# FunAudioLLM/CosyVoice

Measured on NVIDIA H100. Metric: audio-sec/s, CosyVoice2-0.5B zero-shot batch-32, NFE=10, higher is better.
Workload: dtype bf16

## Files before the change

cosyvoice_b200/csrc/cvk_internal.h:

```cpp
#pragma once
#include <cuda_runtime.h>
#include <cuda_bf16.h>
#include <cuda_fp16.h>
#include <cuda.h>
#include <stdint.h>
#include <stdio.h>
#include <string>
#include <vector>
#include <map>
#include <unordered_map>
#include <stdexcept>
#include <atomic>

#include "../../include/cvk.h"

typedef __nv_bfloat16 bf16;

struct CvkError : std::runtime_error {
  int code;
  CvkError(int c, const std::string& m) : std::runtime_error(m), code(c) {}
};

#define CVK_CHECK_CUDA(expr)                                                                       \
  do {                                                                                             \
    cudaError_t _e = (expr);                                                                       \
    if (_e != cudaSuccess)                                                                         \
      throw CvkError(CVK_ERR_CUDA, std::string(#expr) + ": " + cudaGetErrorString(_e) + " @" +     \
                                       __FILE__ + ":" + std::to_string(__LINE__));                 \
  } while (0)

#define CVK_REQUIRE(cond, msg)                                                                     \
  do {                                                                                             \
    if (!(cond))                                                                                   \
      throw CvkError(CVK_ERR_INVALID, std::string(msg) + " (" #cond ") @" + __FILE__ + ":" +       \
                                          std::to_string(__LINE__));                               \
  } while (0)

#define CVK_LAUNCH_CHECK() CVK_CHECK_CUDA(cudaGetLastError())

enum DType { DT_F32 = 0, DT_BF16 = 1, DT_F16 = 2 };

struct Mat {
  void* p = nullptr;
  int dtype = DT_F32;
  int rows = 0;
  int cols = 0;
  int ld = 0;
  Mat() {}
  Mat(void* p_, int dt, int r, int c, int ld_) : p(p_), dtype(dt), rows(r), cols(c), ld(ld_) {}
  size_t esize() const { return dtype == DT_F32 ? 4 : 2; }
  Mat slice(int c0, int n) const { return Mat((char*)p + (size_t)c0 * esize(), dtype, rows, n, ld); }
  float* f32() const { return (float*)p; }
  bf16* b16() const { return (bf16*)p; }
};

struct Seqs {
  int B = 0;
  int R = 0;
  std::vector<int> start, len;
  int* d_start = nullptr;
  int* d_len = nullptr;
  int* d_row2seq = nullptr;
  int max_len = 0;
  int64_t sum_len = 0;
};

struct ConvW {
  int N = 0, K = 0, taps = 1, dil = 1, shift0 = 0;
  float* w32 = nullptr;
  bf16* w16 = nullptr;
  __half* wf16 = nullptr;
  float* bias = nullptr;
};

enum Act {
  ACT_NONE = 0, ACT_GELU = 1, ACT_SILU = 2, ACT_MISH = 3, ACT_ELU = 4, ACT_LRELU = 5, ACT_SNAKE = 6, ACT_TANH = 7, ACT_ABS = 8,
  ACT_GELU_TANH = 9
};

struct Epilogue {
  const float* bias = nullptr;
  const float* rowvec = nullptr;
  int rowvec_ld = 0;
  int act1 = ACT_NONE;
  float act1_param = 0.f;
  const float* alpha1 = nullptr;
  float scale = 1.f;
  Mat resid;
  const int* row2seq = nullptr;
  int accumulate = 0;
  Mat out;
  int act2 = ACT_NONE;
  float act2_param = 0.f;
  const float* alpha2 = nullptr;
  Mat out2;
};

extern thread_local int cvk_in_capture;

struct Arena {
  char* base = nullptr;
  size_t cap = 0, off = 0, high = 0;
  void* alloc(size_t bytes) {
    size_t a = (off + 255) & ~(size_t)255;
    if (a + bytes > cap) throw CvkError(CVK_ERR_OOM, "workspace arena exhausted: need " + std::to_string(a + bytes) +
                                                          " of " + std::to_string(cap));
    off = a + bytes;
    if (off > high) high = off;
    return base + a;
  }
  void reset() { off = 0; }
};

struct RawTensor {
  float* p = nullptr;
  std::vector<int64_t> shape;
  int64_t numel() const { int64_t n = 1; for (auto s : shape) n *= s; return n; }
};

enum ProfFamily { FAM_GEMM_TC = 0, FAM_GEMM_SIMT = 1, FAM_ATTN = 2, FAM_COUNT = 3 };
struct ProfRec {
  cudaEvent_t a, b;
  int family;
  double work;
  double bytes;
};

struct HiftModel;
struct FlowModel;
struct DitModel;
struct LlmModel;

struct cvk_ctx {
  int device = 0;
  int precision = CVK_PREC_FP32;
  int act_dtype = DT_F32;
  int num_sms = 132;
  std::string last_error;
  std::map<std::string, RawTensor> raw;
  std::vector<void*> owned;
  Arena arena;
  HiftModel* hift = nullptr;
  HiftModel* hift3 = nullptr;
  void* hift3_extra = nullptr;
  FlowModel* flow = nullptr;
  DitModel* dit = nullptr;
  LlmModel* llm = nullptr;
  void* mel_model = nullptr;
  void* prompt_feat_model = nullptr;
  void* encode_tiled = nullptr;
  std::atomic<int64_t> launches{0};
  int op_out_bf16 = 0;
  int op_iters = 0;
  double op_ms = 0.0;
  int tc_epi = 2;
  int tc_persist = 2;
  void* tl = nullptr;
  int tl_seq = 0;
  long long* tl_next() {
    if (!tl) return nullptr;
    long long* p = (long long*)tl + 4 * (tl_seq % 1024);
    ++tl_seq;
    return p;
  }
  int prof_on = 0;
  std::vector<ProfRec> prof;
  std::unordered_map<const void*, void*> tiled;
  std::vector<cudaEvent_t> event_pool;
  int pdl = 1;
  int lm_fused = 1;
  int hift_f16 = 1;
  int build_f16 = 0;
  int enc_tc_attn = 1;
  int lm_mega = 0;
  int mega_coop = 1;
  int use_skinny = 1;
  int use_tc_attn = 1;
  int use_graph = 1;
  int use_tc = 1;
  int flow_fused_ff = 1;
  int flow_qkv_panel = 1;

  void* dmalloc(size_t bytes) {
    void* p = nullptr;
    CVK_CHECK_CUDA(cudaMalloc(&p, bytes ? bytes : 16));
    owned.push_back(p);
    return p;
  }
  const RawTensor& get_raw(const std::string& name) const {
    auto it = raw.find(name);
    if (it == raw.end()) throw CvkError(CVK_ERR_MISSING_WEIGHT, "missing weight tensor: " + name);
    return it->second;
  }
  bool has_raw(const std::string& name) const { return raw.find(name) != raw.end(); }
};

template <typename... KArgs, typename... Args>
inline void launch_ex(void (*kern)(KArgs...), dim3 grid, dim3 block, size_t smem, cudaStream_t st, bool pdl, Args&&... args) {
  cudaLaunchConfig_t cfg = {};
  cfg.gridDim = grid;
  cfg.blockDim = block;
  cfg.dynamicSmemBytes = smem;
  cfg.stream = st;
  cudaLaunchAttribute at[1];
  if (pdl) {
    at[0].id = cudaLaunchAttributeProgrammaticStreamSerialization;
    at[0].val.programmaticStreamSerializationAllowed = 1;
    cfg.attrs = at;
    cfg.numAttrs = 1;
  }
  CVK_CHECK_CUDA(cudaLaunchKernelEx(&cfg, kern, KArgs(std::forward<Args>(args))...));
}

void encode_tma_map(cvk_ctx* ctx, CUtensorMap* map, const void* base, int rank, const cuuint64_t* dims, const cuuint64_t* strides,
                    const cuuint32_t* box, int dtype, CUtensorMapL2promotion l2, const char* what);
void gemm_tc_setup();
void attention_tc_setup();
void skinny_setup();

Seqs make_seqs(cvk_ctx* ctx, const int* lens, int B, int gap, int scale, int extra_front, cudaStream_t st, bool with_row2seq = true);
Seqs scale_seqs(cvk_ctx* ctx, const Seqs& s, int scale, int extra_front, cudaStream_t st, bool with_row2seq = true);

ConvW make_linear(cvk_ctx* ctx, const std::string& wname, const std::string& bname);
ConvW make_conv(cvk_ctx* ctx, const float* w_oik , const float* bias, int N, int K, int taps,
                int dil, int shift0);
ConvW make_conv_named(cvk_ctx* ctx, const std::string& wname, const std::string& bname, int dil, int shift0);
float* fold_weight_norm(cvk_ctx* ctx, const std::string& prefix, int64_t* numel_out);
void finish_convw(cvk_ctx* ctx, ConvW& w);
float* dev_copy_f32(cvk_ctx* ctx, const float* src_dev, size_t n);

void conv_gemm(cvk_ctx* ctx, cudaStream_t st, const Mat& A, const ConvW& W, const Epilogue& ep);
void conv_gemm_simt(cvk_ctx* ctx, cudaStream_t st, const Mat& A, const ConvW& W, const Epilogue& ep);
void conv_gemm_tc(cvk_ctx* ctx, cudaStream_t st, const Mat& A, const ConvW& W, const Epilogue& ep);
void ffn_fused(cvk_ctx* ctx, cudaStream_t st, const Mat& x, const int* row2seq, const float* ln3_g, const float* ln3_b, const ConvW& w1,
               const ConvW& w2, const float* ln_g, const float* ln_b, const Mat& out);
void flow_ff(cvk_ctx* ctx, cudaStream_t st, const Mat& x, const int* row2seq, const float* ln3_g, const float* ln3_b, const ConvW& ff1,
             const ConvW& ff2, const float* ln_g, const float* ln_b, const Mat& out, const Mat& xn, const Mat& hid);
size_t skinny_scratch_floats(int rows, int maxN);
const bf16* skinny_tiled_weights(cvk_ctx* ctx, const ConvW& W);
int conv_gemm_skinny_ex(cvk_ctx* ctx, cudaStream_t st, const Mat& A, const ConvW& W, const Epilogue& ep, float* scratch, size_t scratch_floats,
                        int mode);
void conv_gemm_skinny(cvk_ctx* ctx, cudaStream_t st, const Mat& A, const ConvW& W, const Epilogue& ep, float* scratch, size_t scratch_floats);

void zero_mat(cvk_ctx* ctx, cudaStream_t st, const Mat& m);
void layernorm(cvk_ctx* ctx, cudaStream_t st, const Mat& x, const float* gamma, const float* beta, float eps, int act,
               float post_scale, const int* row2seq, const Mat& out, const float* rowvec = nullptr, int rowvec_ld = 0);
void unpack_rows_skip(cvk_ctx* ctx, cudaStream_t st, const Mat& in, const Seqs& s, const int* skip_host, float* dense, int C);
Seqs shrink_seqs(cvk_ctx* ctx, const Seqs& s, int drop_tail, cudaStream_t st);
Seqs subseqs(cvk_ctx* ctx, const Seqs& s, const int* skip_host, cudaStream_t st);
void rmsnorm(cvk_ctx* ctx, cudaStream_t st, const Mat& x, const float* gamma, float eps, const Mat& out);
void act_copy(cvk_ctx* ctx, cudaStream_t st, const Mat& x, int act, float param, const float* alpha, const int* row2seq,
              const Mat& out);
void act_copy_scaled(cvk_ctx* ctx, cudaStream_t st, const Mat& x, float pre_scale, int act, float param, const float* alpha,
                     const int* row2seq, const Mat& out);
void pack_rows(cvk_ctx* ctx, cudaStream_t st, const float* dense, int C, const Seqs& s, const Mat& out);
void unpack_rows(cvk_ctx* ctx, cudaStream_t st, const Mat& in, const Seqs& s, int skip, float* dense, int C);
void bcast_rows(cvk_ctx* ctx, cudaStream_t st, const float* vec, int C, int vec_ld, const Seqs& s, const Mat& out);
void convert_mat(cvk_ctx* ctx, cudaStream_t st, const Mat& in, const Mat& out);

struct KvGeom {
  const int* d_kstart = nullptr;
  const int* d_klen = nullptr;
  const int* d_qoff = nullptr;
};
void whisper_log_mel(cvk_ctx* ctx, const float* wav, const int* lens, int B, float* out, cudaStream_t st);
void kaldi_fbank80(cvk_ctx* ctx, const float* wav, const int* lens, int B, int subtract_mean, float* out, cudaStream_t st);
struct cvk_flow_stream;
cvk_flow_stream* flow_stream_create(cvk_ctx* ctx, int kind, int slots, int max_frames, int n_timesteps);
void flow_stream_destroy(cvk_flow_stream* fs);
size_t flow_stream_bytes(const cvk_flow_stream* fs);
void flow_stream_begin(cvk_ctx* ctx, cvk_flow_stream* fs, int slot, const float* prompt_feat, int prompt_frames, const float* embedding,
                       cudaStream_t st);
void flow_stream_chunk(cvk_ctx* ctx, cvk_flow_stream* fs, int B, const int* slots, const int32_t* tokens, const int* token_lens,
                       float* mel_out, int mel_cap_frames, int* n_out, cudaStream_t st);
void attention_fwd(cvk_ctx* ctx, cudaStream_t st, const Mat& q, const Mat& k, const Mat& v, const Seqs& s, int H, int chunk,
                   float scale, const Mat& out, int kv_div = 1, const KvGeom* kg = nullptr);
void relpos_attention_fwd(cvk_ctx* ctx, cudaStream_t st, const Mat& q, const Mat& k, const Mat& v, const Mat& pos ,
                          int pos_center, const float* bias_u, const float* bias_v, const Seqs& s, int H, int chunk, float scale,
                          const Mat& out);

struct ProfScope {
  cvk_ctx* ctx;
  cudaStream_t st;
  ProfRec rec;
  bool on;
  ProfScope(cvk_ctx* c, cudaStream_t s, int family, double work, double bytes) : ctx(c), st(s), on(c->prof_on && !cvk_in_capture) {
    if (!on) return;
    auto get = [&]() {
      cudaEvent_t e;
      if (!ctx->event_pool.empty()) { e = ctx->event_pool.back(); ctx->event_pool.pop_back(); }
      else cudaEventCreate(&e);
      return e;
    };
    rec.a = get(); rec.b = get(); rec.family = family; rec.work = work; rec.bytes = bytes;
    cudaEventRecord(rec.a, st);
  }
  ~ProfScope() {
    if (!on) return;
    cudaEventRecord(rec.b, st);
    ctx->prof.push_back(rec);
  }
};

static inline int ceil_div(int a, int b) { return (a + b - 1) / b; }
static inline int round_up(int a, int b) { return ceil_div(a, b) * b; }

inline Mat arena_mat(cvk_ctx* ctx, int dtype, int rows, int cols, int ld = 0) {
  if (ld == 0) ld = round_up(cols, 8);
  size_t es = dtype == DT_F32 ? 4 : 2;
  void* p = ctx->arena.alloc((size_t)rows * ld * es);
  return Mat(p, dtype, rows, cols, ld);
}
```

cosyvoice_b200/csrc/gemm_skinny.cu:

```cuda
#include "common.cuh"
#include "wgmma.cuh"
#include "tma.cuh"

namespace {

constexpr int SK_BM = 128;
constexpr int SK_BK = 64;
constexpr int SK_STAGES = 8;
constexpr int SK_THREADS = 384;

__global__ void tile_weights_kernel(const bf16* __restrict__ w, bf16* __restrict__ out, int N, int K, int tiles, int kchunks) {
  size_t total = (size_t)tiles * kchunks * SK_BM * 8;
  for (size_t i = blockIdx.x * (size_t)blockDim.x + threadIdx.x; i < total; i += (size_t)gridDim.x * blockDim.x) {
    int c = i & 7;
    int r = (i >> 3) & (SK_BM - 1);
    size_t blk = i >> 10;
    int kc = blk % kchunks, nt = blk / kchunks;
    int n = nt * SK_BM + r, k = kc * SK_BK + c * 8;
    uint4 v = make_uint4(0, 0, 0, 0);
    if (n < N && k + 8 <= K) v = *reinterpret_cast<const uint4*>(w + (size_t)n * K + k);
    else if (n < N && k < K) {
      __align__(16) bf16 t[8];
      for (int e = 0; e < 8; ++e) t[e] = k + e < K ? w[(size_t)n * K + k + e] : __float2bfloat16_rn(0.f);
      v = *reinterpret_cast<uint4*>(t);
    }
    *reinterpret_cast<uint4*>(reinterpret_cast<char*>(out) + blk * (SK_BM * SK_BK * 2) + r * 128 + ((c ^ (r & 7)) << 4)) = v;
  }
}

template <int BPAD>
__global__ void __launch_bounds__(SK_THREADS, 1)
skinny_gemm_kernel(const bf16* __restrict__ w_tiled, const __grid_constant__ CUtensorMap tmap_x, int N, int K, int rows,
                   int chunks_per_split, float* __restrict__ partial , EpiDev ep, int swiglu,
                   long long* __restrict__ tl) {
  extern __shared__ uint8_t smem_raw[];
  pdl_trigger();
  tl_stamp(tl, 0);
  __shared__ __align__(8) uint64_t bar_full[SK_STAGES];
  __shared__ __align__(8) uint64_t bar_empty[SK_STAGES];
  constexpr uint32_t A_BYTES = SK_BM * SK_BK * 2;
  constexpr uint32_t B_BYTES = BPAD * SK_BK * 2;
  constexpr uint32_t STAGE = A_BYTES + B_BYTES;

  const uint32_t base = (smem_u32(smem_raw) + 1023u) & ~1023u;
  const int warp = threadIdx.x >> 5, lane = threadIdx.x & 31;
  const int n0 = blockIdx.x * SK_BM;
  const int kchunks = (K + SK_BK - 1) / SK_BK;
  const int kc0 = blockIdx.y * chunks_per_split;
  const int kc1 = min(kchunks, kc0 + chunks_per_split);
  const int iters = kc1 - kc0;

  if (threadIdx.x == 0) {
    for (int s = 0; s < SK_STAGES; ++s) {
      mbar_init(smem_u32(&bar_full[s]), 1);
      mbar_init(smem_u32(&bar_empty[s]), 8);
    }
    asm volatile("fence.mbarrier_init.release.cluster;" ::: "memory");
  }
  __syncthreads();

  if (warp < 4) {
    if (warp == 0 && lane == 0) {
      const int pre = min(iters, SK_STAGES);
      for (int it = 0; it < pre; ++it) {
        const uint32_t fb = smem_u32(&bar_full[it]);
        mbar_expect_tx(fb, STAGE);
        bulk_load(base + it * STAGE, w_tiled + ((size_t)blockIdx.x * kchunks + (kc0 + it)) * (SK_BM * SK_BK), A_BYTES, fb);
      }
      pdl_wait();
      tl_stamp(tl, 1);
      for (int it = 0; it < pre; ++it) tma_load_2d(base + it * STAGE + A_BYTES, &tmap_x, smem_u32(&bar_full[it]), (kc0 + it) * SK_BK, 0);
      for (int it = pre; it < iters; ++it) {
        const int s = it % SK_STAGES;
        const uint32_t round = (uint32_t)(it / SK_STAGES);
        mbar_wait(smem_u32(&bar_empty[s]), (round & 1u) ^ 1u);
        const uint32_t sa = base + s * STAGE, sb = sa + A_BYTES;
        const uint32_t fb = smem_u32(&bar_full[s]);
        mbar_expect_tx(fb, STAGE);
        bulk_load(sa, w_tiled + ((size_t)blockIdx.x * kchunks + (kc0 + it)) * (SK_BM * SK_BK), A_BYTES, fb);
        tma_load_2d(sb, &tmap_x, fb, (kc0 + it) * SK_BK, 0);
      }
    } else {
      pdl_wait();
    }
  } else {
    const int wg = (threadIdx.x - 128) >> 7;
    const int q = lane & 3;
    const int fr = wg * 64 + (warp & 3) * 16 + (lane >> 2);
    float bias_n[2];
#pragma unroll
    for (int hh = 0; hh < 2; ++hh) bias_n[hh] = (!partial && !swiglu && ep.bias && n0 + fr + 8 * hh < N) ? ep.bias[n0 + fr + 8 * hh] : 0.f;
    pdl_wait();
    float acc[BPAD / 2];
#pragma unroll
    for (int e = 0; e < BPAD / 2; ++e) acc[e] = 0.f;
    for (int it = 0; it < iters; ++it) {
      const int s = it % SK_STAGES;
      mbar_wait(smem_u32(&bar_full[s]), (uint32_t)(it / SK_STAGES) & 1u);
      const uint32_t sa = base + s * STAGE + (uint32_t)wg * (A_BYTES / 2), sb = base + s * STAGE + A_BYTES;
      const uint64_t da = wg_desc_sw128(sa), db = wg_desc_sw128(sb);
      wg_fence();
#pragma unroll
      for (int k = 0; k < SK_BK / 16; ++k) wgmma_ss<BPAD, 0>(acc, da + (uint64_t)(2 * k), db + (uint64_t)(2 * k), 1);
      wg_commit();
      wg_wait<0>();
      __syncwarp();
      if (lane == 0) mbar_arrive(smem_u32(&bar_empty[s]));
    }
    wg_touch<BPAD / 2>(acc);
    const bool plain = ep.act1 == ACT_NONE && !ep.resid && !ep.rowvec && !ep.row2seq && !ep.accumulate && !ep.out2 && ep.scale == 1.f;
#pragma unroll
    for (int e = 0; e < BPAD / 2; ++e) {
      const int hh = (e >> 1) & 1;
      const int n = n0 + fr + 8 * hh, b = 8 * (e >> 2) + 2 * q + (e & 1);
      if (swiglu) {
        const float other = __shfl_xor_sync(0xffffffffu, acc[e], 4);
        if (!((lane >> 2) & 1) && n + 1 < N && b < rows) {
          const float g = acc[e];
          st_any(ep.out, ep.out_dtype, (size_t)b * ep.out_ld + (n >> 1), __fdividef(g, 1.f + fast_exp(-g)) * other);
        }
      } else if (n < N && b < rows) {
        if (partial) partial[((size_t)blockIdx.y * rows + b) * N + n] = acc[e];
        else if (plain) st_any(ep.out, ep.out_dtype, (size_t)b * ep.out_ld + n, acc[e] + bias_n[hh]);
        else epi_store(ep, b, n, acc[e]);
      }
    }
  }
  tl_stamp(tl, 2);
}

__global__ void splitk_finish_kernel(const float* __restrict__ partial, int splits, int rows, int N, EpiDev ep, long long* __restrict__ tl) {
  pdl_trigger();
  tl_stamp(tl, 0);
  pdl_wait();
  tl_stamp(tl, 1);
  size_t total = (size_t)rows * N;
  for (size_t i = blockIdx.x * (size_t)blockDim.x + threadIdx.x; i < total; i += (size_t)gridDim.x * blockDim.x) {
    float acc = 0.f;
    for (int s = 0; s < splits; ++s) acc += partial[(size_t)s * total + i];
    epi_store(ep, (int)(i / N), (int)(i % N), acc);
  }
  tl_stamp(tl, 2);
}

template <int BPAD>
constexpr size_t skinny_smem() {
  return (size_t)SK_STAGES * (SK_BM * SK_BK * 2 + BPAD * SK_BK * 2) + 1024;
}

template <int BPAD>
void launch(cudaStream_t st, dim3 grid, const bf16* tw, const CUtensorMap& tx, const ConvW& W, int rows, int cps, float* partial,
            const EpiDev& e, int swiglu, bool pdl, long long* tl) {
  launch_ex(skinny_gemm_kernel<BPAD>, grid, dim3(SK_THREADS), skinny_smem<BPAD>(), st, pdl, tw, tx, W.N, W.K, rows, cps, partial, e, swiglu, tl);
}

}

const bf16* skinny_tiled_weights(cvk_ctx* ctx, const ConvW& W) {
  auto it = ctx->tiled.find(W.w16);
  if (it != ctx->tiled.end()) return (const bf16*)it->second;
  CVK_REQUIRE(!cvk_in_capture, "skinny_tiled_weights: weight was not pre-tiled before graph capture");
  const int tiles = ceil_div(W.N, SK_BM), kchunks = ceil_div(W.K, SK_BK);
  bf16* out = (bf16*)ctx->dmalloc((size_t)tiles * kchunks * SK_BM * SK_BK * sizeof(bf16));
  tile_weights_kernel<<<ctx->num_sms * 8, 256>>>(W.w16, out, W.N, W.K, tiles, kchunks);
  CVK_LAUNCH_CHECK();
  CVK_CHECK_CUDA(cudaDeviceSynchronize());
  ctx->tiled[W.w16] = out;
  return out;
}

size_t skinny_scratch_floats(int rows, int maxN) { return (size_t)32 * rows * maxN; }

int conv_gemm_skinny_ex(cvk_ctx* ctx, cudaStream_t st, const Mat& A, const ConvW& W, const Epilogue& ep, float* scratch, size_t scratch_floats,
                        int mode) {
  CVK_REQUIRE(A.dtype == DT_BF16 && W.w16 != nullptr && W.taps == 1, "conv_gemm_skinny: bf16 1-tap operands required");
  const int rows = mode == 1 ? A.rows : ep.out.rows;
  CVK_REQUIRE(rows <= 64 && A.rows >= rows, "conv_gemm_skinny: at most 64 rows");
  CVK_REQUIRE(W.K % 8 == 0 && A.ld % 8 == 0 && ((uintptr_t)A.p & 15) == 0, "conv_gemm_skinny: 16-byte aligned operands required");
  const int BPAD = rows <= 32 ? 32 : 64;
  CUtensorMap tx;
  const bf16* tw = skinny_tiled_weights(ctx, W);
  {
    const cuuint64_t dims[2] = {(cuuint64_t)W.K, (cuuint64_t)rows};
    const cuuint64_t strides[1] = {(cuuint64_t)A.ld * 2};
    const cuuint32_t box[2] = {SK_BK, (cuuint32_t)BPAD};
    encode_tma_map(ctx, &tx, A.p, 2, dims, strides, box, DT_BF16, CU_TENSOR_MAP_L2_PROMOTION_L2_128B, "skinny x");
  }
  const int tiles = ceil_div(W.N, SK_BM);
  const int kchunks = ceil_div(W.K, SK_BK);
  int splits = ctx->num_sms / tiles;
  if (splits > kchunks / 4) splits = kchunks / 4;
  if (splits > 32) splits = 32;
  if (splits < 1) splits = 1;
  int cps = ceil_div(kchunks, splits);
  splits = ceil_div(kchunks, cps);
  if (mode == 2 || (splits > 1 && (scratch == nullptr || (size_t)splits * rows * W.N > scratch_floats))) {
    splits = 1;
    cps = kchunks;
  }
  CVK_REQUIRE(mode != 1 || (scratch != nullptr && (size_t)splits * rows * W.N <= scratch_floats), "conv_gemm_skinny: scratch too small");
  EpiDev e = to_dev(ep);
  if (!e.bias) e.bias = W.bias;
  const double flops = 2.0 * rows * (double)W.N * W.K;
  const double bytes = (double)W.N * W.K * 2 + (double)rows * W.K * 2 + (double)rows * W.N * 2;
  ProfScope ps(ctx, st, FAM_GEMM_TC, flops, bytes);
  dim3 grid(tiles, splits);
  float* partial = (splits > 1 || mode == 1) ? scratch : nullptr;
  long long* tl = ctx->tl_next();
  if (BPAD == 32) launch<32>(st, grid, tw, tx, W, rows, cps, partial, e, mode == 2, ctx->pdl != 0, tl);
  else launch<64>(st, grid, tw, tx, W, rows, cps, partial, e, mode == 2, ctx->pdl != 0, tl);
  ctx->launches++;
  CVK_LAUNCH_CHECK();
  if (splits > 1 && mode == 0) {
    size_t total = (size_t)rows * W.N;
    int g = (int)((total + 255) / 256);
    if (g > ctx->num_sms * 4) g = ctx->num_sms * 4;
    launch_ex(splitk_finish_kernel, dim3(g), dim3(256), 0, st, ctx->pdl != 0, (const float*)partial, splits, rows, W.N, e, ctx->tl_next());
    ctx->launches++;
    CVK_LAUNCH_CHECK();
  }
  return splits;
}

void conv_gemm_skinny(cvk_ctx* ctx, cudaStream_t st, const Mat& A, const ConvW& W, const Epilogue& ep, float* scratch, size_t scratch_floats) {
  conv_gemm_skinny_ex(ctx, st, A, W, ep, scratch, scratch_floats, 0);
}

void skinny_setup() {
  CVK_CHECK_CUDA(cudaFuncSetAttribute(skinny_gemm_kernel<32>, cudaFuncAttributeMaxDynamicSharedMemorySize, (int)skinny_smem<32>()));
  CVK_CHECK_CUDA(cudaFuncSetAttribute(skinny_gemm_kernel<64>, cudaFuncAttributeMaxDynamicSharedMemorySize, (int)skinny_smem<64>()));
  CVK_CHECK_CUDA(cudaFuncSetAttribute(skinny_gemm_kernel<32>, cudaFuncAttributePreferredSharedMemoryCarveout, cudaSharedmemCarveoutMaxShared));
  CVK_CHECK_CUDA(cudaFuncSetAttribute(skinny_gemm_kernel<64>, cudaFuncAttributePreferredSharedMemoryCarveout, cudaSharedmemCarveoutMaxShared));
  CVK_CHECK_CUDA(cudaFuncSetAttribute(splitk_finish_kernel, cudaFuncAttributePreferredSharedMemoryCarveout, cudaSharedmemCarveoutMaxShared));
}
```

cosyvoice_b200/csrc/llm.cu:

```cuda
#include "llm_decode_attn.cuh"
#include <math.h>
#include <algorithm>

using namespace lm;

namespace {

float* copy_param(cvk_ctx* ctx, const std::string& name) {
  const RawTensor& t = ctx->get_raw(name);
  return dev_copy_f32(ctx, t.p, (size_t)t.numel());
}

ConvW concat_linear(cvk_ctx* ctx, const std::vector<std::string>& wn, const std::vector<std::string>& bn) {
  int K = (int)ctx->get_raw(wn[0]).shape[1], N = 0;
  for (auto& n : wn) N += (int)ctx->get_raw(n).shape[0];
  ConvW w;
  w.N = N; w.K = K;
  w.w32 = (float*)ctx->dmalloc((size_t)N * K * sizeof(float));
  size_t off = 0;
  for (auto& n : wn) {
    const RawTensor& t = ctx->get_raw(n);
    CVK_CHECK_CUDA(cudaMemcpy(w.w32 + off, t.p, (size_t)t.numel() * sizeof(float), cudaMemcpyDeviceToDevice));
    off += t.numel();
  }
  if (!bn.empty()) {
    w.bias = (float*)ctx->dmalloc((size_t)N * sizeof(float));
    size_t bo = 0;
    for (auto& n : bn) {
      const RawTensor& t = ctx->get_raw(n);
      CVK_CHECK_CUDA(cudaMemcpy(w.bias + bo, t.p, (size_t)t.numel() * sizeof(float), cudaMemcpyDeviceToDevice));
      bo += t.numel();
    }
  }
  finish_convw(ctx, w);
  return w;
}

__global__ void build_input_kernel(const int32_t* __restrict__ text, const int* __restrict__ text_off, const int* __restrict__ text_len,
                                   const int32_t* __restrict__ speech, const int* __restrict__ sp_off, const int* __restrict__ sp_len,
                                   const float* __restrict__ text_emb, const float* __restrict__ llm_emb, const float* __restrict__ speech_emb,
                                   const int* __restrict__ start, float* __restrict__ out) {
  int b = blockIdx.y;
  int nt = text_len[b], ns = sp_len[b];
  int L = 1 + nt + 1 + ns;
  for (int t = blockIdx.x; t < L; t += gridDim.x) {
    const float* src;
    if (t == 0) src = llm_emb;
    else if (t <= nt) src = text_emb + (size_t)text[text_off[b] + t - 1] * D;
    else if (t == nt + 1) src = llm_emb + D;
    else src = speech_emb + (size_t)speech[sp_off[b] + t - nt - 2] * D;
    float* dst = out + (size_t)(start[b] + t) * D;
    for (int c = threadIdx.x; c < D; c += blockDim.x) dst[c] = src[c];
  }
}

template <typename T>
__global__ void rope_append_kernel(T* __restrict__ qkv, int ld, const int* __restrict__ start, const int* __restrict__ len,
                                   const int* __restrict__ pos0, const float* __restrict__ inv_freq, T* __restrict__ kc, T* __restrict__ vc,
                                   int max_ctx, int rows_are_seqs, const int2* __restrict__ rowpos) {
  int b = blockIdx.y;
  int L = rows_are_seqs ? 1 : len[b];
  int base = rows_are_seqs ? b : start[b];
  const int cb = rowpos ? rowpos[b].x : b;
  const int p0 = rowpos ? rowpos[b].y : (pos0 ? pos0[b] : 0);
  for (int t = blockIdx.x; t < L; t += gridDim.x) {
    int pos = p0 + t;
    T* row = qkv + (size_t)(base + t) * ld;
    for (int e = threadIdx.x; e < (NH + NKV) * (HD / 2); e += blockDim.x) {
      int h = e / (HD / 2), i = e % (HD / 2);
      float fr = (float)pos * inv_freq[i];
      float c = cosf(fr), s = sinf(fr);
      T* p = row + h * HD;
      float x1 = to_f32(p[i]), x2 = to_f32(p[i + HD / 2]);
      p[i] = from_f32<T>(x1 * c - x2 * s);
      p[i + HD / 2] = from_f32<T>(x2 * c + x1 * s);
    }
    __syncthreads();
    if (pos < max_ctx) {
      for (int e = threadIdx.x; e < NKV * HD; e += blockDim.x) {
        int h = e / HD, d = e % HD;
        size_t ci = (((size_t)cb * NKV + h) * max_ctx + pos) * HD + d;
        kc[ci] = row[NH * HD + e];
        vc[ci] = row[NH * HD + NKV * HD + e];
      }
    }
    __syncthreads();
  }
}

template <typename T>
__global__ void __launch_bounds__((NH / NKV) * 32)
decode_attn_kernel(const T* __restrict__ qkv, int ld, const T* __restrict__ kc, const T* __restrict__ vc,
                   const int* __restrict__ ctx_len, int max_ctx, T* __restrict__ out, int ldo, const int2* __restrict__ rowpos) {
  extern __shared__ float sc_all[];
  const int b = blockIdx.x, kvh = blockIdx.y;
  const int w = threadIdx.x >> 5, lane = threadIdx.x & 31;
  const int h = kvh * (NH / NKV) + w;
  const int cb = rowpos ? rowpos[b].x : b;
  const int L = min((rowpos ? rowpos[b].y : ctx_len[b]) + 1, max_ctx);
  float* sc = sc_all + (size_t)w * max_ctx;
  const T* q = qkv + (size_t)b * ld + h * HD;
  const T* kb = kc + ((size_t)cb * NKV + kvh) * max_ctx * HD;
  const T* vb = vc + ((size_t)cb * NKV + kvh) * max_ctx * HD;
  float qr[HD];
#pragma unroll
  for (int d = 0; d < HD; ++d) qr[d] = to_f32(q[d]) * 0.125f;
  float m = -INFINITY;
  for (int j = lane; j < L; j += 32) {
    const T* kr = kb + (size_t)j * HD;
    float s = 0.f;
    if (sizeof(T) == 2) {
      const uint4* k4 = reinterpret_cast<const uint4*>(kr);
#pragma unroll
      for (int c = 0; c < 8; ++c) {
        uint4 u = k4[c];
        const __nv_bfloat162* h2 = reinterpret_cast<const __nv_bfloat162*>(&u);
#pragma unroll
        for (int e = 0; e < 4; ++e) {
          float2 f = __bfloat1622float2(h2[e]);
          s = fmaf(qr[c * 8 + 2 * e], f.x, s);
          s = fmaf(qr[c * 8 + 2 * e + 1], f.y, s);
        }
      }
    } else {
      const float4* k4 = reinterpret_cast<const float4*>(kr);
#pragma unroll
      for (int c = 0; c < 16; ++c) {
        float4 f = k4[c];
        s = fmaf(qr[c * 4], f.x, s);
        s = fmaf(qr[c * 4 + 1], f.y, s);
        s = fmaf(qr[c * 4 + 2], f.z, s);
        s = fmaf(qr[c * 4 + 3], f.w, s);
      }
    }
    sc[j] = s;
    m = fmaxf(m, s);
  }
  m = warp_max(m);
  float l = 0.f;
  for (int j = lane; j < L; j += 32) {
    float p = expf(sc[j] - m);
    sc[j] = p;
    l += p;
  }
  l = warp_sum(l);
  __syncwarp();
  float o0 = 0.f, o1 = 0.f;
  int j = 0;
  for (; j + 4 <= L; j += 4) {
    float p0 = sc[j], p1 = sc[j + 1], p2 = sc[j + 2], p3 = sc[j + 3];
    const T* v0 = vb + (size_t)j * HD;
    float a0 = to_f32(v0[lane]), a1 = to_f32(v0[lane + 32]);
    float b0 = to_f32(v0[HD + lane]), b1 = to_f32(v0[HD + lane + 32]);
    float c0 = to_f32(v0[2 * HD + lane]), c1 = to_f32(v0[2 * HD + lane + 32]);
    float d0 = to_f32(v0[3 * HD + lane]), d1 = to_f32(v0[3 * HD + lane + 32]);
    o0 = fmaf(p0, a0, o0); o1 = fmaf(p0, a1, o1);
    o0 = fmaf(p1, b0, o0); o1 = fmaf(p1, b1, o1);
    o0 = fmaf(p2, c0, o0); o1 = fmaf(p2, c1, o1);
    o0 = fmaf(p3, d0, o0); o1 = fmaf(p3, d1, o1);
  }
  for (; j < L; ++j) {
    float p = sc[j];
    o0 = fmaf(p, to_f32(vb[(size_t)j * HD + lane]), o0);
    o1 = fmaf(p, to_f32(vb[(size_t)j * HD + lane + 32]), o1);
  }
  T* op = out + (size_t)b * ldo + h * HD;
  float inv = 1.f / l;
  op[lane] = from_f32<T>(o0 * inv);
  op[lane + 32] = from_f32<T>(o1 * inv);
}

__global__ void qkv_reduce_kernel(const float* __restrict__ partial, int splits, int rows, const float* __restrict__ bias, bf16* __restrict__ qkv) {
  const size_t total = (size_t)rows * QKV_N;
  for (size_t i = blockIdx.x * (size_t)blockDim.x + threadIdx.x; i < total; i += (size_t)gridDim.x * blockDim.x) {
    float acc = 0.f;
    for (int s = 0; s < splits; ++s) acc += partial[(size_t)s * total + i];
    qkv[i] = __float2bfloat16_rn(acc + bias[i % QKV_N]);
  }
}

__global__ void __launch_bounds__(D) finish_rms_kernel(const float* __restrict__ partial, int splits, int rows, float* __restrict__ x,
                                                       const float* __restrict__ gamma, bf16* __restrict__ xn, long long* __restrict__ tl) {
  __shared__ float red[D / 32];
  pdl_trigger();
  tl_stamp(tl, 0);
  const int b = blockIdx.x, n = threadIdx.x;
  const float gam = gamma[n];
  pdl_wait();
  tl_stamp(tl, 1);
  const float* p = partial + (size_t)b * D + n;
  const size_t stride = (size_t)rows * D;
  float a0 = 0.f, a1 = 0.f, a2 = 0.f, a3 = 0.f;
  int s = 0;
  for (; s + 4 <= splits; s += 4) {
    a0 += p[(size_t)s * stride];
    a1 += p[(size_t)(s + 1) * stride];
    a2 += p[(size_t)(s + 2) * stride];
    a3 += p[(size_t)(s + 3) * stride];
  }
  for (; s < splits; ++s) a0 += p[(size_t)s * stride];
  const float v = x[(size_t)b * D + n] + ((a0 + a1) + (a2 + a3));
  x[(size_t)b * D + n] = v;
  float ss = warp_sum(v * v);
  if ((n & 31) == 0) red[n >> 5] = ss;
  __syncthreads();
  float tot = 0.f;
#pragma unroll
  for (int i = 0; i < D / 32; ++i) tot += red[i];
  xn[(size_t)b * D + n] = __float2bfloat16_rn(gam * (v * rsqrtf(tot / D + RMS_EPS)));
  tl_stamp(tl, 2);
}

constexpr int AF_WARPS = 16;
__global__ void __launch_bounds__(32 * AF_WARPS)
attn_fused_kernel(const float* __restrict__ partial , int splits, int rows, const float* __restrict__ bias,
                  bf16* __restrict__ kc, bf16* __restrict__ vc, const int* __restrict__ ctx_len, int max_ctx,
                  const float* __restrict__ inv_freq, bf16* __restrict__ out, int ldo, long long* __restrict__ tl) {
  extern __shared__ float sm_all[];
  const int b = blockIdx.x, kvh = blockIdx.y;
  pdl_trigger();
  tl_stamp(tl, 0);
  bf16* kb = kc + ((size_t)b * NKV + kvh) * max_ctx * HD;
  bf16* vb = vc + ((size_t)b * NKV + kvh) * max_ctx * HD;
  const int p0 = min(*reinterpret_cast<const volatile int*>(ctx_len + b), max_ctx);
  const int wj0 = (threadIdx.x >> 5) * 16;
  KvFrag pre;
  const bool have_pre = wj0 + 16 <= p0;
  if (have_pre) decode_attn_load_block(kb, vb, wj0, p0, threadIdx.x & 31, pre);
  pdl_wait();
  tl_stamp(tl, 1);
  decode_attn_unit<AF_WARPS, 0>(sm_all, threadIdx.x, partial, splits, rows, b, kvh, bias, kb, vb, ctx_len[b], max_ctx, inv_freq,
                                out + (size_t)b * ldo, pre, have_pre);
  tl_stamp(tl, 2);
}

__global__ void interleave_rows_kernel(const float* __restrict__ gu , float* __restrict__ out, int F, int K) {
  size_t total = (size_t)2 * F * K;
  for (size_t i = blockIdx.x * (size_t)blockDim.x + threadIdx.x; i < total; i += (size_t)gridDim.x * blockDim.x) {
    int k = i % K;
    int r = i / K;
    int src = (r & 1) ? F + (r >> 1) : (r >> 1);
    out[i] = gu[(size_t)src * K + k];
  }
}

template <typename T>
__global__ void swiglu_kernel(const T* __restrict__ gu, int ld, int rows, T* __restrict__ out, int ldo) {
  size_t total = (size_t)rows * DFF;
  for (size_t i = blockIdx.x * (size_t)blockDim.x + threadIdx.x; i < total; i += (size_t)gridDim.x * blockDim.x) {
    int r = i / DFF, c = i % DFF;
    float g = to_f32(gu[(size_t)r * ld + c]), u = to_f32(gu[(size_t)r * ld + DFF + c]);
    out[(size_t)r * ldo + c] = from_f32<T>(g / (1.f + expf(-g)) * u);
  }
}

__global__ void gather_last_kernel(const float* __restrict__ x, const int* __restrict__ start, const int* __restrict__ len,
                                   float* __restrict__ out) {
  int b = blockIdx.x;
  const float* src = x + (size_t)(start[b] + len[b] - 1) * D;
  for (int c = threadIdx.x; c < D; c += blockDim.x) out[(size_t)b * D + c] = src[c];
}

__global__ void ragged_embed_kernel(const int* __restrict__ ids, const int* __restrict__ kinds, const float* __restrict__ text_emb,
                                    const float* __restrict__ llm_emb, const float* __restrict__ speech_emb, float* __restrict__ x) {
  const int m = blockIdx.x, kind = kinds[m], id = ids[m];
  const float* src = kind == 0 ? text_emb + (size_t)id * D : (kind == 1 ? speech_emb + (size_t)id * D : llm_emb + (size_t)id * D);
  for (int c = threadIdx.x; c < D; c += blockDim.x) x[(size_t)m * D + c] = src[c];
}

__global__ void feed_scatter_kernel(const int* __restrict__ sc, const float* __restrict__ x, float* __restrict__ hidden, int* __restrict__ ctx_len) {
  const int i = blockIdx.x, b = sc[3 * i], ml = sc[3 * i + 1];
  for (int c = threadIdx.x; c < D; c += blockDim.x) hidden[(size_t)b * D + c] = x[(size_t)ml * D + c];
  if (threadIdx.x == 0) ctx_len[b] += sc[3 * i + 2];
}

__global__ void gather_rows_kernel(const int* __restrict__ rows, const float* __restrict__ hidden, float* __restrict__ out) {
  const int i = blockIdx.x;
  for (int c = threadIdx.x; c < D; c += blockDim.x) out[(size_t)i * D + c] = hidden[(size_t)rows[i] * D + c];
}

__device__ __forceinline__ void mma_16816_full(float* c, uint32_t a0, uint32_t a1, uint32_t a2, uint32_t a3, uint32_t b0, uint32_t b1) {
  asm volatile("mma.sync.aligned.m16n8k16.row.col.f32.bf16.bf16.f32 {%0,%1,%2,%3}, {%4,%5,%6,%7}, {%8,%9}, {%0,%1,%2,%3};"
               : "+f"(c[0]), "+f"(c[1]), "+f"(c[2]), "+f"(c[3])
               : "r"(a0), "r"(a1), "r"(a2), "r"(a3), "r"(b0), "r"(b1));
}

constexpr int RA_WARPS = 4;
__global__ void __launch_bounds__(32 * RA_WARPS)
ragged_attn_tc_kernel(const bf16* __restrict__ qkv, int ld, const bf16* __restrict__ kc, const bf16* __restrict__ vc, int max_ctx,
                      const int4* __restrict__ tiles, bf16* __restrict__ out, int ldo) {
  constexpr int G = NH / NKV;
  __shared__ float ml[RA_WARPS][16][2];
  __shared__ __align__(16) float po[RA_WARPS][16][HD];
  const int4 tl = tiles[blockIdx.x];
  const int m0 = tl.x, b = tl.y, pos0 = tl.z, n = tl.w, kvh = blockIdx.y;
  const int warp = threadIdx.x >> 5, lane = threadIdx.x & 31, g = lane >> 2, t4 = lane & 3;
  const bf16* kb = kc + ((size_t)b * NKV + kvh) * max_ctx * HD;
  const bf16* vb = vc + ((size_t)b * NKV + kvh) * max_ctx * HD;
  const int L0 = pos0 + 1, L1 = pos0 + n;
  const bf16* qa_row = qkv + (size_t)m0 * ld + (kvh * G + g) * HD;
  const bf16* qb_row = qkv + (size_t)(m0 + n - 1) * ld + (kvh * G + g) * HD;
  auto qpair = [&](const bf16* p, int d) -> uint32_t {
    if (g >= G) return 0u;
    const float2 f = __bfloat1622float2(*reinterpret_cast<const __nv_bfloat162*>(p + d));
    return pack_bf16x2(f.x * 0.125f, f.y * 0.125f);
  };
  uint32_t qf[4][4];
#pragma unroll
  for (int kk = 0; kk < 4; ++kk) {
    const int d = kk * 16 + t4 * 2;
    qf[kk][0] = qpair(qa_row, d);
    qf[kk][1] = qpair(qb_row, d);
    qf[kk][2] = qpair(qa_row, d + 8);
    qf[kk][3] = qpair(qb_row, d + 8);
  }
  float o[4][2][4];
#pragma unroll
  for (int q = 0; q < 4; ++q)
#pragma unroll
    for (int t = 0; t < 2; ++t)
#pragma unroll
      for (int e = 0; e < 4; ++e) o[q][t][e] = 0.f;
  float m_a = -INFINITY, l_a = 0.f, m_b = -INFINITY, l_b = 0.f;
  KvFrag fr;
  for (int j0 = warp * 16; j0 < L1; j0 += RA_WARPS * 16) {
    decode_attn_load_block(kb, vb, j0, L1, lane, fr);
    float s0[4] = {0.f, 0.f, 0.f, 0.f}, s1[4] = {0.f, 0.f, 0.f, 0.f};
#pragma unroll
    for (int kk = 0; kk < 4; ++kk) {
      mma_16816_full(s0, qf[kk][0], qf[kk][1], qf[kk][2], qf[kk][3], fr.kf[0][kk][0], fr.kf[0][kk][1]);
      mma_16816_full(s1, qf[kk][0], qf[kk][1], qf[kk][2], qf[kk][3], fr.kf[1][kk][0], fr.kf[1][kk][1]);
    }
    const int ka = j0 + t4 * 2;
    const int key[4] = {ka, ka + 1, ka + 8, ka + 9};
    const float sa[4] = {s0[0], s0[1], s1[0], s1[1]}, sb[4] = {s0[2], s0[3], s1[2], s1[3]};
    float mxa = -INFINITY, mxb = -INFINITY;
#pragma unroll
    for (int e = 0; e < 4; ++e) {
      if (key[e] < L0) mxa = fmaxf(mxa, sa[e]);
      if (key[e] < L1) mxb = fmaxf(mxb, sb[e]);
    }
    mxa = fmaxf(mxa, __shfl_xor_sync(0xffffffffu, mxa, 1));
    mxa = fmaxf(mxa, __shfl_xor_sync(0xffffffffu, mxa, 2));
    mxb = fmaxf(mxb, __shfl_xor_sync(0xffffffffu, mxb, 1));
    mxb = fmaxf(mxb, __shfl_xor_sync(0xffffffffu, mxb, 2));
    const float na = fmaxf(m_a, mxa), nb = fmaxf(m_b, mxb);
    const float ua = na == -INFINITY ? 0.f : na, ub = nb == -INFINITY ? 0.f : nb;
    const float ca = __expf(m_a - ua), cb = __expf(m_b - ub);
    float pa[4], pb[4];
#pragma unroll
    for (int e = 0; e < 4; ++e) {
      pa[e] = key[e] < L0 ? __expf(sa[e] - ua) : 0.f;
      pb[e] = key[e] < L1 ? __expf(sb[e] - ub) : 0.f;
    }
    l_a = l_a * ca + ((pa[0] + pa[1]) + (pa[2] + pa[3]));
    l_b = l_b * cb + ((pb[0] + pb[1]) + (pb[2] + pb[3]));
    m_a = na;
    m_b = nb;
    const uint32_t p0 = pack_bf16x2(pa[0], pa[1]), p1 = pack_bf16x2(pb[0], pb[1]), p2 = pack_bf16x2(pa[2], pa[3]), p3 = pack_bf16x2(pb[2], pb[3]);
#pragma unroll
    for (int q = 0; q < 4; ++q) {
#pragma unroll
      for (int t = 0; t < 2; ++t) {
        o[q][t][0] *= ca; o[q][t][1] *= ca;
        o[q][t][2] *= cb; o[q][t][3] *= cb;
      }
      mma_16816_full(o[q][0], p0, p1, p2, p3, __byte_perm(fr.vw[q][0], fr.vw[q][1], 0x5410), __byte_perm(fr.vw[q][2], fr.vw[q][3], 0x5410));
      mma_16816_full(o[q][1], p0, p1, p2, p3, __byte_perm(fr.vw[q][0], fr.vw[q][1], 0x7632), __byte_perm(fr.vw[q][2], fr.vw[q][3], 0x7632));
    }
  }
  l_a += __shfl_xor_sync(0xffffffffu, l_a, 1);
  l_a += __shfl_xor_sync(0xffffffffu, l_a, 2);
  l_b += __shfl_xor_sync(0xffffffffu, l_b, 1);
  l_b += __shfl_xor_sync(0xffffffffu, l_b, 2);
  if (g < G) {
    if (t4 == 0) {
      ml[warp][g][0] = m_a;
      ml[warp][g][1] = l_a;
      ml[warp][g + 8][0] = m_b;
      ml[warp][g + 8][1] = l_b;
    }
#pragma unroll
    for (int q = 0; q < 4; ++q) {
      *reinterpret_cast<float4*>(&po[warp][g][q * 16 + t4 * 4]) = make_float4(o[q][0][0], o[q][1][0], o[q][0][1], o[q][1][1]);
      *reinterpret_cast<float4*>(&po[warp][g + 8][q * 16 + t4 * 4]) = make_float4(o[q][0][2], o[q][1][2], o[q][0][3], o[q][1][3]);
    }
  }
  __syncthreads();
  for (int e = threadIdx.x; e < n * G * HD; e += 32 * RA_WARPS) {
    const int r = e / (G * HD), hq = (e / HD) % G, d = e % HD, mr = r * 8 + hq;
    float M = -INFINITY;
#pragma unroll
    for (int w2 = 0; w2 < RA_WARPS; ++w2) M = fmaxf(M, ml[w2][mr][0]);
    float num = 0.f, den = 0.f;
#pragma unroll
    for (int w2 = 0; w2 < RA_WARPS; ++w2) {
      const float wgt = __expf(ml[w2][mr][0] - M);
      den = fmaf(wgt, ml[w2][mr][1], den);
      num = fmaf(wgt, po[w2][mr][d], num);
    }
    out[(size_t)(m0 + r) * ldo + (kvh * G + hq) * HD + d] = __float2bfloat16_rn(num / den);
  }
}

static inline size_t sampler_smem(int V) { return (size_t)2 * ((V + 3) & ~3) * sizeof(float); }

__device__ __forceinline__ float block_max(float v, float* red) {
  v = warp_max(v);
  __syncthreads();
  if ((threadIdx.x & 31) == 0) red[threadIdx.x >> 5] = v;
  __syncthreads();
  float r = red[0];
  for (int i = 1; i < SAMPLER_THREADS / 32; ++i) r = fmaxf(r, red[i]);
  return r;
}
__device__ __forceinline__ float block_hsum(float seg, float* part, float* total) {
  __syncthreads();
  part[threadIdx.x] = seg;
  __syncthreads();
  if (threadIdx.x == 0) {
    float t = 0.f;
    for (int i = 0; i < SAMPLER_THREADS; ++i) t += part[i];
    *total = t;
  }
  __syncthreads();
  return *total;
}

__global__ void __launch_bounds__(SAMPLER_THREADS)
ras_sampler_kernel(float* __restrict__ scores, int V, int from_logits, const float* __restrict__ uniforms , int B,
                   const int32_t* __restrict__ min_len, const int32_t* __restrict__ max_len, int32_t* __restrict__ out_ids, int out_ld,
                   int32_t* __restrict__ out_count, int32_t* __restrict__ done, int* __restrict__ ctx_len, const int* __restrict__ base_len,
                   int* __restrict__ live,
                   const float* __restrict__ speech_emb, float* __restrict__ next_x,
                   const int32_t* __restrict__ history, int hist_ld, const int32_t* __restrict__ hist_count,
                   const int32_t* __restrict__ ignore_eos_in, int32_t* __restrict__ ids_out, const float* __restrict__ ln_gamma,
                   bf16* __restrict__ xn_out, long long* __restrict__ tl, long long* __restrict__ dbg_fine) {
  extern __shared__ __align__(16) float sp_all[];
  __shared__ float red[SAMPLER_THREADS / 32];
  __shared__ float part[SAMPLER_THREADS];
  __shared__ float tot;
  __shared__ int bi[2][SAMPLER_THREADS / 32];
  __shared__ float kept_p[TOPK];
  __shared__ int kept_i[TOPK];
  __shared__ int s_n, s_top;

  const int b = blockIdx.x, tid = threadIdx.x;
  const bool standalone = ids_out != nullptr;
  pdl_trigger();
  tl_stamp(tl, 0);
  pdl_wait();
  tl_stamp(tl, 1);
  long long* sf = (dbg_fine && b == 0 && tid == 0) ? dbg_fine : nullptr;
  int sf_i = 0;
#define SF() do { if (sf) { long long t_; asm volatile("mov.u64 %0, %globaltimer;" : "=l"(t_)); sf[sf_i++] = t_; } } while (0)
  SF();
  if (!standalone && done[b]) { tl_stamp(tl, 2); return; }
  const int V4 = (V + 3) & ~3;
  float* sp = sp_all;
  float* x = sp_all + V4;
  float* xg = scores + (size_t)b * V;
  if ((V & 3) == 0) {
    for (int i = tid; i < V / 4; i += SAMPLER_THREADS) reinterpret_cast<float4*>(x)[i] = __ldcg(reinterpret_cast<const float4*>(xg) + i);
  } else {
    for (int i = tid; i < V; i += SAMPLER_THREADS) x[i] = __ldcg(xg + i);
  }
  const int per = (V + SAMPLER_THREADS - 1) / SAMPLER_THREADS;
  const int lo = tid * per, hi = min(lo + per, V);
  const int cnt = standalone ? hist_count[b] : out_count[b];
  const bool ignore_eos = standalone ? (ignore_eos_in[b] != 0) : (cnt < min_len[b]);
  const float u1 = standalone ? uniforms[b * 2] : uniforms[((size_t)cnt * B + b) * 2];
  const float u2 = standalone ? uniforms[b * 2 + 1] : uniforms[((size_t)cnt * B + b) * 2 + 1];
  __syncthreads();
  float xr[SAMPLER_PER], pr[SAMPLER_PER];
#pragma unroll
  for (int i = 0; i < SAMPLER_PER; ++i) xr[i] = (i < per && lo + i < hi) ? x[lo + i] : -INFINITY;
  SF();

  if (from_logits) {
    float mx = -INFINITY;
#pragma unroll
    for (int i = 0; i < SAMPLER_PER; ++i) mx = fmaxf(mx, xr[i]);
    mx = block_max(mx, red);
    float seg = 0.f;
#pragma unroll
    for (int i = 0; i < SAMPLER_PER; ++i)
      if (i < per && lo + i < hi) seg += expf(xr[i] - mx);
    float s = block_hsum(seg, part, &tot);
    float ls = logf(s);
#pragma unroll
    for (int i = 0; i < SAMPLER_PER; ++i)
      if (i < per && lo + i < hi) xr[i] = (xr[i] - mx) - ls;
  }
  SF();
  if (ignore_eos) {
#pragma unroll
    for (int i = 0; i < SAMPLER_PER; ++i)
      if (i < per && lo + i == EOS && lo + i < hi) xr[i] = -INFINITY;
  }
  float mx = -INFINITY;
#pragma unroll
  for (int i = 0; i < SAMPLER_PER; ++i) mx = fmaxf(mx, xr[i]);
  mx = block_max(mx, red);
  {
    float seg = 0.f;
#pragma unroll
    for (int i = 0; i < SAMPLER_PER; ++i) {
      const bool ok = i < per && lo + i < hi;
      float e = (!ok || xr[i] == -INFINITY) ? 0.f : expf(xr[i] - mx);
      pr[i] = e;
      if (ok) seg += e;
    }
    float s = block_hsum(seg, part, &tot);
#pragma unroll
    for (int i = 0; i < SAMPLER_PER; ++i) pr[i] = (i < per && lo + i < hi) ? pr[i] / s : -3.f;
  }
  SF();
  float c_v[3];
  int c_i[3], c_n;
  auto rebuild = [&]() {
    c_v[0] = c_v[1] = c_v[2] = -1.f;
    c_i[0] = c_i[1] = c_i[2] = -1;
#pragma unroll
    for (int i = 0; i < SAMPLER_PER; ++i) {
      const float v = pr[i];
      const int ix = lo + i;
      if (v > c_v[0]) { c_v[2] = c_v[1]; c_i[2] = c_i[1]; c_v[1] = c_v[0]; c_i[1] = c_i[0]; c_v[0] = v; c_i[0] = ix; }
      else if (v > c_v[1]) { c_v[2] = c_v[1]; c_i[2] = c_i[1]; c_v[1] = v; c_i[1] = ix; }
      else if (v > c_v[2]) { c_v[2] = v; c_i[2] = ix; }
    }
    c_n = (c_v[0] >= 0.f) + (c_v[1] >= 0.f) + (c_v[2] >= 0.f);
  };
  rebuild();
  __shared__ unsigned bk[2][SAMPLER_THREADS / 32];
  __shared__ int s_cnt[SAMPLER_THREADS / 32 + 1];
  __shared__ unsigned s_thr_key;
  int n_kept = 0;
  float cum = 0.f;
  constexpr int CAND_CAP = 512;
  unsigned* tk = reinterpret_cast<unsigned*>(sp);
  int* ti = reinterpret_cast<int*>(sp) + SAMPLER_THREADS;
  float* cv = sp + 2 * SAMPLER_THREADS;
  int* ci = reinterpret_cast<int*>(sp) + 2 * SAMPLER_THREADS + CAND_CAP;
  bool fast_done = false;
  {
    const unsigned mykey = c_n > 0 ? __float_as_uint(c_v[0]) + 1u : 0u;
    const int myidx = c_n > 0 ? c_i[0] : 0x7fffffff;
    tk[tid] = mykey;
    ti[tid] = myidx;
    __syncthreads();
    int rank = 0;
    for (int q = 0; q < SAMPLER_THREADS / 4; ++q) {
      const uint4 k4 = reinterpret_cast<const uint4*>(tk)[q];
      const int4 i4 = reinterpret_cast<const int4*>(ti)[q];
      rank += (k4.x > mykey || (k4.x == mykey && i4.x < myidx)) + (k4.y > mykey || (k4.y == mykey && i4.y < myidx)) +
              (k4.z > mykey || (k4.z == mykey && i4.z < myidx)) + (k4.w > mykey || (k4.w == mykey && i4.w < myidx));
    }
    if (tid == 0) s_thr_key = 0u;
    __syncthreads();
    if (rank == TOPK - 1) s_thr_key = mykey;
    __syncthreads();
    const unsigned thr = s_thr_key;
    if (thr != 0u) {
      int cnt = 0;
#pragma unroll
      for (int i = 0; i < SAMPLER_PER; ++i) cnt += (pr[i] >= 0.f && __float_as_uint(pr[i]) + 1u >= thr) ? 1 : 0;
      int incl = cnt;
#pragma unroll
      for (int o = 1; o < 32; o <<= 1) {
        const int t = __shfl_up_sync(0xffffffffu, incl, o);
        if ((tid & 31) >= o) incl += t;
      }
      if ((tid & 31) == 31) s_cnt[tid >> 5] = incl;
      __syncthreads();
      int base = 0, total = 0;
#pragma unroll
      for (int w = 0; w < SAMPLER_THREADS / 32; ++w) {
        if (w < (tid >> 5)) base += s_cnt[w];
        total += s_cnt[w];
      }
      if (total <= CAND_CAP) {
        int pos = base + incl - cnt;
#pragma unroll
        for (int i = 0; i < SAMPLER_PER; ++i)
          if (pr[i] >= 0.f && __float_as_uint(pr[i]) + 1u >= thr) { cv[pos] = pr[i]; ci[pos] = lo + i; ++pos; }
        __syncthreads();
        for (int j = tid; j < total; j += SAMPLER_THREADS) {
          const float vj = cv[j];
          const int ij = ci[j];
          int r = 0;
          for (int k = 0; k < total; ++k) r += (cv[k] > vj || (cv[k] == vj && ci[k] < ij)) ? 1 : 0;
          if (r < TOPK) { kept_p[r] = vj; kept_i[r] = ij; }
        }
        __syncthreads();
        const int avail = total < TOPK ? total : TOPK;
        while (n_kept < avail && cum < 0.8f) {
          cum = cum + kept_p[n_kept];
          ++n_kept;
        }
        fast_done = true;
      }
    }
  }
  for (int round = 0; round < TOPK && !fast_done; ++round) {
    if (!(cum < 0.8f)) break;
    const unsigned key = c_n > 0 ? __float_as_uint(c_v[0]) + 1u : 0u;
    const unsigned wmax = __reduce_max_sync(0xffffffffu, key);
    const int widx = __reduce_min_sync(0xffffffffu, (key == wmax && wmax != 0u) ? c_i[0] : 0x7fffffff);
    const int pb = round & 1;
    if ((tid & 31) == 0) { bk[pb][tid >> 5] = wmax; bi[pb][tid >> 5] = widx; }
    __syncthreads();
    unsigned gk = bk[pb][0];
    int gi = bi[pb][0];
#pragma unroll
    for (int w = 1; w < SAMPLER_THREADS / 32; ++w) {
      const unsigned k2 = bk[pb][w];
      const int i2 = bi[pb][w];
      if (k2 > gk || (k2 == gk && i2 < gi)) { gk = k2; gi = i2; }
    }
    if (gk == 0u) break;
    const float gv = __uint_as_float(gk - 1u);
    if (tid == 0) {
      kept_p[n_kept] = gv;
      kept_i[n_kept] = gi;
    }
    n_kept += 1;
    cum = cum + gv;
    if (gi >= lo && gi < hi) {
#pragma unroll
      for (int i = 0; i < SAMPLER_PER; ++i)
        if (lo + i == gi) pr[i] = -2.f;
      c_v[0] = c_v[1]; c_i[0] = c_i[1];
      c_v[1] = c_v[2]; c_i[1] = c_i[2];
      c_v[2] = -1.f; c_i[2] = -1;
      if (--c_n == 0) rebuild();
    }
  }
  SF();
  if (tid == 0) {
    int n = n_kept;
    float total = 0.f;
    for (int i = 0; i < n; ++i) total += kept_p[i];
    float thr = u1 * total, acc = 0.f;
    int pick = -1, last = -1;
    for (int i = 0; i < n; ++i) {
      if (kept_p[i] > 0.f) last = i;
      acc += kept_p[i];
      if (pick < 0 && acc > thr && kept_p[i] > 0.f) pick = i;
    }
    if (pick < 0) pick = last;
    int top = kept_i[pick];
    int rep = 0;
    const int32_t* hist = standalone ? history + (size_t)b * hist_ld : out_ids + (size_t)b * out_ld;
    for (int i = max(0, cnt - WIN); i < cnt; ++i) rep += hist[i] == top;
    s_top = top;
    s_n = rep >= 1 ? 1 : 0;
  }
  __syncthreads();
  SF();
  if (s_n) {
    int top = s_top;
#pragma unroll
    for (int i = 0; i < SAMPLER_PER; ++i)
      if (lo + i == top) xr[i] = -INFINITY;
    float m3 = -INFINITY;
#pragma unroll
    for (int i = 0; i < SAMPLER_PER; ++i) m3 = fmaxf(m3, xr[i]);
    m3 = block_max(m3, red);
    float seg = 0.f;
#pragma unroll
    for (int i = 0; i < SAMPLER_PER; ++i) {
      const bool ok = i < per && lo + i < hi;
      float e = (!ok || xr[i] == -INFINITY) ? 0.f : expf(xr[i] - m3);
      pr[i] = e;
      if (ok) seg += e;
    }
    float s = block_hsum(seg, part, &tot);
    seg = 0.f;
#pragma unroll
    for (int i = 0; i < SAMPLER_PER; ++i) {
      if (i < per && lo + i < hi) {
        pr[i] = pr[i] / s;
        seg += pr[i];
        sp[lo + i] = pr[i];
      }
    }
    __syncthreads();
    part[tid] = seg;
    __syncthreads();
    if (tid == 0) {
      float pre = 0.f;
      for (int i = 0; i < SAMPLER_THREADS; ++i) pre += part[i];
      float thr = u2 * pre;
      float acc = 0.f;
      int segi = -1, lastseg = -1;
      float segbase = 0.f, lastbase = 0.f;
      for (int i = 0; i < SAMPLER_THREADS; ++i) {
        if (part[i] > 0.f) {
          lastseg = i;
          lastbase = acc;
          if (acc + part[i] > thr) { segi = i; segbase = acc; break; }
        }
        acc += part[i];
      }
      int pick = -1, last = -1;
      if (segi < 0) { segi = lastseg; segbase = lastbase; }
      float sgbase = segbase;
      for (int sg = segi; sg >= 0 && sg < SAMPLER_THREADS && pick < 0; ++sg) {
        const float a0 = sgbase;
        sgbase += part[sg];
        if (sg > segi && !(part[sg] > 0.f)) continue;
        float a = a0;
        int l2 = sg * per, h2 = min(l2 + per, V);
        for (int i = l2; i < h2; ++i) {
          if (sp[i] > 0.f) last = i;
          a += sp[i];
          if (a > thr && sp[i] > 0.f) { pick = i; break; }
        }
      }
      if (pick < 0) pick = last;
      s_top = pick;
    }
    __syncthreads();
  }
  SF();
#pragma unroll
  for (int i = 0; i < SAMPLER_PER; ++i)
    if (i < per && lo + i < hi) x[lo + i] = xr[i];
  __syncthreads();
  const int top = s_top;
  if ((V & 3) == 0) {
    for (int i = tid; i < V / 4; i += SAMPLER_THREADS) reinterpret_cast<float4*>(xg)[i] = reinterpret_cast<const float4*>(x)[i];
  } else {
    for (int i = tid; i < V; i += SAMPLER_THREADS) xg[i] = x[i];
  }
  SF();
  if (standalone) {
    if (tid == 0) ids_out[b] = top;
    return;
  }
  const bool stop = top >= EOS;
  if (!stop) {
    float ss = 0.f;
    float ev[(D + SAMPLER_THREADS - 1) / SAMPLER_THREADS];
#pragma unroll
    for (int k = 0; k < (D + SAMPLER_THREADS - 1) / SAMPLER_THREADS; ++k) {
      const int c = tid + k * SAMPLER_THREADS;
      ev[k] = c < D ? speech_emb[(size_t)top * D + c] : 0.f;
    }
#pragma unroll
    for (int k = 0; k < (D + SAMPLER_THREADS - 1) / SAMPLER_THREADS; ++k) {
      const int c = tid + k * SAMPLER_THREADS;
      if (c < D) {
        next_x[(size_t)b * D + c] = ev[k];
        ss += ev[k] * ev[k];
      }
    }
    if (xn_out) {
      ss = warp_sum(ss);
      __syncthreads();
      if ((tid & 31) == 0) red[tid >> 5] = ss;
      __syncthreads();
      float t2 = 0.f;
      for (int i = 0; i < SAMPLER_THREADS / 32; ++i) t2 += red[i];
      const float r = rsqrtf(t2 / D + RMS_EPS);
#pragma unroll
      for (int k = 0; k < (D + SAMPLER_THREADS - 1) / SAMPLER_THREADS; ++k) {
        const int c = tid + k * SAMPLER_THREADS;
        if (c < D) xn_out[(size_t)b * D + c] = __float2bfloat16_rn(ln_gamma[c] * (ev[k] * r));
      }
    }
  }
  if (tid == 0) {
    bool fin = stop;
    if (!stop) {
      out_ids[(size_t)b * out_ld + cnt] = top;
      out_count[b] = cnt + 1;
      ctx_len[b] = base_len[b] + cnt;
      if (cnt + 1 >= max_len[b]) fin = true;
    }
    if (fin) {
      done[b] = 1;
      atomicSub(live, 1);
    }
  }
  SF();
  tl_stamp(tl, 2);
#undef SF
}

__global__ void logsoftmax_rows_kernel(float* __restrict__ x, int V) {
  __shared__ float red[SAMPLER_THREADS / 32];
  __shared__ float part[SAMPLER_THREADS];
  __shared__ float tot;
  float* row = x + (size_t)blockIdx.x * V;
  const int per = (V + SAMPLER_THREADS - 1) / SAMPLER_THREADS;
  const int lo = threadIdx.x * per, hi = min(lo + per, V);
  float mx = -INFINITY;
  for (int i = lo; i < hi; ++i) mx = fmaxf(mx, row[i]);
  mx = block_max(mx, red);
  float seg = 0.f;
  for (int i = lo; i < hi; ++i) seg += expf(row[i] - mx);
  float s = block_hsum(seg, part, &tot);
  float ls = logf(s);
  for (int i = lo; i < hi; ++i) row[i] = (row[i] - mx) - ls;
}

__global__ void init_state_kernel(const int* __restrict__ len, int B, int* ctx_len, int* base_len, int* live) {
  int b = threadIdx.x;
  if (b < B) {
    ctx_len[b] = len[b];
    base_len[b] = len[b];
  }
  if (b == 0) *live = B;
}

int* upload(cvk_ctx* ctx, const std::vector<int>& v, cudaStream_t st) {
  int* d = (int*)ctx->arena.alloc(sizeof(int) * (v.size() ? v.size() : 1));
  if (!v.empty()) CVK_CHECK_CUDA(cudaMemcpyAsync(d, v.data(), sizeof(int) * v.size(), cudaMemcpyHostToDevice, st));
  return d;
}
std::vector<int> prefix(const int* lens, int B) {
  std::vector<int> off(B);
  int a = 0;
  for (int b = 0; b < B; ++b) { off[b] = a; a += lens[b]; }
  return off;
}

void lm_gemm(cvk_ctx* ctx, cudaStream_t st, const Mat& A, const ConvW& W, const Epilogue& e, float* scratch, size_t scratch_floats) {
  if (scratch && A.dtype == DT_BF16 && ctx->use_tc && ctx->use_skinny && e.out.rows <= 64 && W.w16)
    conv_gemm_skinny(ctx, st, A, W, e, scratch, scratch_floats);
  else
    conv_gemm(ctx, st, A, W, e);
}

static Mat row_slice(const Mat& a, int r0, int n) { return Mat((char*)a.p + (size_t)r0 * a.ld * a.esize(), a.dtype, n, a.cols, a.ld); }

void lm_gemm_rows(cvk_ctx* ctx, cudaStream_t st, const Mat& A, const ConvW& W, const Epilogue& e, float* scratch, size_t scratch_floats) {
  if (!(scratch && A.dtype == DT_BF16 && ctx->use_tc && ctx->use_skinny && W.w16)) {
    conv_gemm(ctx, st, A, W, e);
    return;
  }
  for (int r0 = 0; r0 < e.out.rows; r0 += 64) {
    const int n = std::min(64, e.out.rows - r0);
    Epilogue es = e;
    es.out = row_slice(e.out, r0, n);
    if (e.resid.p) es.resid = row_slice(e.resid, r0, n);
    conv_gemm_skinny(ctx, st, row_slice(A, r0, n), W, es, scratch, scratch_floats);
  }
}

struct RaggedPass {
  const int2* rowpos = nullptr;
  const int4* tiles = nullptr;
  int ntiles = 0;
};

void layer_forward(cvk_ctx* ctx, cudaStream_t st, const LlmModel* m, int li, const Mat& x, const Mat& xn, const Mat& qkv, const Mat& att,
                   const Mat& gu, const Mat& ffa, const Seqs* s, cvk_lm_session* sess, bool decode, const RaggedPass* rg = nullptr) {
  const LayerW& w = m->layers[li];
  const int rows = x.rows;
  float* scr = rg ? sess->fscratch : (decode ? sess->scratch : nullptr);
  const size_t scr_n = rg ? sess->fscratch_floats : (decode ? sess->scratch_floats : 0);
  rmsnorm(ctx, st, x, w.ln1, RMS_EPS, xn);
  {
    Epilogue e;
    e.out = qkv;
    (rg ? lm_gemm_rows : lm_gemm)(ctx, st, xn, w.qkv, e, scr, scr_n);
  }
  size_t es = qkv.dtype == DT_F32 ? 4 : 2;
  void* kc = sess ? (char*)sess->kcache + (size_t)li * sess->max_batch * NKV * sess->max_ctx * HD * es : nullptr;
  void* vc = sess ? (char*)sess->vcache + (size_t)li * sess->max_batch * NKV * sess->max_ctx * HD * es : nullptr;
  if (rg) {
    if (qkv.dtype == DT_F32) {
      rope_append_kernel<float><<<dim3(1, rows), 128, 0, st>>>(qkv.f32(), qkv.ld, nullptr, nullptr, nullptr, m->d_inv_freq, (float*)kc,
                                                               (float*)vc, sess->max_ctx, 1, rg->rowpos);
      decode_attn_kernel<float><<<dim3(rows, NKV), (NH / NKV) * 32, (NH / NKV) * sess->max_ctx * sizeof(float), st>>>(
          qkv.f32(), qkv.ld, (const float*)kc, (const float*)vc, nullptr, sess->max_ctx, att.f32(), att.ld, rg->rowpos);
    } else {
      rope_append_kernel<bf16><<<dim3(1, rows), 128, 0, st>>>(qkv.b16(), qkv.ld, nullptr, nullptr, nullptr, m->d_inv_freq, (bf16*)kc,
                                                              (bf16*)vc, sess->max_ctx, 1, rg->rowpos);
      ragged_attn_tc_kernel<<<dim3(rg->ntiles, NKV), 32 * RA_WARPS, 0, st>>>(qkv.b16(), qkv.ld, (const bf16*)kc, (const bf16*)vc, sess->max_ctx,
                                                                              rg->tiles, att.b16(), att.ld);
    }
    ctx->launches += 2;
    CVK_LAUNCH_CHECK();
  } else if (decode) {
    if (qkv.dtype == DT_F32) {
      rope_append_kernel<float><<<dim3(1, rows), 128, 0, st>>>(qkv.f32(), qkv.ld, nullptr, nullptr, sess->ctx_len, m->d_inv_freq, (float*)kc,
                                                               (float*)vc, sess->max_ctx, 1, nullptr);
      decode_attn_kernel<float><<<dim3(rows, NKV), (NH / NKV) * 32, (NH / NKV) * sess->max_ctx * sizeof(float), st>>>(qkv.f32(), qkv.ld, (const float*)kc, (const float*)vc, sess->ctx_len, sess->max_ctx,
                                                          att.f32(), att.ld, nullptr);
    } else {
      rope_append_kernel<bf16><<<dim3(1, rows), 128, 0, st>>>(qkv.b16(), qkv.ld, nullptr, nullptr, sess->ctx_len, m->d_inv_freq, (bf16*)kc,
                                                              (bf16*)vc, sess->max_ctx, 1, nullptr);
      decode_attn_kernel<bf16><<<dim3(rows, NKV), (NH / NKV) * 32, (NH / NKV) * sess->max_ctx * sizeof(float), st>>>(qkv.b16(), qkv.ld, (const bf16*)kc, (const bf16*)vc, sess->ctx_len, sess->max_ctx,
                                                         att.b16(), att.ld, nullptr);
    }
    ctx->launches += 2;
    CVK_LAUNCH_CHECK();
  } else {
    int bx = s->max_len < 256 ? s->max_len : 256;
    int mc = sess ? sess->max_ctx : 0;
    if (qkv.dtype == DT_F32)
      rope_append_kernel<float><<<dim3(bx, s->B), 128, 0, st>>>(qkv.f32(), qkv.ld, s->d_start, s->d_len, nullptr, m->d_inv_freq, (float*)kc,
                                                                (float*)vc, mc, 0, nullptr);
    else
      rope_append_kernel<bf16><<<dim3(bx, s->B), 128, 0, st>>>(qkv.b16(), qkv.ld, s->d_start, s->d_len, nullptr, m->d_inv_freq, (bf16*)kc,
                                                               (bf16*)vc, mc, 0, nullptr);
    ctx->launches++;
    CVK_LAUNCH_CHECK();
    attention_fwd(ctx, st, qkv.slice(0, NH * HD), qkv.slice(NH * HD, NKV * HD), qkv.slice(NH * HD + NKV * HD, NKV * HD), *s, NH, 1, 0.125f,
                  att, NH / NKV);
  }
  {
    Epilogue e;
    e.resid = x;
    e.out = x;
    (rg ? lm_gemm_rows : lm_gemm)(ctx, st, att, w.o, e, scr, scr_n);
  }
  rmsnorm(ctx, st, x, w.ln2, RMS_EPS, xn);
  {
    Epilogue e;
    e.out = gu;
    (rg ? lm_gemm_rows : lm_gemm)(ctx, st, xn, w.gate_up, e, scr, scr_n);
  }
  {
    size_t total = (size_t)rows * DFF;
    int g = (int)((total + 255) / 256);
    if (g > 132 * 8) g = 132 * 8;
    if (gu.dtype == DT_F32) swiglu_kernel<float><<<g, 256, 0, st>>>(gu.f32(), gu.ld, rows, ffa.f32(), ffa.ld);
    else swiglu_kernel<bf16><<<g, 256, 0, st>>>(gu.b16(), gu.ld, rows, ffa.b16(), ffa.ld);
    ctx->launches++;
    CVK_LAUNCH_CHECK();
  }
  {
    Epilogue e;
    e.resid = x;
    e.out = x;
    (rg ? lm_gemm_rows : lm_gemm)(ctx, st, ffa, w.down, e, scr, scr_n);
  }
}

void head_logits(cvk_ctx* ctx, cudaStream_t st, const LlmModel* m, const Mat& hidden_f32, const Mat& xn_act, const Mat& logits,
                 cvk_lm_session* sess = nullptr) {
  rmsnorm(ctx, st, hidden_f32, m->final_norm, RMS_EPS, xn_act);
  Epilogue e;
  e.out = logits;
  lm_gemm(ctx, st, xn_act, m->head, e, sess ? sess->scratch : nullptr, sess ? sess->scratch_floats : 0);
}

void decode_attn_allow_ctx(int max_ctx) {
  static int decode_attn_smem = 0;
  const size_t need = (size_t)(NH / NKV) * max_ctx * sizeof(float);
  CVK_REQUIRE(need <= 200 * 1024, "session context too long for the decode attention kernel (max ~7300 positions)");
  if ((int)need > decode_attn_smem) {
    CVK_CHECK_CUDA(cudaFuncSetAttribute(decode_attn_kernel<float>, cudaFuncAttributeMaxDynamicSharedMemorySize, (int)need));
    CVK_CHECK_CUDA(cudaFuncSetAttribute(decode_attn_kernel<bf16>, cudaFuncAttributeMaxDynamicSharedMemorySize, (int)need));
    decode_attn_smem = (int)need;
  }
}

constexpr size_t ATTN_FUSED_SMEM = ((NH / NKV + 2) * HD + AF_WARPS * 8 * 2 + AF_WARPS * (NH / NKV) * HD) * sizeof(float);

}

void lm_rope_inv_freq(float* out) {
  for (int i = 0; i < HD / 2; ++i) out[i] = 1.0f / powf(ROPE_THETA, (float)(2 * i) / (float)HD);
}

void llm_decode_attention_op(cvk_ctx* ctx, const float* partial, int splits, int rows, const float* bias, float* k_cache, float* v_cache,
                             const int* ctx_len_host, int max_ctx, float* out, cudaStream_t st) {
  decode_attn_allow_ctx(max_ctx);
  ctx->arena.reset();
  float inv[HD / 2];
  lm_rope_inv_freq(inv);
  float* d_inv = (float*)ctx->arena.alloc(sizeof(inv));
  CVK_CHECK_CUDA(cudaMemcpyAsync(d_inv, inv, sizeof(inv), cudaMemcpyHostToDevice, st));
  int* d_len = upload(ctx, std::vector<int>(ctx_len_host, ctx_len_host + rows), st);
  const int cache_rows = rows * NKV * max_ctx;
  Mat k32(k_cache, DT_F32, cache_rows, HD, HD), v32(v_cache, DT_F32, cache_rows, HD, HD);
  Mat kc = arena_mat(ctx, DT_BF16, cache_rows, HD, HD), vc = arena_mat(ctx, DT_BF16, cache_rows, HD, HD);
  Mat att = arena_mat(ctx, DT_BF16, rows, D, D);
  convert_mat(ctx, st, k32, kc);
  convert_mat(ctx, st, v32, vc);
  if (ctx->lm_fused) {
    launch_ex(attn_fused_kernel, dim3(rows, NKV), dim3(32 * AF_WARPS), ATTN_FUSED_SMEM, st, false, partial, splits, rows, bias, kc.b16(),
              vc.b16(), (const int*)d_len, max_ctx, (const float*)d_inv, att.b16(), att.ld, (long long*)nullptr);
    ctx->launches++;
  } else {
    Mat qkv = arena_mat(ctx, DT_BF16, rows, QKV_N, QKV_N);
    qkv_reduce_kernel<<<ceil_div(rows * QKV_N, 256), 256, 0, st>>>(partial, splits, rows, bias, qkv.b16());
    rope_append_kernel<bf16><<<dim3(1, rows), 128, 0, st>>>(qkv.b16(), qkv.ld, nullptr, nullptr, d_len, d_inv, kc.b16(), vc.b16(), max_ctx, 1, nullptr);
    decode_attn_kernel<bf16><<<dim3(rows, NKV), (NH / NKV) * 32, (NH / NKV) * max_ctx * sizeof(float), st>>>(
        qkv.b16(), qkv.ld, kc.b16(), vc.b16(), d_len, max_ctx, att.b16(), att.ld, nullptr);
    ctx->launches += 3;
  }
  CVK_LAUNCH_CHECK();
  convert_mat(ctx, st, kc, k32);
  convert_mat(ctx, st, vc, v32);
  convert_mat(ctx, st, att, Mat(out, DT_F32, rows, D, D));
  CVK_CHECK_CUDA(cudaStreamSynchronize(st));
}

void llm_ragged_attention_op(cvk_ctx* ctx, const float* q, const float* k_cache, const float* v_cache, int cache_rows, int max_ctx,
                             const int* rowpos, int M, float* out, cudaStream_t st) {
  for (int i = 0; i < M; ++i)
    CVK_REQUIRE(rowpos[2 * i] >= 0 && rowpos[2 * i] < cache_rows && rowpos[2 * i + 1] >= 0 && rowpos[2 * i + 1] < max_ctx,
                "cvk_op_ragged_attention: row or position out of range");
  std::vector<int> tiles;
  for (int i = 0; i < M;) {
    const int n = (i + 1 < M && rowpos[2 * i + 2] == rowpos[2 * i] && rowpos[2 * i + 3] == rowpos[2 * i + 1] + 1) ? 2 : 1;
    tiles.insert(tiles.end(), {i, rowpos[2 * i], rowpos[2 * i + 1], n});
    i += n;
  }
  ctx->arena.reset();
  const int ntiles = (int)tiles.size() / 4;
  int* d_tiles = upload(ctx, tiles, st);
  const int crows = cache_rows * NKV * max_ctx;
  Mat q16 = arena_mat(ctx, DT_BF16, M, D, D), kc = arena_mat(ctx, DT_BF16, crows, HD, HD), vc = arena_mat(ctx, DT_BF16, crows, HD, HD),
      att = arena_mat(ctx, DT_BF16, M, D, D);
  convert_mat(ctx, st, Mat(const_cast<float*>(q), DT_F32, M, D, D), q16);
  convert_mat(ctx, st, Mat(const_cast<float*>(k_cache), DT_F32, crows, HD, HD), kc);
  convert_mat(ctx, st, Mat(const_cast<float*>(v_cache), DT_F32, crows, HD, HD), vc);
  ragged_attn_tc_kernel<<<dim3(ntiles, NKV), 32 * RA_WARPS, 0, st>>>(q16.b16(), q16.ld, kc.b16(), vc.b16(), max_ctx,
                                                                     reinterpret_cast<const int4*>(d_tiles), att.b16(), att.ld);
  ctx->launches++;
  CVK_LAUNCH_CHECK();
  convert_mat(ctx, st, att, Mat(out, DT_F32, M, D, D));
  CVK_CHECK_CUDA(cudaStreamSynchronize(st));
}

void llm_build(cvk_ctx* ctx, const int* cfg, int ncfg) {
  LlmModel* m = new LlmModel();
  if (ncfg >= 1) m->num_layers = cfg[0];
  const std::string P = "llm.";
  m->text_emb = copy_param(ctx, P + "llm.model.model.embed_tokens.weight");
  m->speech_emb = copy_param(ctx, P + "speech_embedding.weight");
  if (ctx->has_raw(P + "llm_embedding.weight")) {
    m->llm_emb = copy_param(ctx, P + "llm_embedding.weight");
    m->head = make_linear(ctx, P + "llm_decoder.weight", P + "llm_decoder.bias");
  } else {
    const RawTensor& se = ctx->get_raw(P + "speech_embedding.weight");
    const RawTensor& hw = ctx->get_raw(P + "llm_decoder.weight");
    CVK_REQUIRE(se.shape[0] == VOUT3 && hw.shape[0] == VOUT3 && hw.shape[1] == D, "CosyVoice3LM: speech_embedding / llm_decoder must have 6761 rows");
    m->llm_emb = (float*)ctx->dmalloc(2 * D * sizeof(float));
    CVK_CHECK_CUDA(cudaMemcpy(m->llm_emb, se.p + (size_t)EOS * D, D * sizeof(float), cudaMemcpyDeviceToDevice));
    CVK_CHECK_CUDA(cudaMemcpy(m->llm_emb + D, se.p + (size_t)(EOS + 2) * D, D * sizeof(float), cudaMemcpyDeviceToDevice));
    float* wpad = (float*)ctx->dmalloc((size_t)VOUT3_PAD * D * sizeof(float));
    CVK_CHECK_CUDA(cudaMemset(wpad, 0, (size_t)VOUT3_PAD * D * sizeof(float)));
    CVK_CHECK_CUDA(cudaMemcpy(wpad, hw.p, (size_t)VOUT3 * D * sizeof(float), cudaMemcpyDeviceToDevice));
    std::vector<float> hb(VOUT3_PAD, 0.f);
    for (int i = VOUT3; i < VOUT3_PAD; ++i) hb[i] = -1.0e30f;
    float* bpad = (float*)ctx->dmalloc(VOUT3_PAD * sizeof(float));
    CVK_CHECK_CUDA(cudaMemcpy(bpad, hb.data(), VOUT3_PAD * sizeof(float), cudaMemcpyHostToDevice));
    m->head = make_conv(ctx, wpad, bpad, VOUT3_PAD, D, 1, 1, 0);
    m->vout = VOUT3_PAD;
  }
  m->final_norm = copy_param(ctx, P + "llm.model.model.norm.weight");
  if (ctx->precision == CVK_PREC_BF16) skinny_tiled_weights(ctx, m->head);
  for (int i = 0; i < m->num_layers; ++i) {
    std::string L = P + "llm.model.model.layers." + std::to_string(i);
    LayerW w;
    w.ln1 = copy_param(ctx, L + ".input_layernorm.weight");
    w.ln2 = copy_param(ctx, L + ".post_attention_layernorm.weight");
    w.qkv = concat_linear(ctx, {L + ".self_attn.q_proj.weight", L + ".self_attn.k_proj.weight", L + ".self_attn.v_proj.weight"},
                          {L + ".self_attn.q_proj.bias", L + ".self_attn.k_proj.bias", L + ".self_attn.v_proj.bias"});
    w.o = make_linear(ctx, L + ".self_attn.o_proj.weight", "");
    w.gate_up = concat_linear(ctx, {L + ".mlp.gate_proj.weight", L + ".mlp.up_proj.weight"}, {});
    w.down = make_linear(ctx, L + ".mlp.down_proj.weight", "");
    if (ctx->precision == CVK_PREC_BF16) {
      w.gate_up_il.N = 2 * DFF; w.gate_up_il.K = D;
      w.gate_up_il.w32 = (float*)ctx->dmalloc((size_t)2 * DFF * D * sizeof(float));
      interleave_rows_kernel<<<132 * 8, 256>>>(w.gate_up.w32, w.gate_up_il.w32, DFF, D);
      CVK_LAUNCH_CHECK();
      finish_convw(ctx, w.gate_up_il);
    }
    if (ctx->precision == CVK_PREC_BF16) {
      skinny_tiled_weights(ctx, w.qkv); skinny_tiled_weights(ctx, w.o); skinny_tiled_weights(ctx, w.gate_up); skinny_tiled_weights(ctx, w.down);
      skinny_tiled_weights(ctx, w.gate_up_il);
      CVK_CHECK_CUDA(cudaFree(w.gate_up_il.w32));
      for (auto it = ctx->owned.begin(); it != ctx->owned.end(); ++it) if (*it == (void*)w.gate_up_il.w32) { ctx->owned.erase(it); break; }
      w.gate_up_il.w32 = nullptr;
    }
    m->layers.push_back(w);
  }
  lm_rope_inv_freq(m->inv_freq);
  m->d_inv_freq = (float*)ctx->dmalloc(sizeof(m->inv_freq));
  CVK_CHECK_CUDA(cudaMemcpy(m->d_inv_freq, m->inv_freq, sizeof(m->inv_freq), cudaMemcpyHostToDevice));
  CVK_CHECK_CUDA(cudaDeviceSynchronize());
  ctx->llm = m;
  if (ctx->precision == CVK_PREC_BF16) lm_mega_build(ctx, m);
}

cvk_lm_session* llm_session_create(cvk_ctx* ctx, int max_batch, int max_context) {
  CVK_REQUIRE(ctx->llm, "llm stage not finalised");
  cvk_lm_session* s = new cvk_lm_session();
  s->max_batch = max_batch;
  s->max_ctx = max_context;
  s->kv_dtype = ctx->act_dtype;
  size_t es = s->kv_dtype == DT_F32 ? 4 : 2;
  auto alloc = [&](size_t bytes) {
    void* p = nullptr;
    CVK_CHECK_CUDA(cudaMalloc(&p, bytes ? bytes : 16));
    CVK_CHECK_CUDA(cudaMemset(p, 0, bytes));
    s->owned.push_back(p);
    return p;
  };
  size_t cache = (size_t)ctx->llm->num_layers * max_batch * NKV * max_context * HD * es;
  s->kcache = alloc(cache);
  s->vcache = alloc(cache);
  s->ctx_len = (int*)alloc(sizeof(int) * max_batch);
  s->base_len = (int*)alloc(sizeof(int) * max_batch);
  CVK_CHECK_CUDA(cudaFuncSetAttribute(ras_sampler_kernel, cudaFuncAttributeMaxDynamicSharedMemorySize, (int)sampler_smem(VOUT3_PAD)));
  CVK_REQUIRE((NH / NKV) * max_context * sizeof(float) <= 200 * 1024, "session context too long for the decode attention kernel");
  decode_attn_allow_ctx(max_context);
  CVK_CHECK_CUDA(cudaFuncSetAttribute(attn_fused_kernel, cudaFuncAttributePreferredSharedMemoryCarveout, cudaSharedmemCarveoutMaxShared));
  CVK_CHECK_CUDA(cudaFuncSetAttribute(finish_rms_kernel, cudaFuncAttributePreferredSharedMemoryCarveout, cudaSharedmemCarveoutMaxShared));
  CVK_CHECK_CUDA(cudaFuncSetAttribute(ras_sampler_kernel, cudaFuncAttributePreferredSharedMemoryCarveout, cudaSharedmemCarveoutMaxShared));
  CVK_CHECK_CUDA(cudaFuncSetAttribute(attn_fused_kernel, cudaFuncAttributeMaxDynamicSharedMemorySize, (int)ATTN_FUSED_SMEM));
  s->count = (int*)alloc(sizeof(int) * max_batch);
  s->done = (int*)alloc(sizeof(int) * max_batch);
  s->live = (int*)alloc(sizeof(int));
  s->x = (float*)alloc(sizeof(float) * max_batch * D);
  s->hidden = (float*)alloc(sizeof(float) * max_batch * D);
  s->logits = (float*)alloc(sizeof(float) * (size_t)max_batch * VOUT3_PAD);
  s->xn = alloc(es * max_batch * D);
  s->qkv = alloc(es * max_batch * QKV_N);
  s->att = alloc(es * max_batch * D);
  s->gu = alloc(es * (size_t)max_batch * 2 * DFF);
  s->ffa = alloc(es * (size_t)max_batch * DFF);
  s->scratch_floats = skinny_scratch_floats(max_batch, 2 * DFF);
  s->scratch = (float*)alloc(s->scratch_floats * sizeof(float));
  s->sel = (int*)alloc(sizeof(int) * max_batch);
  s->rows_fed.assign(max_batch, 0);
  lm_mega_session_init(ctx, s);
  return s;
}

void llm_session_destroy(cvk_ctx* ctx, cvk_lm_session* s) {
  cudaSetDevice(ctx->device);
  if (s->graph) cudaGraphExecDestroy(s->graph);
  for (void* p : s->owned) cudaFree(p);
  lm_mega_session_free(s);
  delete s;
}

static Mat forward_packed(cvk_ctx* ctx, cudaStream_t st, const Seqs& s, const Mat& x, cvk_lm_session* sess) {
  const LlmModel* m = ctx->llm;
  const int adt = ctx->act_dtype;
  Mat xn = arena_mat(ctx, adt, s.R, D), qkv = arena_mat(ctx, adt, s.R, QKV_N), att = arena_mat(ctx, adt, s.R, D),
      gu = arena_mat(ctx, adt, s.R, 2 * DFF), ffa = arena_mat(ctx, adt, s.R, DFF);
  zero_mat(ctx, st, att);
  for (int li = 0; li < m->num_layers; ++li) layer_forward(ctx, st, m, li, x, xn, qkv, att, gu, ffa, &s, sess, false);
  return x;
}

void llm_prefill(cvk_ctx* ctx, cvk_lm_session* sess, const int32_t* text, const int* text_lens, const int32_t* speech,
                 const int* speech_lens, int B, cudaStream_t st) {
  const LlmModel* m = ctx->llm;
  CVK_REQUIRE(m, "llm stage not finalised");
  CVK_REQUIRE(B <= sess->max_batch, "batch larger than the session");
  ctx->arena.reset();
  std::vector<int> lens(B);
  for (int b = 0; b < B; ++b) {
    lens[b] = 1 + text_lens[b] + 1 + speech_lens[b];
    CVK_REQUIRE(lens[b] < sess->max_ctx, "prompt longer than the session context");
  }
  Seqs s = make_seqs(ctx, lens.data(), B, 0, 1, 0, st);
  Mat x = arena_mat(ctx, DT_F32, s.R, D, D);
  zero_mat(ctx, st, x);
  int* toff = upload(ctx, prefix(text_lens, B), st);
  int* tlen = upload(ctx, std::vector<int>(text_lens, text_lens + B), st);
  int* soff = upload(ctx, prefix(speech_lens, B), st);
  int* slen = upload(ctx, std::vector<int>(speech_lens, speech_lens + B), st);
  int bx = s.max_len < 512 ? s.max_len : 512;
  build_input_kernel<<<dim3(bx, B), 128, 0, st>>>(text, toff, tlen, speech, soff, slen, m->text_emb, m->llm_emb, m->speech_emb, s.d_start, x.f32());
  ctx->launches++;
  CVK_LAUNCH_CHECK();
  if (sess->graph) {
    cudaGraphExecDestroy(sess->graph);
    sess->graph = nullptr;
  }
  forward_packed(ctx, st, s, x, sess);
  gather_last_kernel<<<B, 128, 0, st>>>(x.f32(), s.d_start, s.d_len, sess->hidden);
  CVK_REQUIRE(sess->max_batch <= 1024, "max_batch > 1024");
  init_state_kernel<<<1, sess->max_batch < 32 ? 32 : round_up(sess->max_batch, 32), 0, st>>>(s.d_len, B, sess->ctx_len, sess->base_len, sess->live);
  sess->fresh = true;
  sess->ragged = false;
  ctx->launches += 2;
  CVK_LAUNCH_CHECK();
  sess->B = B;
}

static bool lm_fused_path(cvk_ctx* ctx, cvk_lm_session* s) {
  return s->kv_dtype == DT_BF16 && ctx->use_tc && ctx->use_skinny && ctx->lm_fused && s->g_B <= 64;
}

static void decode_layers_fused(cvk_ctx* ctx, cudaStream_t st, cvk_lm_session* s) {
  const LlmModel* m = ctx->llm;
  const int B = s->g_B;
  if (lm_mega_usable(ctx, s, B)) {
    lm_mega_layers(ctx, st, s, B);
    return;
  }
  const bool pdl = ctx->pdl != 0;
  Mat xn(s->xn, DT_BF16, B, D, D), att(s->att, DT_BF16, B, D, D), ffa(s->ffa, DT_BF16, B, DFF, DFF);
  for (int li = 0; li < m->num_layers; ++li) {
    const LayerW& w = m->layers[li];
    bf16* kc = (bf16*)s->kcache + (size_t)li * s->max_batch * NKV * s->max_ctx * HD;
    bf16* vc = (bf16*)s->vcache + (size_t)li * s->max_batch * NKV * s->max_ctx * HD;
    Epilogue none;
    int sp = conv_gemm_skinny_ex(ctx, st, xn, w.qkv, none, s->scratch, s->scratch_floats, 1);
    launch_ex(attn_fused_kernel, dim3(B, NKV), dim3(32 * AF_WARPS), ATTN_FUSED_SMEM, st, pdl, (const float*)s->scratch, sp, B,
              (const float*)w.qkv.bias, kc, vc, (const int*)s->ctx_len, s->max_ctx, (const float*)m->d_inv_freq, att.b16(), att.ld, ctx->tl_next());
    ctx->launches++;
    CVK_LAUNCH_CHECK();
    sp = conv_gemm_skinny_ex(ctx, st, att, w.o, none, s->scratch, s->scratch_floats, 1);
    launch_ex(finish_rms_kernel, dim3(B), dim3(D), 0, st, pdl, (const float*)s->scratch, sp, B, s->x, (const float*)w.ln2, xn.b16(), ctx->tl_next());
    ctx->launches++;
    CVK_LAUNCH_CHECK();
    {
      Epilogue e;
      e.out = ffa;
      conv_gemm_skinny_ex(ctx, st, xn, w.gate_up_il, e, s->scratch, s->scratch_floats, 2);
    }
    sp = conv_gemm_skinny_ex(ctx, st, ffa, w.down, none, s->scratch, s->scratch_floats, 1);
    const float* next_gamma = li + 1 < m->num_layers ? m->layers[li + 1].ln1 : m->final_norm;
    launch_ex(finish_rms_kernel, dim3(B), dim3(D), 0, st, pdl, (const float*)s->scratch, sp, B, s->x, next_gamma, xn.b16(), ctx->tl_next());
    ctx->launches++;
    CVK_LAUNCH_CHECK();
  }
}

static void decode_step_fused(cvk_ctx* ctx, cudaStream_t st, cvk_lm_session* s) {
  const LlmModel* m = ctx->llm;
  const int B = s->g_B;
  const bool fused = true;
  ctx->tl_seq = 0;
  Mat xn(s->xn, DT_BF16, B, D, D), logits(s->logits, DT_F32, B, m->vout, m->vout);
  {
    Epilogue e;
    e.out = logits;
    conv_gemm_skinny_ex(ctx, st, xn, m->head, e, s->scratch, s->scratch_floats, 0);
  }
  const bool pdl = ctx->pdl != 0;
  launch_ex(ras_sampler_kernel, dim3(B), dim3(SAMPLER_THREADS), sampler_smem(m->vout), st, pdl, s->logits, m->vout, 1, s->g_uniforms, B, s->g_min,
            s->g_max, s->g_out_ids, s->g_out_ld, s->g_out_count, s->g_done, s->ctx_len, (const int*)s->base_len, s->live,
            (const float*)m->speech_emb, s->x, (const int32_t*)nullptr, 0, (const int32_t*)nullptr, (const int32_t*)nullptr, (int32_t*)nullptr,
            (const float*)(fused ? m->layers[0].ln1 : nullptr), fused ? (bf16*)s->xn : (bf16*)nullptr, ctx->tl_next(),
            ctx->tl ? (long long*)ctx->tl + 1024 : (long long*)nullptr);
  ctx->launches++;
  CVK_LAUNCH_CHECK();
  decode_layers_fused(ctx, st, s);
}

static void decode_step(cvk_ctx* ctx, cudaStream_t st, cvk_lm_session* s) {
  if (lm_fused_path(ctx, s)) {
    decode_step_fused(ctx, st, s);
    return;
  }
  const LlmModel* m = ctx->llm;
  const int adt = s->kv_dtype;
  const int B = s->g_B;
  const bool fused = false;
  Mat hid(s->hidden, DT_F32, B, D, D), x(s->x, DT_F32, B, D, D), xn(s->xn, adt, B, D, D), qkv(s->qkv, adt, B, QKV_N, QKV_N),
      att(s->att, adt, B, D, D), gu(s->gu, adt, B, 2 * DFF, 2 * DFF), ffa(s->ffa, adt, B, DFF, DFF), logits(s->logits, DT_F32, B, m->vout, m->vout);
  head_logits(ctx, st, m, hid, xn, logits, s);
  ras_sampler_kernel<<<B, SAMPLER_THREADS, sampler_smem(m->vout), st>>>(s->logits, m->vout, 1, s->g_uniforms, B, s->g_min, s->g_max, s->g_out_ids,
                                                                       s->g_out_ld, s->g_out_count, s->g_done, s->ctx_len, s->base_len, s->live,
                                                                       m->speech_emb, s->x, nullptr, 0, nullptr, nullptr, nullptr, fused ? m->layers[0].ln1 : nullptr,
                                                                       fused ? (bf16*)s->xn : nullptr, nullptr, nullptr);
  ctx->launches++;
  CVK_LAUNCH_CHECK();
  for (int li = 0; li < m->num_layers; ++li) layer_forward(ctx, st, m, li, x, xn, qkv, att, gu, ffa, nullptr, s, true);
  CVK_CHECK_CUDA(cudaMemcpyAsync(s->hidden, s->x, sizeof(float) * (size_t)B * D, cudaMemcpyDeviceToDevice, st));
}

void llm_decode(cvk_ctx* ctx, cvk_lm_session* s, int n_steps, const float* uniforms, const int32_t* min_len, const int32_t* max_len,
                int32_t* out_ids, int out_ld, int32_t* out_count, int32_t* done, int* live_host, cudaStream_t st) {
  const LlmModel* m = ctx->llm;
  CVK_REQUIRE(m && s->B > 0, "cvk_lm_prefill must run before cvk_lm_decode");
  const int B = s->B;
  s->ragged = false;
  const bool was_fresh = s->fresh;
  if (s->fresh) {
    CVK_CHECK_CUDA(cudaMemsetAsync(out_count, 0, sizeof(int32_t) * B, st));
    CVK_CHECK_CUDA(cudaMemsetAsync(done, 0, sizeof(int32_t) * B, st));
    s->fresh = false;
  }
  bool same = s->g_out_count == out_count && s->g_done == done && s->g_out_ids == out_ids && s->g_uniforms == uniforms &&
              s->g_min == min_len && s->g_max == max_len && s->g_out_ld == out_ld && s->g_B == B && s->g_pdl == ctx->pdl &&
              s->g_mega == ctx->lm_mega;
  if (!same) {
    if (s->graph) {
      cudaGraphExecDestroy(s->graph);
      s->graph = nullptr;
    }
    s->g_out_count = out_count; s->g_done = done; s->g_out_ids = out_ids; s->g_uniforms = uniforms; s->g_min = min_len; s->g_max = max_len;
    s->g_out_ld = out_ld; s->g_B = B; s->g_pdl = ctx->pdl; s->g_mega = ctx->lm_mega;
  }
  s->g_B = B;
  if (was_fresh && lm_fused_path(ctx, s)) {
    Mat hid(s->hidden, DT_F32, B, D, D), xn(s->xn, DT_BF16, B, D, D);
    rmsnorm(ctx, st, hid, m->final_norm, RMS_EPS, xn);
  }
  const bool can_graph = ctx->use_graph && st != nullptr && st != cudaStreamLegacy && st != cudaStreamPerThread;
  if (can_graph && !s->graph) {
    cudaGraph_t graph = nullptr;
    CVK_CHECK_CUDA(cudaStreamBeginCapture(st, cudaStreamCaptureModeThreadLocal));
    cvk_in_capture = 1;
    try {
      decode_step(ctx, st, s);
      cvk_in_capture = 0;
    } catch (...) {
      cvk_in_capture = 0;
      cudaStreamEndCapture(st, &graph);
      if (graph) cudaGraphDestroy(graph);
      throw;
    }
    CVK_CHECK_CUDA(cudaStreamEndCapture(st, &graph));
    size_t n_nodes = 0;
    CVK_CHECK_CUDA(cudaGraphGetNodes(graph, nullptr, &n_nodes));
    std::vector<cudaGraphNode_t> nodes(n_nodes);
    if (n_nodes) CVK_CHECK_CUDA(cudaGraphGetNodes(graph, nodes.data(), &n_nodes));
    int64_t kernels = 0;
    for (cudaGraphNode_t n : nodes) {
      cudaGraphNodeType t;
      CVK_CHECK_CUDA(cudaGraphNodeGetType(n, &t));
      kernels += t == cudaGraphNodeTypeKernel;
    }
    CVK_CHECK_CUDA(cudaGraphInstantiate(&s->graph, graph, 0));
    cudaGraphDestroy(graph);
    s->graph_kernels = kernels;
    ctx->launches -= kernels;
  }
  for (int i = 0; i < n_steps; ++i) {
    if (can_graph && s->graph) {
      CVK_CHECK_CUDA(cudaGraphLaunch(s->graph, st));
      ctx->launches += s->graph_kernels;
    } else {
      decode_step(ctx, st, s);
    }
  }
  if (live_host) {
    CVK_CHECK_CUDA(cudaMemcpyAsync(live_host, s->live, sizeof(int), cudaMemcpyDeviceToHost, st));
    CVK_CHECK_CUDA(cudaStreamSynchronize(st));
  }
}

void llm_decode_layers_op(cvk_ctx* ctx, int B, const int* ctx_len_host, int max_ctx, float* x, float* k_cache, float* v_cache,
                          float* xn_out, float* att_out, float* ffa_out, cudaStream_t st) {
  const LlmModel* m = ctx->llm;
  ctx->arena.reset();
  cvk_lm_session* s = llm_session_create(ctx, B, max_ctx);
  try {
    s->B = s->g_B = B;
    const int cache_rows = m->num_layers * B * NKV * max_ctx;
    Mat k32(k_cache, DT_F32, cache_rows, HD, HD), v32(v_cache, DT_F32, cache_rows, HD, HD);
    Mat kc(s->kcache, DT_BF16, cache_rows, HD, HD), vc(s->vcache, DT_BF16, cache_rows, HD, HD);
    Mat xs(s->x, DT_F32, B, D, D), xn(s->xn, DT_BF16, B, D, D), att(s->att, DT_BF16, B, D, D), ffa(s->ffa, DT_BF16, B, DFF, DFF);
    CVK_CHECK_CUDA(cudaMemcpyAsync(s->ctx_len, ctx_len_host, sizeof(int) * B, cudaMemcpyHostToDevice, st));
    CVK_CHECK_CUDA(cudaMemcpyAsync(s->x, x, sizeof(float) * (size_t)B * D, cudaMemcpyDeviceToDevice, st));
    convert_mat(ctx, st, k32, kc);
    convert_mat(ctx, st, v32, vc);
    if (lm_fused_path(ctx, s)) {
      launch_ex(finish_rms_kernel, dim3(B), dim3(D), 0, st, ctx->pdl != 0, (const float*)s->scratch, 0, B, s->x, (const float*)m->layers[0].ln1,
                xn.b16(), (long long*)nullptr);
      ctx->launches++;
      CVK_LAUNCH_CHECK();
      decode_layers_fused(ctx, st, s);
    } else {
      Mat qkv(s->qkv, DT_BF16, B, QKV_N, QKV_N), gu(s->gu, DT_BF16, B, 2 * DFF, 2 * DFF);
      for (int li = 0; li < m->num_layers; ++li) layer_forward(ctx, st, m, li, xs, xn, qkv, att, gu, ffa, nullptr, s, true);
      rmsnorm(ctx, st, xs, m->final_norm, RMS_EPS, xn);
    }
    CVK_CHECK_CUDA(cudaMemcpyAsync(x, s->x, sizeof(float) * (size_t)B * D, cudaMemcpyDeviceToDevice, st));
    convert_mat(ctx, st, kc, k32);
    convert_mat(ctx, st, vc, v32);
    convert_mat(ctx, st, xn, Mat(xn_out, DT_F32, B, D, D));
    if (att_out) convert_mat(ctx, st, att, Mat(att_out, DT_F32, B, D, D));
    if (ffa_out) convert_mat(ctx, st, ffa, Mat(ffa_out, DT_F32, B, DFF, DFF));
    CVK_CHECK_CUDA(cudaStreamSynchronize(st));
  } catch (...) {
    cudaStreamSynchronize(st);
    llm_session_destroy(ctx, s);
    throw;
  }
  llm_session_destroy(ctx, s);
}

namespace {
__global__ void feed_embed_kernel(int kind, int id, int B, const float* __restrict__ text_emb, const float* __restrict__ llm_emb,
                                  const float* __restrict__ speech_emb, float* __restrict__ x) {
  const float* src = kind == 0 ? text_emb + (size_t)id * D : (kind == 1 ? speech_emb + (size_t)id * D : llm_emb + (size_t)id * D);
  for (int b = 0; b < B; ++b)
    for (int c = threadIdx.x; c < D; c += blockDim.x) x[(size_t)b * D + c] = src[c];
}
__global__ void bump_ctx_kernel(int* __restrict__ ctx_len, int B) {
  if (threadIdx.x < B) ctx_len[threadIdx.x] += 1;
}
__global__ void zero_state_kernel(int* ctx_len, int* base_len, int* live, int n, int B) {
  if (threadIdx.x < n) {
    ctx_len[threadIdx.x] = 0;
    base_len[threadIdx.x] = 0;
  }
  if (threadIdx.x == 0) *live = B;
}
}

void llm_session_begin(cvk_ctx* ctx, cvk_lm_session* s, int B, cudaStream_t st) {
  CVK_REQUIRE(ctx->llm, "llm stage not finalised");
  CVK_REQUIRE(B >= 1 && B <= s->max_batch && s->max_batch <= 1024, "cvk_lm_begin: bad batch");
  if (s->graph) {
    cudaGraphExecDestroy(s->graph);
    s->graph = nullptr;
  }
  zero_state_kernel<<<1, round_up(s->max_batch, 32), 0, st>>>(s->ctx_len, s->base_len, s->live, s->max_batch, B);
  CVK_CHECK_CUDA(cudaMemsetAsync(s->hidden, 0, sizeof(float) * (size_t)s->max_batch * D, st));
  ctx->launches++;
  CVK_LAUNCH_CHECK();
  s->B = B;
  s->fresh = true;
  s->fed = 0;
  s->ragged = true;
  s->rows_fed.assign(s->max_batch, 0);
}

void llm_feed(cvk_ctx* ctx, cvk_lm_session* s, const int32_t* ids, const int32_t* kinds, int n, cudaStream_t st) {
  const LlmModel* m = ctx->llm;
  CVK_REQUIRE(m && s->B > 0, "cvk_lm_begin or cvk_lm_prefill must run before cvk_lm_feed");
  CVK_REQUIRE(s->fed + n < s->max_ctx, "cvk_lm_feed: session context exhausted");
  const int adt = s->kv_dtype, B = s->B;
  Mat x(s->x, DT_F32, B, D, D), xn(s->xn, adt, B, D, D), qkv(s->qkv, adt, B, QKV_N, QKV_N), att(s->att, adt, B, D, D),
      gu(s->gu, adt, B, 2 * DFF, 2 * DFF), ffa(s->ffa, adt, B, DFF, DFF);
  for (int i = 0; i < n; ++i) {
    const int kind = kinds[i], id = ids[i];
    CVK_REQUIRE((kind == 0 && id >= 0 && id < 151936) || (kind == 1 && id >= 0 && id < m->vout) || (kind == 2 && id >= 0 && id < 2),
                "cvk_lm_feed: id out of range");
    feed_embed_kernel<<<1, 256, 0, st>>>(kind, id, B, m->text_emb, m->llm_emb, m->speech_emb, s->x);
    for (int li = 0; li < m->num_layers; ++li) layer_forward(ctx, st, m, li, x, xn, qkv, att, gu, ffa, nullptr, s, true);
    bump_ctx_kernel<<<1, round_up(B, 32), 0, st>>>(s->ctx_len, B);
    ctx->launches += 2;
    CVK_LAUNCH_CHECK();
  }
  CVK_CHECK_CUDA(cudaMemcpyAsync(s->hidden, s->x, sizeof(float) * (size_t)B * D, cudaMemcpyDeviceToDevice, st));
  s->fed += n;
  for (int b = 0; b < B; ++b) s->rows_fed[b] += n;
  s->fresh = false;
}

void llm_next_logp(cvk_ctx* ctx, cvk_lm_session* s, float* logp, cudaStream_t st) {
  const LlmModel* m = ctx->llm;
  CVK_REQUIRE(m && s->B > 0 && s->fed > 0, "cvk_lm_feed must run before cvk_lm_next_logp");
  const int B = s->B;
  Mat hid(s->hidden, DT_F32, B, D, D), xn(s->xn, s->kv_dtype, B, D, D), logits(s->logits, DT_F32, B, m->vout, m->vout);
  head_logits(ctx, st, m, hid, xn, logits, s);
  logsoftmax_rows_kernel<<<B, SAMPLER_THREADS, 0, st>>>(s->logits, m->vout);
  ctx->launches++;
  CVK_LAUNCH_CHECK();
  CVK_CHECK_CUDA(cudaMemcpyAsync(logp, s->logits, sizeof(float) * (size_t)B * m->vout, cudaMemcpyDeviceToDevice, st));
}

static constexpr int FEED_CAP = 256;

static void feed_buffers(cvk_lm_session* s) {
  if (s->feed_cap) return;
  const size_t es = s->kv_dtype == DT_F32 ? 4 : 2, cap = FEED_CAP;
  auto alloc = [&](size_t bytes) {
    void* p = nullptr;
    CVK_CHECK_CUDA(cudaMalloc(&p, bytes));
    s->owned.push_back(p);
    return p;
  };
  s->fx = (float*)alloc(sizeof(float) * cap * D);
  s->fxn = alloc(es * cap * D);
  s->fqkv = alloc(es * cap * QKV_N);
  s->fatt = alloc(es * cap * D);
  s->fgu = alloc(es * cap * 2 * DFF);
  s->fffa = alloc(es * cap * DFF);
  s->fidx = (int*)alloc(sizeof(int) * (8 * cap + 3 * (size_t)s->max_batch));
  s->fscratch_floats = skinny_scratch_floats(64, D);
  s->fscratch = (float*)alloc(s->fscratch_floats * sizeof(float));
  s->feed_cap = FEED_CAP;
}

static void check_id(const LlmModel* m, int kind, int id, const char* what) {
  CVK_REQUIRE((kind == 0 && id >= 0 && id < 151936) || (kind == 1 && id >= 0 && id < m->vout) || (kind == 2 && id >= 0 && id < 2), what);
}

void llm_feed_rows(cvk_ctx* ctx, cvk_lm_session* s, int n_rows, const int* rows, const int* counts, const int32_t* ids, const int32_t* kinds,
                   cudaStream_t st) {
  const LlmModel* m = ctx->llm;
  CVK_REQUIRE(m && s->B > 0 && s->ragged, "cvk_lm_begin must run before cvk_lm_feed_rows");
  CVK_REQUIRE(n_rows >= 1 && n_rows <= s->B, "cvk_lm_feed_rows: row count out of range");
  std::vector<char> seen(s->B, 0);
  int64_t total = 0;
  for (int r = 0; r < n_rows; ++r) {
    const int b = rows[r];
    CVK_REQUIRE(b >= 0 && b < s->B && !seen[b], "cvk_lm_feed_rows: duplicate or out-of-range row");
    seen[b] = 1;
    CVK_REQUIRE(counts[r] >= 1 && (int64_t)s->rows_fed[b] + counts[r] <= s->max_ctx, "cvk_lm_feed_rows: row context exhausted");
    total += counts[r];
  }
  for (int64_t i = 0; i < total; ++i) check_id(m, kinds[i], ids[i], "cvk_lm_feed_rows: id or kind out of range");
  feed_buffers(s);
  const int adt = s->kv_dtype, cap = s->feed_cap;
  std::vector<int> h((size_t)8 * cap + 3 * (size_t)s->max_batch);
  int* h_ids = h.data();
  int* h_kinds = h_ids + cap;
  int* h_rowpos = h_kinds + cap;
  int* h_tiles = h_rowpos + 2 * cap;
  int* h_sc = h_tiles + 4 * cap;
  const int2* d_rowpos = reinterpret_cast<const int2*>(s->fidx + 2 * cap);
  const int4* d_tiles = reinterpret_cast<const int4*>(s->fidx + 4 * cap);
  const int* d_sc = s->fidx + 8 * cap;
  int r = 0, in_row = 0;
  int64_t off = 0;
  while (off < total) {
    const int M = (int)std::min<int64_t>(cap, total - off);
    int mm = 0, ntiles = 0, nsc = 0;
    while (mm < M) {
      const int b = rows[r], take = std::min(counts[r] - in_row, M - mm), pos = s->rows_fed[b];
      for (int k = 0; k < take; ++k) {
        h_ids[mm + k] = ids[off + mm + k];
        h_kinds[mm + k] = kinds[off + mm + k];
        h_rowpos[2 * (mm + k)] = b;
        h_rowpos[2 * (mm + k) + 1] = pos + k;
      }
      for (int k = 0; k < take; k += 2) {
        int* t = h_tiles + 4 * ntiles++;
        t[0] = mm + k; t[1] = b; t[2] = pos + k; t[3] = std::min(2, take - k);
      }
      h_sc[3 * nsc] = b; h_sc[3 * nsc + 1] = mm + take - 1; h_sc[3 * nsc + 2] = take;
      ++nsc;
      s->rows_fed[b] += take;
      mm += take;
      in_row += take;
      if (in_row == counts[r]) { ++r; in_row = 0; }
    }
    CVK_CHECK_CUDA(cudaMemcpyAsync(s->fidx, h.data(), h.size() * sizeof(int), cudaMemcpyHostToDevice, st));
    Mat x(s->fx, DT_F32, M, D, D), xn(s->fxn, adt, M, D, D), qkv(s->fqkv, adt, M, QKV_N, QKV_N), att(s->fatt, adt, M, D, D),
        gu(s->fgu, adt, M, 2 * DFF, 2 * DFF), ffa(s->fffa, adt, M, DFF, DFF);
    ragged_embed_kernel<<<M, 128, 0, st>>>(s->fidx, s->fidx + cap, m->text_emb, m->llm_emb, m->speech_emb, s->fx);
    ctx->launches++;
    CVK_LAUNCH_CHECK();
    RaggedPass rg;
    rg.rowpos = d_rowpos;
    rg.tiles = d_tiles;
    rg.ntiles = ntiles;
    for (int li = 0; li < m->num_layers; ++li) layer_forward(ctx, st, m, li, x, xn, qkv, att, gu, ffa, nullptr, s, true, &rg);
    feed_scatter_kernel<<<nsc, 128, 0, st>>>(d_sc, s->fx, s->hidden, s->ctx_len);
    ctx->launches++;
    CVK_LAUNCH_CHECK();
    off += M;
  }
  s->fed = std::max(s->fed, *std::max_element(s->rows_fed.begin(), s->rows_fed.begin() + s->B));
  s->fresh = false;
}

void llm_next_logp_rows(cvk_ctx* ctx, cvk_lm_session* s, int n_rows, const int* rows, float* logp, cudaStream_t st) {
  const LlmModel* m = ctx->llm;
  CVK_REQUIRE(m && s->B > 0 && s->ragged, "cvk_lm_begin must run before cvk_lm_next_logp_rows");
  CVK_REQUIRE(n_rows >= 1 && n_rows <= s->B, "cvk_lm_next_logp_rows: row count out of range");
  std::vector<char> seen(s->B, 0);
  for (int r = 0; r < n_rows; ++r) {
    const int b = rows[r];
    CVK_REQUIRE(b >= 0 && b < s->B && !seen[b], "cvk_lm_next_logp_rows: duplicate or out-of-range row");
    CVK_REQUIRE(s->rows_fed[b] > 0, "cvk_lm_next_logp_rows: row has no fed position");
    seen[b] = 1;
  }
  CVK_CHECK_CUDA(cudaMemcpyAsync(s->sel, rows, sizeof(int) * n_rows, cudaMemcpyHostToDevice, st));
  gather_rows_kernel<<<n_rows, 128, 0, st>>>(s->sel, s->hidden, s->x);
  ctx->launches++;
  CVK_LAUNCH_CHECK();
  Mat hid(s->x, DT_F32, n_rows, D, D), xn(s->xn, s->kv_dtype, n_rows, D, D), logits(s->logits, DT_F32, n_rows, m->vout, m->vout);
  rmsnorm(ctx, st, hid, m->final_norm, RMS_EPS, xn);
  Epilogue e;
  e.out = logits;
  lm_gemm_rows(ctx, st, xn, m->head, e, s->scratch, s->scratch_floats);
  logsoftmax_rows_kernel<<<n_rows, SAMPLER_THREADS, 0, st>>>(s->logits, m->vout);
  ctx->launches++;
  CVK_LAUNCH_CHECK();
  CVK_CHECK_CUDA(cudaMemcpyAsync(logp, s->logits, sizeof(float) * (size_t)n_rows * m->vout, cudaMemcpyDeviceToDevice, st));
}

int llm_vocab(cvk_ctx* ctx) { return ctx->llm ? ctx->llm->vout : 0; }

void llm_last_logits(cvk_ctx* ctx, cvk_lm_session* s, float* logits, cudaStream_t st) {
  CVK_REQUIRE(s->B > 0 && s->logits, "cvk_lm_last_logits: no decode step has run");
  CVK_REQUIRE(ctx->llm, "llm stage not finalised");
  CVK_CHECK_CUDA(cudaMemcpyAsync(logits, s->logits, sizeof(float) * (size_t)s->B * ctx->llm->vout, cudaMemcpyDeviceToDevice, st));
}

void llm_forward_logp(cvk_ctx* ctx, const float* embeds, const int* lens, int B, float* logp, cudaStream_t st) {
  const LlmModel* m = ctx->llm;
  CVK_REQUIRE(m, "llm stage not finalised");
  ctx->arena.reset();
  Seqs s = make_seqs(ctx, lens, B, 0, 1, 0, st);
  Mat x = arena_mat(ctx, DT_F32, s.R, D, D);
  zero_mat(ctx, st, x);
  pack_rows(ctx, st, embeds, D, s, x);
  forward_packed(ctx, st, s, x, nullptr);
  Mat xn = arena_mat(ctx, ctx->act_dtype, s.R, D), logits = arena_mat(ctx, DT_F32, s.R, m->vout, m->vout);
  head_logits(ctx, st, m, x, xn, logits);
  logsoftmax_rows_kernel<<<s.R, SAMPLER_THREADS, 0, st>>>(logits.f32(), m->vout);
  ctx->launches++;
  CVK_LAUNCH_CHECK();
  unpack_rows(ctx, st, logits, s, 0, logp, m->vout);
}

void llm_ras_sample(cvk_ctx* ctx, float* logp, int B, int V, const int32_t* history, int hist_ld, const int32_t* hist_count,
                    const float* uniforms, const int32_t* ignore_eos, int32_t* out_ids, cudaStream_t st) {
  CVK_REQUIRE(V > EOS + 2 && V <= SAMPLER_PER * SAMPLER_THREADS, "vocabulary size out of range (6564 .. 6912 supported)");
  CVK_CHECK_CUDA(cudaFuncSetAttribute(ras_sampler_kernel, cudaFuncAttributeMaxDynamicSharedMemorySize,
                                      (int)sampler_smem(V > VOUT3_PAD ? V : VOUT3_PAD)));
  ras_sampler_kernel<<<B, SAMPLER_THREADS, sampler_smem(V), st>>>(logp, V, 0, uniforms, B, nullptr, nullptr, nullptr, 0, nullptr, nullptr, nullptr,
                                                                    nullptr, nullptr, nullptr, nullptr, history, hist_ld, hist_count, ignore_eos,
                                                                    out_ids, nullptr, nullptr, nullptr, nullptr);
  ctx->launches++;
  CVK_LAUNCH_CHECK();
}

void llm_sample_step_op(cvk_ctx* ctx, float* logits, int B, int V, const float* uniforms, const int32_t* min_len, const int32_t* max_len,
                        int32_t* out_ids, int out_ld, int32_t* out_count, int32_t* done, int* ctx_len, const int* base_len, int* live,
                        const float* speech_emb, float* next_x, const float* gamma, float* xn, cudaStream_t st) {
  CVK_CHECK_CUDA(cudaFuncSetAttribute(ras_sampler_kernel, cudaFuncAttributeMaxDynamicSharedMemorySize,
                                      (int)sampler_smem(V > VOUT3_PAD ? V : VOUT3_PAD)));
  ctx->arena.reset();
  Mat xn16;
  if (gamma) {
    xn16 = arena_mat(ctx, DT_BF16, B, D, D);
    convert_mat(ctx, st, Mat(xn, DT_F32, B, D, D), xn16);
  }
  ras_sampler_kernel<<<B, SAMPLER_THREADS, sampler_smem(V), st>>>(logits, V, 1, uniforms, B, min_len, max_len, out_ids, out_ld, out_count,
                                                                    done, ctx_len, base_len, live, speech_emb, next_x, nullptr, 0, nullptr,
                                                                    nullptr, nullptr, gamma, gamma ? xn16.b16() : nullptr, nullptr, nullptr);
  ctx->launches++;
  CVK_LAUNCH_CHECK();
  if (gamma) convert_mat(ctx, st, xn16, Mat(xn, DT_F32, B, D, D));
}

void llm_log_softmax_op(cvk_ctx* ctx, float* x, int rows, int V, cudaStream_t st) {
  logsoftmax_rows_kernel<<<rows, SAMPLER_THREADS, 0, st>>>(x, V);
  ctx->launches++;
  CVK_LAUNCH_CHECK();
}
```

cosyvoice_b200/csrc/llm_decode_attn.cuh:

```cuda
#pragma once
#include "llm_internal.h"

namespace lm {

__device__ __forceinline__ uint32_t pack_bf16x2(float lo, float hi) {
  __nv_bfloat162 h2 = __floats2bfloat162_rn(lo, hi);
  return *reinterpret_cast<uint32_t*>(&h2);
}
__device__ __forceinline__ void mma_16816(float* c, uint32_t a0, uint32_t a2, uint32_t b0, uint32_t b1) {
  asm volatile("mma.sync.aligned.m16n8k16.row.col.f32.bf16.bf16.f32 {%0,%1,%2,%3}, {%4,%5,%6,%7}, {%8,%9}, {%0,%1,%2,%3};"
               : "+f"(c[0]), "+f"(c[1]), "+f"(c[2]), "+f"(c[3])
               : "r"(a0), "r"(0u), "r"(a2), "r"(0u), "r"(b0), "r"(b1));
}
template <int BAR_ID, int NTHREADS>
__device__ __forceinline__ void attn_bar() {
  if (BAR_ID == 0) __syncthreads();
  else asm volatile("bar.sync %0, %1;" ::"n"(BAR_ID), "n"(NTHREADS) : "memory");
}

template <int NW>
__host__ __device__ constexpr int decode_attn_smem_floats() { return (NH / NKV + 2) * HD + NW * 8 * 2 + NW * (NH / NKV) * HD; }

struct KvFrag {
  uint32_t kf[2][4][2], vw[4][4];
};
__device__ __forceinline__ void decode_attn_load_block(const bf16* __restrict__ kb, const bf16* __restrict__ vb, int j0, int L, int lane, KvFrag& f) {
  const int g = lane >> 2, t4 = lane & 3;
#pragma unroll
  for (int nt = 0; nt < 2; ++nt) {
    const uint32_t* kr = reinterpret_cast<const uint32_t*>(kb + (size_t)min(j0 + nt * 8 + g, L - 1) * HD);
#pragma unroll
    for (int kk = 0; kk < 4; ++kk) {
      f.kf[nt][kk][0] = kr[kk * 8 + t4];
      f.kf[nt][kk][1] = kr[kk * 8 + 4 + t4];
    }
  }
  const uint32_t* v0 = reinterpret_cast<const uint32_t*>(vb + (size_t)min(j0 + t4 * 2, L - 1) * HD);
  const uint32_t* v1 = reinterpret_cast<const uint32_t*>(vb + (size_t)min(j0 + t4 * 2 + 1, L - 1) * HD);
  const uint32_t* v2 = reinterpret_cast<const uint32_t*>(vb + (size_t)min(j0 + 8 + t4 * 2, L - 1) * HD);
  const uint32_t* v3 = reinterpret_cast<const uint32_t*>(vb + (size_t)min(j0 + 9 + t4 * 2, L - 1) * HD);
#pragma unroll
  for (int q = 0; q < 4; ++q) {
    f.vw[q][0] = v0[q * 8 + g];
    f.vw[q][1] = v1[q * 8 + g];
    f.vw[q][2] = v2[q * 8 + g];
    f.vw[q][3] = v3[q * 8 + g];
  }
}

template <int NW, int BAR_ID, int SPLITS = 0>
__device__ __forceinline__ void decode_attn_unit(float* __restrict__ sm_all, int tid, const float* __restrict__ partial, int splits, int rows,
                                                 int b, int kvh, const float* __restrict__ bias, bf16* __restrict__ kb, bf16* __restrict__ vb,
                                                 int pos, int max_ctx, const float* __restrict__ inv_freq, bf16* __restrict__ out_row,
                                                 KvFrag& fr ,
                                                 bool have_pre) {
  constexpr int G = NH / NKV;
  constexpr int NT = NW * 32;
  const int warp = tid >> 5, lane = tid & 31;
  float* stage = sm_all;
  float* ml = stage + (G + 2) * HD;
  float* po = ml + NW * 8 * 2;
  if (SPLITS > 0) {
    constexpr int PER = ((G + 2) * HD + NT - 1) / NT;
    constexpr int S = SPLITS > 0 ? SPLITS : 1;
    float ld[PER][S], bs[PER];
    const size_t stride = (size_t)rows * QKV_N;
#pragma unroll
    for (int i = 0; i < PER; ++i) {
      const int e = tid + i * NT;
      const bool ok = e < (G + 2) * HD;
      const int vec = ok ? e / HD : 0, d = e % HD;
      const int col = vec < G ? (kvh * G + vec) * HD + d : (vec == G ? NH * HD + kvh * HD + d : NH * HD + NKV * HD + kvh * HD + d);
      const float* p = partial + (size_t)b * QKV_N + col;
      bs[i] = bias[col];
#pragma unroll
      for (int s2 = 0; s2 < S; ++s2) ld[i][s2] = ok ? __ldcg(p + (size_t)s2 * stride) : 0.f;
    }
#pragma unroll
    for (int i = 0; i < PER; ++i) {
      const int e = tid + i * NT;
      float a = bs[i];
#pragma unroll
      for (int s2 = 0; s2 < S; ++s2) a += ld[i][s2];
      if (e < (G + 2) * HD) stage[e] = a;
    }
  } else {
    for (int e = tid; e < (G + 2) * HD; e += NT) {
      const int vec = e / HD, d = e % HD;
      const int col = vec < G ? (kvh * G + vec) * HD + d : (vec == G ? NH * HD + kvh * HD + d : NH * HD + NKV * HD + kvh * HD + d);
      const float* p = partial + (size_t)b * QKV_N + col;
      const size_t stride = (size_t)rows * QKV_N;
      float a0 = bias[col], a1 = 0.f, a2 = 0.f, a3 = 0.f;
      int s = 0;
      for (; s + 4 <= splits; s += 4) {
        a0 += p[(size_t)s * stride];
        a1 += p[(size_t)(s + 1) * stride];
        a2 += p[(size_t)(s + 2) * stride];
        a3 += p[(size_t)(s + 3) * stride];
      }
      for (; s < splits; ++s) a0 += p[(size_t)s * stride];
      stage[e] = (a0 + a1) + (a2 + a3);
    }
  }
  attn_bar<BAR_ID, NT>();
  for (int e = tid; e < (G + 1) * (HD / 2); e += NT) {
    const int vec = e / (HD / 2), i = e % (HD / 2);
    const float fr = (float)pos * inv_freq[i];
    const float c = cosf(fr), sn = sinf(fr);
    float* p = stage + vec * HD;
    const float x1 = p[i], x2 = p[i + HD / 2];
    p[i] = x1 * c - x2 * sn;
    p[i + HD / 2] = x2 * c + x1 * sn;
  }
  attn_bar<BAR_ID, NT>();
  if (pos < max_ctx && tid < 2 * HD) {
    const int d = tid % HD;
    if (tid < HD) kb[(size_t)pos * HD + d] = __float2bfloat16_rn(stage[G * HD + d]);
    else vb[(size_t)pos * HD + d] = __float2bfloat16_rn(stage[(G + 1) * HD + d]);
  }
  attn_bar<BAR_ID, NT>();
  const int L = min(pos + 1, max_ctx);
  const int g = lane >> 2, t4 = lane & 3;
  uint32_t qa[4][2];
#pragma unroll
  for (int kk = 0; kk < 4; ++kk)
#pragma unroll
    for (int hv = 0; hv < 2; ++hv) {
      const int d = kk * 16 + hv * 8 + t4 * 2;
      qa[kk][hv] = g < G ? pack_bf16x2(__bfloat162float(__float2bfloat16_rn(stage[g * HD + d])) * 0.125f,
                                       __bfloat162float(__float2bfloat16_rn(stage[g * HD + d + 1])) * 0.125f)
                         : 0u;
    }
  float o[4][2][4];
#pragma unroll
  for (int q = 0; q < 4; ++q)
#pragma unroll
    for (int t = 0; t < 2; ++t)
#pragma unroll
      for (int e = 0; e < 4; ++e) o[q][t][e] = 0.f;
  float m_run = -INFINITY, l_run = 0.f;
  for (int j0 = warp * 16; j0 < L; j0 += NW * 16) {
    if (!(have_pre && j0 == warp * 16)) decode_attn_load_block(kb, vb, j0, L, lane, fr);
    uint32_t (&kf)[2][4][2] = fr.kf;
    uint32_t (&vw)[4][4] = fr.vw;
    float s0[4] = {0.f, 0.f, 0.f, 0.f}, s1[4] = {0.f, 0.f, 0.f, 0.f};
#pragma unroll
    for (int kk = 0; kk < 4; ++kk) {
      mma_16816(s0, qa[kk][0], qa[kk][1], kf[0][kk][0], kf[0][kk][1]);
      mma_16816(s1, qa[kk][0], qa[kk][1], kf[1][kk][0], kf[1][kk][1]);
    }
    const int ka = j0 + t4 * 2;
    const bool va0 = ka < L, va1 = ka + 1 < L, vb0 = ka + 8 < L, vb1 = ka + 9 < L;
    float mx = fmaxf(fmaxf(va0 ? s0[0] : -INFINITY, va1 ? s0[1] : -INFINITY), fmaxf(vb0 ? s1[0] : -INFINITY, vb1 ? s1[1] : -INFINITY));
    mx = fmaxf(mx, __shfl_xor_sync(0xffffffffu, mx, 1));
    mx = fmaxf(mx, __shfl_xor_sync(0xffffffffu, mx, 2));
    const float m_new = fmaxf(m_run, mx);
    const float corr = __expf(m_run - m_new);
    const float p0 = va0 ? __expf(s0[0] - m_new) : 0.f, p1 = va1 ? __expf(s0[1] - m_new) : 0.f;
    const float p2 = vb0 ? __expf(s1[0] - m_new) : 0.f, p3 = vb1 ? __expf(s1[1] - m_new) : 0.f;
    l_run = l_run * corr + ((p0 + p1) + (p2 + p3));
    m_run = m_new;
    const uint32_t pa0 = pack_bf16x2(p0, p1), pa2 = pack_bf16x2(p2, p3);
#pragma unroll
    for (int q = 0; q < 4; ++q) {
      o[q][0][0] *= corr; o[q][0][1] *= corr;
      o[q][1][0] *= corr; o[q][1][1] *= corr;
      mma_16816(o[q][0], pa0, pa2, __byte_perm(vw[q][0], vw[q][1], 0x5410), __byte_perm(vw[q][2], vw[q][3], 0x5410));
      mma_16816(o[q][1], pa0, pa2, __byte_perm(vw[q][0], vw[q][1], 0x7632), __byte_perm(vw[q][2], vw[q][3], 0x7632));
    }
  }
  l_run += __shfl_xor_sync(0xffffffffu, l_run, 1);
  l_run += __shfl_xor_sync(0xffffffffu, l_run, 2);
  if (g < G) {
    if (t4 == 0) {
      ml[(warp * 8 + g) * 2] = m_run;
      ml[(warp * 8 + g) * 2 + 1] = l_run;
    }
#pragma unroll
    for (int q = 0; q < 4; ++q)
      *reinterpret_cast<float4*>(po + ((size_t)warp * G + g) * HD + q * 16 + t4 * 4) = make_float4(o[q][0][0], o[q][1][0], o[q][0][1], o[q][1][1]);
  }
  attn_bar<BAR_ID, NT>();
  for (int e = tid; e < G * HD; e += NT) {
    const int hq = e / HD, d = e % HD;
    float M = -INFINITY;
#pragma unroll
    for (int w2 = 0; w2 < NW; ++w2) M = fmaxf(M, ml[(w2 * 8 + hq) * 2]);
    float num = 0.f, den = 0.f;
#pragma unroll
    for (int w2 = 0; w2 < NW; ++w2) {
      const float wgt = __expf(ml[(w2 * 8 + hq) * 2] - M);
      den = fmaf(wgt, ml[(w2 * 8 + hq) * 2 + 1], den);
      num = fmaf(wgt, po[((size_t)w2 * G + hq) * HD + d], num);
    }
    out_row[(kvh * G + hq) * HD + d] = __float2bfloat16_rn(num / den);
  }
}

}
```

cosyvoice_b200/csrc/llm_mega.cu:

```cuda
#include "llm_decode_attn.cuh"
#include "wgmma.cuh"
#include "tma.cuh"
#include <algorithm>
#include <type_traits>

using namespace lm;

namespace {

constexpr int MG_THREADS = 512;
constexpr int MG_WORKERS = MG_THREADS - 32;
constexpr int MG_NW = MG_WORKERS / 32;
constexpr int MG_BK = 64;
constexpr int MG_MAXROWS = 80;
constexpr uint32_t MG_SLOT = MG_MAXROWS * 128;
constexpr int MG_MAX_STAGES = 16;
constexpr int MG_INFLIGHT = 3;
constexpr int MG_KCH = D / MG_BK;
constexpr int MG_PH = 4;
constexpr int MG_MAX_LAYERS = 32;
constexpr int MG_TILE = 64;
constexpr int MG_CPU_QKV = 2, MG_CPU_O = 2;
constexpr int MG_SPL_QKV = MG_KCH / MG_CPU_QKV;
constexpr int MG_SPL_O = MG_KCH / MG_CPU_O;
constexpr int MG_SPL_DOWN = 9;

struct MegaUnit { int row0, nrows, kc0, nblk, split; };
struct MegaLayerDev { const float* qkv_bias; const float* ln2; const float* next_gamma; };

struct MegaParams {
  const uint8_t* wstream;
  const unsigned long long* cta_off;
  const MegaUnit* units;
  const MegaLayerDev* layers;
  int num_layers, B, max_ctx;
  float* x; bf16* xn; bf16* att; bf16* ffa;
  float *part_qkv, *part_o, *part_down;
  bf16 *kcache, *vcache;
  unsigned long long kv_layer_stride;
  const int* ctx_len;
  const float* inv_freq;
  unsigned* bar;
  long long* tl;
};

__device__ __forceinline__ void worker_bar() { asm volatile("bar.sync 1, %0;" ::"n"(MG_WORKERS) : "memory"); }
__device__ __forceinline__ void epi_bar() { asm volatile("bar.sync 2, 256;" ::: "memory"); }
__device__ __forceinline__ unsigned ld_acquire(const unsigned* p) {
  unsigned v;
  asm volatile("ld.acquire.gpu.global.u32 %0, [%1];" : "=r"(v) : "l"(p) : "memory");
  return v;
}
__device__ __forceinline__ void red_release_add(unsigned* p, unsigned v) {
  asm volatile("red.release.gpu.global.add.u32 [%0], %1;" ::"l"(p), "r"(v) : "memory");
}
__device__ __forceinline__ void prefetch_l2(const void* p) { asm volatile("prefetch.global.L2 [%0];" ::"l"(p)); }
__device__ __forceinline__ long long gtime() {
  long long t;
  asm volatile("mov.u64 %0, %globaltimer;" : "=l"(t));
  return t;
}

template <int BPAD>
__global__ void __launch_bounds__(MG_THREADS, 1)
lm_mega_kernel(const MegaParams p) {
  constexpr int NST = BPAD == 32 ? 16 : 10;
  constexpr uint32_t ACT_CHUNK = BPAD * 128;
  constexpr int STG_LD = 40;
  static_assert(decode_attn_smem_floats<MG_NW>() * 4 <= MG_KCH * ACT_CHUNK, "attention scratch must fit the activation buffer");
  static_assert(BPAD * STG_LD * 2 <= MG_KCH * ACT_CHUNK, "SwiGLU staging must fit the activation buffer");
  extern __shared__ uint8_t smem_raw[];
  __shared__ __align__(8) uint64_t bar_full[MG_MAX_STAGES];
  __shared__ __align__(8) uint64_t bar_empty[MG_MAX_STAGES];
  __shared__ float red[16];
  __shared__ MegaUnit s_units[MG_PH];
  __shared__ MegaLayerDev s_layers[MG_MAX_LAYERS];

  const uint32_t sbase = (smem_u32(smem_raw) + 1023u) & ~1023u;
  uint8_t* sptr = smem_raw + (sbase - smem_u32(smem_raw));
  const uint32_t ring = sbase, act = sbase + NST * MG_SLOT;
  uint8_t* act_ptr = sptr + NST * MG_SLOT;
  float* attn_sm = reinterpret_cast<float*>(act_ptr);
  const int warp = threadIdx.x >> 5, lane = threadIdx.x & 31;
  const int cta = blockIdx.x, G = gridDim.x;
  const int B = p.B;

  if (threadIdx.x == 0) {
    for (int s = 0; s < NST; ++s) {
      mbar_init(smem_u32(&bar_full[s]), 1);
      mbar_init(smem_u32(&bar_empty[s]), 8);
    }
    asm volatile("fence.mbarrier_init.release.cluster;" ::: "memory");
  }
  if (threadIdx.x >= 64 && threadIdx.x < 64 + MG_PH) s_units[threadIdx.x - 64] = p.units[(threadIdx.x - 64) * G + cta];
  if (threadIdx.x >= 128 && threadIdx.x < 128 + p.num_layers) s_layers[threadIdx.x - 128] = p.layers[threadIdx.x - 128];
  __syncthreads();

  if (warp == 0) {
    if (lane == 0) {
      const uint8_t* src = p.wstream + p.cta_off[cta];
      int it = 0;
      for (int l = 0; l < p.num_layers; ++l)
        for (int ph = 0; ph < MG_PH; ++ph) {
          const int nblk = s_units[ph].nblk;
          const uint32_t bytes = (uint32_t)s_units[ph].nrows * 128u;
          for (int j = 0; j < nblk; ++j, ++it) {
            const int s = it % NST;
            if (it >= NST) mbar_wait(smem_u32(&bar_empty[s]), ((uint32_t)(it / NST) & 1u) ^ 1u);
            if (it >= MG_INFLIGHT) {
              const int itp = it - MG_INFLIGHT;
              mbar_wait(smem_u32(&bar_full[itp % NST]), (uint32_t)(itp / NST) & 1u);
            }
            const uint32_t fb = smem_u32(&bar_full[s]);
            mbar_expect_tx(fb, bytes);
            bulk_load(ring + s * MG_SLOT, src, bytes, fb);
            src += bytes;
          }
        }
    }
    __syncwarp();
  } else {
    const int wt = threadIdx.x - 32;
    const int ww = warp - 1;
    unsigned bar_target = __ldcg(p.bar + 1);
    const unsigned gen0 = bar_target;
    int mma_it = 0, tl_i = 0;
    const bool stamp = p.tl != nullptr && cta == 0 && wt == 0;
    if (stamp) p.tl[tl_i++] = gtime();
    int fs_i = 0;
    bool fs_on = false;
    long long* fs = p.tl ? p.tl + (cta == 0 ? 512 : 768) : nullptr;
    const bool fs_cta = p.tl != nullptr && (cta == 0 || cta == 100) && wt == 0;
#define FS() do { if (fs_cta && fs_on && fs_i < 250) fs[fs_i++] = gtime(); } while (0)

    auto grid_sync = [&]() {
      bar_target += (unsigned)G;
      FS();
      worker_bar();
      if (wt == 0) {
        red_release_add(p.bar, 1u);
        FS();
        const long long t0 = clock64();
        while ((int)(ld_acquire(p.bar) - bar_target) < 0) {
          if (clock64() - t0 > 4000000000ll) __trap();
        }
        if (stamp) p.tl[tl_i++] = gtime();
        FS();
      }
      worker_bar();
    };

    auto gemm_phase = [&](int ph, const bf16* actg, int K, float* out_f32, int N, int mode) {
      const MegaUnit u = s_units[ph];
      if (u.nblk <= 0) return;
      {
        const int items = u.nblk * B * 8;
        constexpr int UN = 4;
        for (int i0 = wt; i0 < items; i0 += MG_WORKERS * UN) {
          uint4 v[UN];
#pragma unroll
          for (int q = 0; q < UN; ++q) {
            const int i = i0 + q * MG_WORKERS;
            if (i < items) {
              const int c = i & 7, b = (i >> 3) % B, j = (i >> 3) / B;
              v[q] = __ldcg(reinterpret_cast<const uint4*>(actg + (size_t)b * K + (size_t)(u.kc0 + j) * MG_BK) + c);
            }
          }
#pragma unroll
          for (int q = 0; q < UN; ++q) {
            const int i = i0 + q * MG_WORKERS;
            if (i < items) {
              const int c = i & 7, b = (i >> 3) % B, j = (i >> 3) / B;
              *reinterpret_cast<uint4*>(act_ptr + j * ACT_CHUNK + b * 128 + ((c ^ (b & 7)) << 4)) = v[q];
            }
          }
        }
        asm volatile("fence.proxy.async.shared::cta;" ::: "memory");
        worker_bar();
        FS();
      }
      if (warp >= 4 && warp < 12) {
        const int wg = (warp - 4) >> 2, q = lane & 3;
        const bool active = wg * 64 < u.nrows;
        float acc[BPAD / 2];
#pragma unroll
        for (int e = 0; e < BPAD / 2; ++e) acc[e] = 0.f;
        for (int j = 0; j < u.nblk; ++j) {
          const int it = mma_it + j;
          const int s = it % NST;
          mbar_wait(smem_u32(&bar_full[s]), (uint32_t)(it / NST) & 1u);
          if (active) {
            const uint64_t da = wg_desc_sw128(ring + s * MG_SLOT + (uint32_t)wg * 8192u), db = wg_desc_sw128(act + j * ACT_CHUNK);
            wg_fence();
#pragma unroll
            for (int k = 0; k < MG_BK / 16; ++k) wgmma_ss<BPAD, 0>(acc, da + (uint64_t)(2 * k), db + (uint64_t)(2 * k), 1);
            wg_commit();
            wg_wait<0>();
          }
          __syncwarp();
          if (lane == 0) mbar_arrive(smem_u32(&bar_empty[s]));
        }
        wg_touch<BPAD / 2>(acc);
        bf16* stage = reinterpret_cast<bf16*>(act_ptr);
        if (mode == 1) epi_bar();
        if (active) {
#pragma unroll
          for (int e = 0; e < BPAD / 2; ++e) {
            const int r = wg * 64 + (warp & 3) * 16 + (lane >> 2) + 8 * ((e >> 1) & 1);
            const int b = 8 * (e >> 2) + 2 * q + (e & 1);
            if (mode == 1) {
              const float other = __shfl_xor_sync(0xffffffffu, acc[e], 4);
              if (!((lane >> 2) & 1) && r < u.nrows && b < B) {
                const float g = acc[e];
                stage[b * STG_LD + (r >> 1)] = __float2bfloat16_rn(__fdividef(g, 1.f + fast_exp(-g)) * other);
              }
            } else if (r < u.nrows && b < B) {
              out_f32[((size_t)u.split * B + b) * N + u.row0 + r] = acc[e];
            }
          }
        }
        if (mode == 1) {
          epi_bar();
          const int nq = u.nrows >> 3;
          const int ch0 = u.row0 >> 1;
          for (int i = threadIdx.x - 128; i < B * nq; i += 256) {
            const int b = i / nq, c4 = i % nq;
            *reinterpret_cast<uint2*>(p.ffa + (size_t)b * DFF + ch0 + c4 * 4) = *reinterpret_cast<const uint2*>(stage + b * STG_LD + c4 * 4);
          }
        }
      }
      mma_it += u.nblk;
    };

    auto reduce_norm = [&](const float* part, auto splits_tag, const float* gamma) {
      constexpr int S = decltype(splits_tag)::value;
      for (int b = cta; b < B; b += G) {
        float ld[2][S + 1];
#pragma unroll
        for (int h = 0; h < 2; ++h) {
          const int n = wt + h * MG_WORKERS;
          const bool ok = n < D;
          ld[h][0] = ok ? __ldcg(p.x + (size_t)b * D + n) : 0.f;
#pragma unroll
          for (int s = 0; s < S; ++s) ld[h][s + 1] = ok ? __ldcg(part + ((size_t)s * B + b) * D + n) : 0.f;
        }
        float v[2], ss = 0.f;
#pragma unroll
        for (int h = 0; h < 2; ++h) {
          float a = 0.f;
#pragma unroll
          for (int s = 0; s < S; ++s) a += ld[h][s + 1];
          v[h] = ld[h][0] + a;
          const int n = wt + h * MG_WORKERS;
          if (n < D) {
            p.x[(size_t)b * D + n] = v[h];
            ss += v[h] * v[h];
          }
        }
        ss = warp_sum(ss);
        if (lane == 0) red[ww] = ss;
        FS();
        worker_bar();
        float tot = 0.f;
#pragma unroll
        for (int i = 0; i < MG_NW; ++i) tot += red[i];
        const float r = rsqrtf(tot / D + RMS_EPS);
#pragma unroll
        for (int h = 0; h < 2; ++h) {
          const int n = wt + h * MG_WORKERS;
          if (n < D) p.xn[(size_t)b * D + n] = __float2bfloat16_rn(gamma[n] * (v[h] * r));
        }
        worker_bar();
      }
    };

    for (int l = 0; l < p.num_layers; ++l) {
      const MegaLayerDev Lw = s_layers[l];
      fs_on = l == 1;
      bf16* kc_l = p.kcache + (size_t)l * p.kv_layer_stride;
      bf16* vc_l = p.vcache + (size_t)l * p.kv_layer_stride;
      if (cta < B * NKV && warp >= 8) {
        const int b = cta / NKV, kvh = cta % NKV;
        const int L = min(p.ctx_len[b], p.max_ctx);
        const bf16* kb = kc_l + ((size_t)b * NKV + kvh) * p.max_ctx * HD;
        const bf16* vb = vc_l + ((size_t)b * NKV + kvh) * p.max_ctx * HD;
        for (int j = threadIdx.x - 256; j < L; j += MG_THREADS - 256) {
          prefetch_l2(kb + (size_t)j * HD);
          prefetch_l2(vb + (size_t)j * HD);
        }
      }
      gemm_phase(0, p.xn, D, p.part_qkv, QKV_N, 0);
      grid_sync();
      for (int u = cta; u < B * NKV; u += G) {
        const int b = u / NKV, kvh = u % NKV;
        bf16* kb = kc_l + ((size_t)b * NKV + kvh) * p.max_ctx * HD;
        bf16* vb = vc_l + ((size_t)b * NKV + kvh) * p.max_ctx * HD;
        KvFrag fr;
        decode_attn_unit<MG_NW, 1, MG_SPL_QKV>(attn_sm, wt, p.part_qkv, MG_SPL_QKV, B, b, kvh, Lw.qkv_bias, kb, vb, p.ctx_len[b], p.max_ctx,
                                               p.inv_freq, p.att + (size_t)b * D, fr, false);
        worker_bar();
      }
      grid_sync();
      gemm_phase(1, p.att, D, p.part_o, D, 0);
      grid_sync();
      reduce_norm(p.part_o, std::integral_constant<int, MG_SPL_O>(), Lw.ln2);
      grid_sync();
      gemm_phase(2, p.xn, D, nullptr, 2 * DFF, 1);
      grid_sync();
      gemm_phase(3, p.ffa, DFF, p.part_down, D, 0);
      grid_sync();
      reduce_norm(p.part_down, std::integral_constant<int, MG_SPL_DOWN>(), Lw.next_gamma);
      if (l + 1 < p.num_layers) grid_sync();
    }
    if (cta == 0 && wt == 0) {
      p.bar[1] = gen0 + (unsigned)G * (unsigned)(7 * p.num_layers - 1);
      if (stamp) p.tl[tl_i++] = gtime();
    }
  }
}

struct PackDesc { const bf16* w; int K, row0, nrows, kc; unsigned long long dst; };
__global__ void pack_blocks_kernel(const PackDesc* __restrict__ descs, int n, uint8_t* __restrict__ out) {
  for (int i = blockIdx.x; i < n; i += gridDim.x) {
    const PackDesc d = descs[i];
    for (int e = threadIdx.x; e < d.nrows * 8; e += blockDim.x) {
      const int r = e >> 3, c = e & 7;
      const uint4 v = *reinterpret_cast<const uint4*>(d.w + (size_t)(d.row0 + r) * d.K + (size_t)d.kc * MG_BK + c * 8);
      *reinterpret_cast<uint4*>(out + d.dst + r * 128 + ((c ^ (r & 7)) << 4)) = v;
    }
  }
}

template <int BPAD> constexpr size_t mega_smem() { return (size_t)(BPAD == 32 ? 16 : 10) * MG_SLOT + (size_t)MG_KCH * BPAD * 128 + 1024; }

}

struct LmMega {
  int G = 0;
  int splits[MG_PH] = {0, 0, 0, 0};
  uint8_t* wstream = nullptr;
  unsigned long long* cta_off = nullptr;
  MegaUnit* units = nullptr;
  MegaLayerDev* layers = nullptr;
  size_t stream_bytes = 0;
};

struct MegaSession {
  float *part_qkv = nullptr, *part_o = nullptr, *part_down = nullptr;
  unsigned* bar = nullptr;
};

void lm_mega_build(cvk_ctx* ctx, LlmModel* m) {
  const int G = ctx->num_sms, L = m->num_layers;
  if (L > MG_MAX_LAYERS) return;
  std::vector<MegaUnit> units((size_t)MG_PH * G, MegaUnit{0, 0, 0, 0, 0});
  auto put = [&](int ph, int c, MegaUnit u) {
    c = ((c % G) + G) % G;
    CVK_REQUIRE(units[(size_t)ph * G + c].nblk == 0, "lm mega: two units on one CTA in a phase");
    units[(size_t)ph * G + c] = u;
  };
  const int qkv_tiles = QKV_N / MG_TILE, o_tiles = D / MG_TILE, down_chunks = DFF / MG_BK;
  if (qkv_tiles * MG_SPL_QKV > G || o_tiles * MG_SPL_O > G || o_tiles * MG_SPL_DOWN > G) return;
  for (int t = 0; t < qkv_tiles; ++t)
    for (int s = 0; s < MG_SPL_QKV; ++s) put(0, t * MG_SPL_QKV + s, MegaUnit{t * MG_TILE, MG_TILE, s * MG_CPU_QKV, MG_CPU_QKV, s});
  for (int t = 0; t < o_tiles; ++t)
    for (int s = 0; s < MG_SPL_O; ++s) put(1, G - o_tiles * MG_SPL_O + t * MG_SPL_O + s, MegaUnit{t * MG_TILE, MG_TILE, s * MG_CPU_O, MG_CPU_O, s});
  {
    const int groups = 2 * DFF / 8, base = groups / G, extra = groups % G;
    if ((base + (extra ? 1 : 0)) * 8 > MG_MAXROWS || base < 1) return;
    int row = 0;
    for (int c = 0; c < G; ++c) {
      const int nr = (base + (c < extra ? 1 : 0)) * 8;
      put(2, c, MegaUnit{row, nr, 0, MG_KCH, 0});
      row += nr;
    }
  }
  {
    const int base = down_chunks / MG_SPL_DOWN, extra = down_chunks % MG_SPL_DOWN;
    for (int t = 0; t < o_tiles; ++t) {
      int kc = 0;
      for (int s = 0; s < MG_SPL_DOWN; ++s) {
        const int nb = base + (s < extra ? 1 : 0);
        put(3, t * MG_SPL_DOWN + s, MegaUnit{t * MG_TILE, MG_TILE, kc, nb, s});
        kc += nb;
      }
    }
  }
  LmMega* mg = new LmMega();
  mg->G = G;
  mg->splits[0] = MG_SPL_QKV; mg->splits[1] = MG_SPL_O; mg->splits[2] = 1; mg->splits[3] = MG_SPL_DOWN;
  std::vector<unsigned> lbytes(G, 0);
  std::vector<unsigned long long> off(G, 0);
  size_t total = 0;
  for (int c = 0; c < G; ++c) {
    for (int ph = 0; ph < MG_PH; ++ph) lbytes[c] += (unsigned)(units[(size_t)ph * G + c].nblk * units[(size_t)ph * G + c].nrows * 128);
    off[c] = total;
    total += (size_t)lbytes[c] * L;
  }
  mg->stream_bytes = total;
  mg->wstream = (uint8_t*)ctx->dmalloc(total);
  std::vector<PackDesc> descs;
  for (int c = 0; c < G; ++c)
    for (int l = 0; l < L; ++l) {
      const LayerW& w = m->layers[l];
      const ConvW* Ws[MG_PH] = {&w.qkv, &w.o, &w.gate_up_il, &w.down};
      unsigned long long dst = off[c] + (unsigned long long)l * lbytes[c];
      for (int ph = 0; ph < MG_PH; ++ph) {
        const MegaUnit& u = units[(size_t)ph * G + c];
        CVK_REQUIRE(u.nblk == 0 || (Ws[ph]->w16 && u.row0 + u.nrows <= Ws[ph]->N && (u.kc0 + u.nblk) * MG_BK <= Ws[ph]->K), "lm mega: unit outside its weight");
        for (int j = 0; j < u.nblk; ++j) {
          descs.push_back(PackDesc{Ws[ph]->w16, Ws[ph]->K, u.row0, u.nrows, u.kc0 + j, dst});
          dst += (unsigned long long)u.nrows * 128;
        }
      }
    }
  {
    PackDesc* dd = nullptr;
    CVK_CHECK_CUDA(cudaMalloc((void**)&dd, descs.size() * sizeof(PackDesc)));
    CVK_CHECK_CUDA(cudaMemcpy(dd, descs.data(), descs.size() * sizeof(PackDesc), cudaMemcpyHostToDevice));
    pack_blocks_kernel<<<G * 8, 256>>>(dd, (int)descs.size(), mg->wstream);
    CVK_LAUNCH_CHECK();
    CVK_CHECK_CUDA(cudaDeviceSynchronize());
    cudaFree(dd);
  }
  std::vector<MegaLayerDev> lay(L);
  for (int l = 0; l < L; ++l) {
    lay[l].qkv_bias = m->layers[l].qkv.bias;
    lay[l].ln2 = m->layers[l].ln2;
    lay[l].next_gamma = l + 1 < L ? m->layers[l + 1].ln1 : m->final_norm;
  }
  auto up = [&](const void* h, size_t bytes) {
    void* d = ctx->dmalloc(bytes);
    CVK_CHECK_CUDA(cudaMemcpy(d, h, bytes, cudaMemcpyHostToDevice));
    return d;
  };
  mg->cta_off = (unsigned long long*)up(off.data(), off.size() * sizeof(unsigned long long));
  mg->units = (MegaUnit*)up(units.data(), units.size() * sizeof(MegaUnit));
  mg->layers = (MegaLayerDev*)up(lay.data(), lay.size() * sizeof(MegaLayerDev));
  CVK_CHECK_CUDA(cudaFuncSetAttribute(lm_mega_kernel<32>, cudaFuncAttributeMaxDynamicSharedMemorySize, (int)mega_smem<32>()));
  CVK_CHECK_CUDA(cudaFuncSetAttribute(lm_mega_kernel<64>, cudaFuncAttributeMaxDynamicSharedMemorySize, (int)mega_smem<64>()));
  m->mega = mg;
}

bool lm_mega_usable(cvk_ctx* ctx, const cvk_lm_session* s, int B) {
  return ctx->lm_mega && ctx->llm && ctx->llm->mega && s->kv_dtype == DT_BF16 && ctx->use_tc && B >= 1 && B <= 64 && s->mega_state;
}

void lm_mega_session_init(cvk_ctx* ctx, cvk_lm_session* s) {
  const LmMega* mg = ctx->llm ? ctx->llm->mega : nullptr;
  if (!mg || s->kv_dtype != DT_BF16 || s->max_batch > 64) return;
  MegaSession* ms = new MegaSession();
  auto alloc = [&](size_t bytes) {
    void* p = nullptr;
    CVK_CHECK_CUDA(cudaMalloc(&p, bytes));
    CVK_CHECK_CUDA(cudaMemset(p, 0, bytes));
    s->owned.push_back(p);
    return p;
  };
  ms->part_qkv = (float*)alloc((size_t)mg->splits[0] * s->max_batch * QKV_N * sizeof(float));
  ms->part_o = (float*)alloc((size_t)mg->splits[1] * s->max_batch * D * sizeof(float));
  ms->part_down = (float*)alloc((size_t)mg->splits[3] * s->max_batch * D * sizeof(float));
  ms->bar = (unsigned*)alloc(64);
  s->mega_state = ms;
}

void lm_mega_session_free(cvk_lm_session* s) {
  delete (MegaSession*)s->mega_state;
  s->mega_state = nullptr;
}

void lm_mega_layers(cvk_ctx* ctx, cudaStream_t st, cvk_lm_session* s, int B) {
  const LlmModel* m = ctx->llm;
  const LmMega* mg = m->mega;
  const MegaSession* ms = (const MegaSession*)s->mega_state;
  CVK_REQUIRE(mg && ms && B >= 1 && B <= 64 && m->num_layers <= MG_MAX_LAYERS, "lm mega: not initialised");
  const int bpad = B <= 32 ? 32 : 64;
  MegaParams p;
  p.wstream = mg->wstream; p.cta_off = mg->cta_off; p.units = mg->units; p.layers = mg->layers;
  p.num_layers = m->num_layers; p.B = B; p.max_ctx = s->max_ctx;
  p.x = s->x; p.xn = (bf16*)s->xn; p.att = (bf16*)s->att; p.ffa = (bf16*)s->ffa;
  p.part_qkv = ms->part_qkv; p.part_o = ms->part_o; p.part_down = ms->part_down;
  p.kcache = (bf16*)s->kcache; p.vcache = (bf16*)s->vcache;
  p.kv_layer_stride = (unsigned long long)s->max_batch * NKV * s->max_ctx * HD;
  p.ctx_len = s->ctx_len; p.inv_freq = m->d_inv_freq;
  p.bar = ms->bar;
  p.tl = ctx->tl ? (long long*)ctx->tl + 2048 : nullptr;
  cudaLaunchConfig_t cfg = {};
  cfg.gridDim = dim3(mg->G);
  cfg.blockDim = dim3(MG_THREADS);
  cfg.dynamicSmemBytes = bpad == 32 ? mega_smem<32>() : mega_smem<64>();
  cfg.stream = st;
  cudaLaunchAttribute at[1];
  at[0].id = cudaLaunchAttributeCooperative;
  at[0].val.cooperative = 1;
  cfg.attrs = at;
  cfg.numAttrs = ctx->mega_coop ? 1 : 0;
  if (bpad == 32) CVK_CHECK_CUDA(cudaLaunchKernelEx(&cfg, lm_mega_kernel<32>, p));
  else CVK_CHECK_CUDA(cudaLaunchKernelEx(&cfg, lm_mega_kernel<64>, p));
  ctx->launches++;
}
```

Before: 430.5.

## Replace mega-kernel grid barriers with per-CTA dependency waits and rebalance skinny GEMM

```diff
diff --git a/cosyvoice_b200/csrc/cvk_internal.h b/cosyvoice_b200/csrc/cvk_internal.h
--- a/cosyvoice_b200/csrc/cvk_internal.h
+++ b/cosyvoice_b200/csrc/cvk_internal.h
@@ -237,6 +237,8 @@
 void flow_ff(cvk_ctx* ctx, cudaStream_t st, const Mat& x, const int* row2seq, const float* ln3_g, const float* ln3_b, const ConvW& ff1,
              const ConvW& ff2, const float* ln_g, const float* ln_b, const Mat& out, const Mat& xn, const Mat& hid);
 size_t skinny_scratch_floats(int rows, int maxN);
+struct SkinnySplit { int splits, cps; };
+SkinnySplit skinny_split(int num_sms, int N, int K);
 const bf16* skinny_tiled_weights(cvk_ctx* ctx, const ConvW& W);
 int conv_gemm_skinny_ex(cvk_ctx* ctx, cudaStream_t st, const Mat& A, const ConvW& W, const Epilogue& ep, float* scratch, size_t scratch_floats,
                         int mode);
diff --git a/cosyvoice_b200/csrc/gemm_skinny.cu b/cosyvoice_b200/csrc/gemm_skinny.cu
--- a/cosyvoice_b200/csrc/gemm_skinny.cu
+++ b/cosyvoice_b200/csrc/gemm_skinny.cu
@@ -5,9 +5,10 @@
 namespace {
 
 constexpr int SK_BM = 128;
+constexpr int SK_CM = 64;
 constexpr int SK_BK = 64;
-constexpr int SK_STAGES = 8;
-constexpr int SK_THREADS = 384;
+constexpr int SK_THREADS = 256;
+template <int BPAD> constexpr int sk_stages() { return BPAD == 32 ? 8 : 6; }
 
 __global__ void tile_weights_kernel(const bf16* __restrict__ w, bf16* __restrict__ out, int N, int K, int tiles, int kchunks) {
   size_t total = (size_t)tiles * kchunks * SK_BM * 8;
@@ -29,23 +30,25 @@
 }
 
 template <int BPAD>
-__global__ void __launch_bounds__(SK_THREADS, 1)
+__global__ void __launch_bounds__(SK_THREADS, 2)
 skinny_gemm_kernel(const bf16* __restrict__ w_tiled, const __grid_constant__ CUtensorMap tmap_x, int N, int K, int rows,
                    int chunks_per_split, float* __restrict__ partial , EpiDev ep, int swiglu,
                    long long* __restrict__ tl) {
   extern __shared__ uint8_t smem_raw[];
   pdl_trigger();
   tl_stamp(tl, 0);
+  constexpr int SK_STAGES = sk_stages<BPAD>();
   __shared__ __align__(8) uint64_t bar_full[SK_STAGES];
   __shared__ __align__(8) uint64_t bar_empty[SK_STAGES];
-  constexpr uint32_t A_BYTES = SK_BM * SK_BK * 2;
+  constexpr uint32_t A_BYTES = SK_CM * SK_BK * 2;
   constexpr uint32_t B_BYTES = BPAD * SK_BK * 2;
   constexpr uint32_t STAGE = A_BYTES + B_BYTES;
 
   const uint32_t base = (smem_u32(smem_raw) + 1023u) & ~1023u;
   const int warp = threadIdx.x >> 5, lane = threadIdx.x & 31;
-  const int n0 = blockIdx.x * SK_BM;
+  const int n0 = blockIdx.x * SK_CM;
   const int kchunks = (K + SK_BK - 1) / SK_BK;
+  const bf16* w_half = w_tiled + (size_t)(blockIdx.x >> 1) * kchunks * (SK_BM * SK_BK) + (blockIdx.x & 1) * (SK_CM * SK_BK);
   const int kc0 = blockIdx.y * chunks_per_split;
   const int kc1 = min(kchunks, kc0 + chunks_per_split);
   const int iters = kc1 - kc0;
@@ -53,7 +56,7 @@
   if (threadIdx.x == 0) {
     for (int s = 0; s < SK_STAGES; ++s) {
       mbar_init(smem_u32(&bar_full[s]), 1);
-      mbar_init(smem_u32(&bar_empty[s]), 8);
+      mbar_init(smem_u32(&bar_empty[s]), 4);
     }
     asm volatile("fence.mbarrier_init.release.cluster;" ::: "memory");
   }
@@ -65,7 +68,7 @@
       for (int it = 0; it < pre; ++it) {
         const uint32_t fb = smem_u32(&bar_full[it]);
         mbar_expect_tx(fb, STAGE);
-        bulk_load(base + it * STAGE, w_tiled + ((size_t)blockIdx.x * kchunks + (kc0 + it)) * (SK_BM * SK_BK), A_BYTES, fb);
+        bulk_load(base + it * STAGE, w_half + (size_t)(kc0 + it) * (SK_BM * SK_BK), A_BYTES, fb);
       }
       pdl_wait();
       tl_stamp(tl, 1);
@@ -77,16 +80,15 @@
         const uint32_t sa = base + s * STAGE, sb = sa + A_BYTES;
         const uint32_t fb = smem_u32(&bar_full[s]);
         mbar_expect_tx(fb, STAGE);
-        bulk_load(sa, w_tiled + ((size_t)blockIdx.x * kchunks + (kc0 + it)) * (SK_BM * SK_BK), A_BYTES, fb);
+        bulk_load(sa, w_half + (size_t)(kc0 + it) * (SK_BM * SK_BK), A_BYTES, fb);
         tma_load_2d(sb, &tmap_x, fb, (kc0 + it) * SK_BK, 0);
       }
     } else {
       pdl_wait();
     }
   } else {
-    const int wg = (threadIdx.x - 128) >> 7;
     const int q = lane & 3;
-    const int fr = wg * 64 + (warp & 3) * 16 + (lane >> 2);
+    const int fr = (warp & 3) * 16 + (lane >> 2);
     float bias_n[2];
 #pragma unroll
     for (int hh = 0; hh < 2; ++hh) bias_n[hh] = (!partial && !swiglu && ep.bias && n0 + fr + 8 * hh < N) ? ep.bias[n0 + fr + 8 * hh] : 0.f;
@@ -97,7 +99,7 @@
     for (int it = 0; it < iters; ++it) {
       const int s = it % SK_STAGES;
       mbar_wait(smem_u32(&bar_full[s]), (uint32_t)(it / SK_STAGES) & 1u);
-      const uint32_t sa = base + s * STAGE + (uint32_t)wg * (A_BYTES / 2), sb = base + s * STAGE + A_BYTES;
+      const uint32_t sa = base + s * STAGE, sb = base + s * STAGE + A_BYTES;
       const uint64_t da = wg_desc_sw128(sa), db = wg_desc_sw128(sb);
       wg_fence();
 #pragma unroll
@@ -145,7 +147,7 @@
 
 template <int BPAD>
 constexpr size_t skinny_smem() {
-  return (size_t)SK_STAGES * (SK_BM * SK_BK * 2 + BPAD * SK_BK * 2) + 1024;
+  return (size_t)sk_stages<BPAD>() * (SK_CM * SK_BK * 2 + BPAD * SK_BK * 2) + 1024;
 }
 
 template <int BPAD>
@@ -170,6 +172,16 @@
 }
 
 size_t skinny_scratch_floats(int rows, int maxN) { return (size_t)32 * rows * maxN; }
+
+SkinnySplit skinny_split(int num_sms, int N, int K) {
+  const int tiles = ceil_div(N, SK_BM), kchunks = ceil_div(K, SK_BK);
+  int splits = num_sms / tiles;
+  if (splits > kchunks / 4) splits = kchunks / 4;
+  if (splits > 32) splits = 32;
+  if (splits < 1) splits = 1;
+  const int cps = ceil_div(kchunks, splits);
+  return SkinnySplit{ceil_div(kchunks, cps), cps};
+}
 
 int conv_gemm_skinny_ex(cvk_ctx* ctx, cudaStream_t st, const Mat& A, const ConvW& W, const Epilogue& ep, float* scratch, size_t scratch_floats,
                         int mode) {
@@ -188,12 +200,8 @@
   }
   const int tiles = ceil_div(W.N, SK_BM);
   const int kchunks = ceil_div(W.K, SK_BK);
-  int splits = ctx->num_sms / tiles;
-  if (splits > kchunks / 4) splits = kchunks / 4;
-  if (splits > 32) splits = 32;
-  if (splits < 1) splits = 1;
-  int cps = ceil_div(kchunks, splits);
-  splits = ceil_div(kchunks, cps);
+  const SkinnySplit sp = skinny_split(ctx->num_sms, W.N, W.K);
+  int splits = sp.splits, cps = sp.cps;
   if (mode == 2 || (splits > 1 && (scratch == nullptr || (size_t)splits * rows * W.N > scratch_floats))) {
     splits = 1;
     cps = kchunks;
@@ -204,7 +212,7 @@
   const double flops = 2.0 * rows * (double)W.N * W.K;
   const double bytes = (double)W.N * W.K * 2 + (double)rows * W.K * 2 + (double)rows * W.N * 2;
   ProfScope ps(ctx, st, FAM_GEMM_TC, flops, bytes);
-  dim3 grid(tiles, splits);
+  dim3 grid(2 * tiles, splits);
   float* partial = (splits > 1 || mode == 1) ? scratch : nullptr;
   long long* tl = ctx->tl_next();
   if (BPAD == 32) launch<32>(st, grid, tw, tx, W, rows, cps, partial, e, mode == 2, ctx->pdl != 0, tl);
diff --git a/cosyvoice_b200/csrc/llm.cu b/cosyvoice_b200/csrc/llm.cu
--- a/cosyvoice_b200/csrc/llm.cu
+++ b/cosyvoice_b200/csrc/llm.cu
@@ -190,16 +190,14 @@
   tl_stamp(tl, 1);
   const float* p = partial + (size_t)b * D + n;
   const size_t stride = (size_t)rows * D;
-  float a0 = 0.f, a1 = 0.f, a2 = 0.f, a3 = 0.f;
-  int s = 0;
-  for (; s + 4 <= splits; s += 4) {
-    a0 += p[(size_t)s * stride];
-    a1 += p[(size_t)(s + 1) * stride];
-    a2 += p[(size_t)(s + 2) * stride];
-    a3 += p[(size_t)(s + 3) * stride];
-  }
-  for (; s < splits; ++s) a0 += p[(size_t)s * stride];
-  const float v = x[(size_t)b * D + n] + ((a0 + a1) + (a2 + a3));
+  float a[4] = {0.f, 0.f, 0.f, 0.f};
+  for (int s0 = 0; s0 < splits; s0 += 4) {
+    float ld[4];
+#pragma unroll
+    for (int q = 0; q < 4; ++q) ld[q] = s0 + q < splits ? p[(size_t)(s0 + q) * stride] : 0.f;
+    split_add(a, ld, s0, splits);
+  }
+  const float v = x[(size_t)b * D + n] + split_total(a);
   x[(size_t)b * D + n] = v;
   float ss = warp_sum(v * v);
   if ((n & 31) == 0) red[n >> 5] = ss;
diff --git a/cosyvoice_b200/csrc/llm_decode_attn.cuh b/cosyvoice_b200/csrc/llm_decode_attn.cuh
--- a/cosyvoice_b200/csrc/llm_decode_attn.cuh
+++ b/cosyvoice_b200/csrc/llm_decode_attn.cuh
@@ -48,59 +48,55 @@
   }
 }
 
-template <int NW, int BAR_ID, int SPLITS = 0>
+__device__ __forceinline__ void split_add(float (&a)[4], const float (&v)[4], int s0, int splits) {
+  const int whole = splits & ~3;
+#pragma unroll
+  for (int q = 0; q < 4; ++q) {
+    if (s0 + q < whole) a[q] += v[q];
+    else if (s0 + q < splits) a[0] += v[q];
+  }
+}
+__device__ __forceinline__ float split_total(const float (&a)[4]) { return (a[0] + a[1]) + (a[2] + a[3]); }
+
+template <int NW, int BAR_ID, int NWR = NW>
 __device__ __forceinline__ void decode_attn_unit(float* __restrict__ sm_all, int tid, const float* __restrict__ partial, int splits, int rows,
                                                  int b, int kvh, const float* __restrict__ bias, bf16* __restrict__ kb, bf16* __restrict__ vb,
                                                  int pos, int max_ctx, const float* __restrict__ inv_freq, bf16* __restrict__ out_row,
                                                  KvFrag& fr ,
                                                  bool have_pre) {
+  static_assert(NWR <= NW, "more warps than key partitions");
   constexpr int G = NH / NKV;
-  constexpr int NT = NW * 32;
+  constexpr int NT = NWR * 32;
   const int warp = tid >> 5, lane = tid & 31;
   float* stage = sm_all;
   float* ml = stage + (G + 2) * HD;
   float* po = ml + NW * 8 * 2;
-  if (SPLITS > 0) {
+  {
     constexpr int PER = ((G + 2) * HD + NT - 1) / NT;
-    constexpr int S = SPLITS > 0 ? SPLITS : 1;
-    float ld[PER][S], bs[PER];
+    float a[PER][4];
+    const float* src[PER];
     const size_t stride = (size_t)rows * QKV_N;
 #pragma unroll
     for (int i = 0; i < PER; ++i) {
       const int e = tid + i * NT;
-      const bool ok = e < (G + 2) * HD;
-      const int vec = ok ? e / HD : 0, d = e % HD;
+      const int vec = e < (G + 2) * HD ? e / HD : 0, d = e % HD;
       const int col = vec < G ? (kvh * G + vec) * HD + d : (vec == G ? NH * HD + kvh * HD + d : NH * HD + NKV * HD + kvh * HD + d);
-      const float* p = partial + (size_t)b * QKV_N + col;
-      bs[i] = bias[col];
+      src[i] = partial + (size_t)b * QKV_N + col;
+      a[i][0] = bias[col];
+      a[i][1] = a[i][2] = a[i][3] = 0.f;
+    }
+    for (int s0 = 0; s0 < splits; s0 += 4) {
+      float v[PER][4];
 #pragma unroll
-      for (int s2 = 0; s2 < S; ++s2) ld[i][s2] = ok ? __ldcg(p + (size_t)s2 * stride) : 0.f;
+      for (int i = 0; i < PER; ++i)
+#pragma unroll
+        for (int q = 0; q < 4; ++q) v[i][q] = tid + i * NT < (G + 2) * HD && s0 + q < splits ? __ldcg(src[i] + (size_t)(s0 + q) * stride) : 0.f;
+#pragma unroll
+      for (int i = 0; i < PER; ++i) split_add(a[i], v[i], s0, splits);
     }
 #pragma unroll
-    for (int i = 0; i < PER; ++i) {
-      const int e = tid + i * NT;
-      float a = bs[i];
-#pragma unroll
-      for (int s2 = 0; s2 < S; ++s2) a += ld[i][s2];
-      if (e < (G + 2) * HD) stage[e] = a;
-    }
-  } else {
-    for (int e = tid; e < (G + 2) * HD; e += NT) {
-      const int vec = e / HD, d = e % HD;
-      const int col = vec < G ? (kvh * G + vec) * HD + d : (vec == G ? NH * HD + kvh * HD + d : NH * HD + NKV * HD + kvh * HD + d);
-      const float* p = partial + (size_t)b * QKV_N + col;
-      const size_t stride = (size_t)rows * QKV_N;
-      float a0 = bias[col], a1 = 0.f, a2 = 0.f, a3 = 0.f;
-      int s = 0;
-      for (; s + 4 <= splits; s += 4) {
-        a0 += p[(size_t)s * stride];
-        a1 += p[(size_t)(s + 1) * stride];
-        a2 += p[(size_t)(s + 2) * stride];
-        a3 += p[(size_t)(s + 3) * stride];
-      }
-      for (; s < splits; ++s) a0 += p[(size_t)s * stride];
-      stage[e] = (a0 + a1) + (a2 + a3);
-    }
+    for (int i = 0; i < PER; ++i)
+      if (tid + i * NT < (G + 2) * HD) stage[tid + i * NT] = split_total(a[i]);
   }
   attn_bar<BAR_ID, NT>();
   for (int e = tid; e < (G + 1) * (HD / 2); e += NT) {
@@ -131,54 +127,56 @@
                                        __bfloat162float(__float2bfloat16_rn(stage[g * HD + d + 1])) * 0.125f)
                          : 0u;
     }
-  float o[4][2][4];
-#pragma unroll
-  for (int q = 0; q < 4; ++q)
-#pragma unroll
-    for (int t = 0; t < 2; ++t)
-#pragma unroll
-      for (int e = 0; e < 4; ++e) o[q][t][e] = 0.f;
-  float m_run = -INFINITY, l_run = 0.f;
-  for (int j0 = warp * 16; j0 < L; j0 += NW * 16) {
-    if (!(have_pre && j0 == warp * 16)) decode_attn_load_block(kb, vb, j0, L, lane, fr);
-    uint32_t (&kf)[2][4][2] = fr.kf;
-    uint32_t (&vw)[4][4] = fr.vw;
-    float s0[4] = {0.f, 0.f, 0.f, 0.f}, s1[4] = {0.f, 0.f, 0.f, 0.f};
-#pragma unroll
-    for (int kk = 0; kk < 4; ++kk) {
-      mma_16816(s0, qa[kk][0], qa[kk][1], kf[0][kk][0], kf[0][kk][1]);
-      mma_16816(s1, qa[kk][0], qa[kk][1], kf[1][kk][0], kf[1][kk][1]);
-    }
-    const int ka = j0 + t4 * 2;
-    const bool va0 = ka < L, va1 = ka + 1 < L, vb0 = ka + 8 < L, vb1 = ka + 9 < L;
-    float mx = fmaxf(fmaxf(va0 ? s0[0] : -INFINITY, va1 ? s0[1] : -INFINITY), fmaxf(vb0 ? s1[0] : -INFINITY, vb1 ? s1[1] : -INFINITY));
-    mx = fmaxf(mx, __shfl_xor_sync(0xffffffffu, mx, 1));
-    mx = fmaxf(mx, __shfl_xor_sync(0xffffffffu, mx, 2));
-    const float m_new = fmaxf(m_run, mx);
-    const float corr = __expf(m_run - m_new);
-    const float p0 = va0 ? __expf(s0[0] - m_new) : 0.f, p1 = va1 ? __expf(s0[1] - m_new) : 0.f;
-    const float p2 = vb0 ? __expf(s1[0] - m_new) : 0.f, p3 = vb1 ? __expf(s1[1] - m_new) : 0.f;
-    l_run = l_run * corr + ((p0 + p1) + (p2 + p3));
-    m_run = m_new;
-    const uint32_t pa0 = pack_bf16x2(p0, p1), pa2 = pack_bf16x2(p2, p3);
-#pragma unroll
-    for (int q = 0; q < 4; ++q) {
-      o[q][0][0] *= corr; o[q][0][1] *= corr;
-      o[q][1][0] *= corr; o[q][1][1] *= corr;
-      mma_16816(o[q][0], pa0, pa2, __byte_perm(vw[q][0], vw[q][1], 0x5410), __byte_perm(vw[q][2], vw[q][3], 0x5410));
-      mma_16816(o[q][1], pa0, pa2, __byte_perm(vw[q][0], vw[q][1], 0x7632), __byte_perm(vw[q][2], vw[q][3], 0x7632));
-    }
-  }
-  l_run += __shfl_xor_sync(0xffffffffu, l_run, 1);
-  l_run += __shfl_xor_sync(0xffffffffu, l_run, 2);
-  if (g < G) {
-    if (t4 == 0) {
-      ml[(warp * 8 + g) * 2] = m_run;
-      ml[(warp * 8 + g) * 2 + 1] = l_run;
-    }
+  for (int vw = warp; vw < NW; vw += NWR) {
+    float o[4][2][4];
 #pragma unroll
     for (int q = 0; q < 4; ++q)
-      *reinterpret_cast<float4*>(po + ((size_t)warp * G + g) * HD + q * 16 + t4 * 4) = make_float4(o[q][0][0], o[q][1][0], o[q][0][1], o[q][1][1]);
+#pragma unroll
+      for (int t = 0; t < 2; ++t)
+#pragma unroll
+        for (int e = 0; e < 4; ++e) o[q][t][e] = 0.f;
+    float m_run = -INFINITY, l_run = 0.f;
+    for (int j0 = vw * 16; j0 < L; j0 += NW * 16) {
+      if (!(have_pre && vw == warp && j0 == warp * 16)) decode_attn_load_block(kb, vb, j0, L, lane, fr);
+      uint32_t (&kf)[2][4][2] = fr.kf;
+      uint32_t (&vw)[4][4] = fr.vw;
+      float s0[4] = {0.f, 0.f, 0.f, 0.f}, s1[4] = {0.f, 0.f, 0.f, 0.f};
+#pragma unroll
+      for (int kk = 0; kk < 4; ++kk) {
+        mma_16816(s0, qa[kk][0], qa[kk][1], kf[0][kk][0], kf[0][kk][1]);
+        mma_16816(s1, qa[kk][0], qa[kk][1], kf[1][kk][0], kf[1][kk][1]);
+      }
+      const int ka = j0 + t4 * 2;
+      const bool va0 = ka < L, va1 = ka + 1 < L, vb0 = ka + 8 < L, vb1 = ka + 9 < L;
+      float mx = fmaxf(fmaxf(va0 ? s0[0] : -INFINITY, va1 ? s0[1] : -INFINITY), fmaxf(vb0 ? s1[0] : -INFINITY, vb1 ? s1[1] : -INFINITY));
+      mx = fmaxf(mx, __shfl_xor_sync(0xffffffffu, mx, 1));
+      mx = fmaxf(mx, __shfl_xor_sync(0xffffffffu, mx, 2));
+      const float m_new = fmaxf(m_run, mx);
+      const float corr = __expf(m_run - m_new);
+      const float p0 = va0 ? __expf(s0[0] - m_new) : 0.f, p1 = va1 ? __expf(s0[1] - m_new) : 0.f;
+      const float p2 = vb0 ? __expf(s1[0] - m_new) : 0.f, p3 = vb1 ? __expf(s1[1] - m_new) : 0.f;
+      l_run = l_run * corr + ((p0 + p1) + (p2 + p3));
+      m_run = m_new;
+      const uint32_t pa0 = pack_bf16x2(p0, p1), pa2 = pack_bf16x2(p2, p3);
+#pragma unroll
+      for (int q = 0; q < 4; ++q) {
+        o[q][0][0] *= corr; o[q][0][1] *= corr;
+        o[q][1][0] *= corr; o[q][1][1] *= corr;
+        mma_16816(o[q][0], pa0, pa2, __byte_perm(vw[q][0], vw[q][1], 0x5410), __byte_perm(vw[q][2], vw[q][3], 0x5410));
+        mma_16816(o[q][1], pa0, pa2, __byte_perm(vw[q][0], vw[q][1], 0x7632), __byte_perm(vw[q][2], vw[q][3], 0x7632));
+      }
+    }
+    l_run += __shfl_xor_sync(0xffffffffu, l_run, 1);
+    l_run += __shfl_xor_sync(0xffffffffu, l_run, 2);
+    if (g < G) {
+      if (t4 == 0) {
+        ml[(vw * 8 + g) * 2] = m_run;
+        ml[(vw * 8 + g) * 2 + 1] = l_run;
+      }
+#pragma unroll
+      for (int q = 0; q < 4; ++q)
+        *reinterpret_cast<float4*>(po + ((size_t)vw * G + g) * HD + q * 16 + t4 * 4) = make_float4(o[q][0][0], o[q][1][0], o[q][0][1], o[q][1][1]);
+    }
   }
   attn_bar<BAR_ID, NT>();
   for (int e = tid; e < G * HD; e += NT) {
diff --git a/cosyvoice_b200/csrc/llm_mega.cu b/cosyvoice_b200/csrc/llm_mega.cu
--- a/cosyvoice_b200/csrc/llm_mega.cu
+++ b/cosyvoice_b200/csrc/llm_mega.cu
@@ -11,6 +11,7 @@
 constexpr int MG_THREADS = 512;
 constexpr int MG_WORKERS = MG_THREADS - 32;
 constexpr int MG_NW = MG_WORKERS / 32;
+constexpr int MG_ATTN_NW = 16;
 constexpr int MG_BK = 64;
 constexpr int MG_MAXROWS = 80;
 constexpr uint32_t MG_SLOT = MG_MAXROWS * 128;
@@ -20,27 +21,33 @@
 constexpr int MG_PH = 4;
 constexpr int MG_MAX_LAYERS = 32;
 constexpr int MG_TILE = 64;
-constexpr int MG_CPU_QKV = 2, MG_CPU_O = 2;
-constexpr int MG_SPL_QKV = MG_KCH / MG_CPU_QKV;
-constexpr int MG_SPL_O = MG_KCH / MG_CPU_O;
-constexpr int MG_SPL_DOWN = 9;
+constexpr int MG_MAX_UNITS = 8;
+constexpr int MG_MASKW = 8;
+enum { P_QKV, P_ATTN, P_O, P_NORM1, P_GATE_UP, P_DOWN, P_NORM2, MG_NPHASE };
+enum { W_ATTN, W_NORM1, W_DOWN, W_NORM2, MG_NWAIT };
 
 struct MegaUnit { int row0, nrows, kc0, nblk, split; };
+struct MegaCta {
+  MegaUnit u[MG_MAX_UNITS];
+  int n[MG_PH];
+  unsigned wait[MG_NWAIT][MG_MASKW];
+};
 struct MegaLayerDev { const float* qkv_bias; const float* ln2; const float* next_gamma; };
 
 struct MegaParams {
   const uint8_t* wstream;
   const unsigned long long* cta_off;
-  const MegaUnit* units;
+  const MegaCta* ctas;
   const MegaLayerDev* layers;
   int num_layers, B, max_ctx;
+  int spl_qkv, spl_o, spl_down;
   float* x; bf16* xn; bf16* att; bf16* ffa;
   float *part_qkv, *part_o, *part_down;
   bf16 *kcache, *vcache;
   unsigned long long kv_layer_stride;
   const int* ctx_len;
   const float* inv_freq;
-  unsigned* bar;
+  unsigned* prog;
   long long* tl;
 };
 
@@ -51,8 +58,8 @@
   asm volatile("ld.acquire.gpu.global.u32 %0, [%1];" : "=r"(v) : "l"(p) : "memory");
   return v;
 }
-__device__ __forceinline__ void red_release_add(unsigned* p, unsigned v) {
-  asm volatile("red.release.gpu.global.add.u32 [%0], %1;" ::"l"(p), "r"(v) : "memory");
+__device__ __forceinline__ void st_release(unsigned* p, unsigned v) {
+  asm volatile("st.release.gpu.global.u32 [%0], %1;" ::"l"(p), "r"(v) : "memory");
 }
 __device__ __forceinline__ void prefetch_l2(const void* p) { asm volatile("prefetch.global.L2 [%0];" ::"l"(p)); }
 __device__ __forceinline__ long long gtime() {
@@ -67,13 +74,13 @@
   constexpr int NST = BPAD == 32 ? 16 : 10;
   constexpr uint32_t ACT_CHUNK = BPAD * 128;
   constexpr int STG_LD = 40;
-  static_assert(decode_attn_smem_floats<MG_NW>() * 4 <= MG_KCH * ACT_CHUNK, "attention scratch must fit the activation buffer");
+  static_assert(decode_attn_smem_floats<MG_ATTN_NW>() * 4 <= MG_KCH * ACT_CHUNK, "attention scratch must fit the activation buffer");
   static_assert(BPAD * STG_LD * 2 <= MG_KCH * ACT_CHUNK, "SwiGLU staging must fit the activation buffer");
   extern __shared__ uint8_t smem_raw[];
   __shared__ __align__(8) uint64_t bar_full[MG_MAX_STAGES];
   __shared__ __align__(8) uint64_t bar_empty[MG_MAX_STAGES];
-  __shared__ float red[16];
-  __shared__ MegaUnit s_units[MG_PH];
+  __shared__ float red[D / 32];
+  __shared__ MegaCta s_cta;
   __shared__ MegaLayerDev s_layers[MG_MAX_LAYERS];
 
   const uint32_t sbase = (smem_u32(smem_raw) + 1023u) & ~1023u;
@@ -92,18 +99,19 @@
     }
     asm volatile("fence.mbarrier_init.release.cluster;" ::: "memory");
   }
-  if (threadIdx.x >= 64 && threadIdx.x < 64 + MG_PH) s_units[threadIdx.x - 64] = p.units[(threadIdx.x - 64) * G + cta];
+  if (threadIdx.x == 64) s_cta = p.ctas[cta];
   if (threadIdx.x >= 128 && threadIdx.x < 128 + p.num_layers) s_layers[threadIdx.x - 128] = p.layers[threadIdx.x - 128];
   __syncthreads();
 
   if (warp == 0) {
     if (lane == 0) {
       const uint8_t* src = p.wstream + p.cta_off[cta];
+      const int nu = s_cta.n[0] + s_cta.n[1] + s_cta.n[2] + s_cta.n[3];
       int it = 0;
       for (int l = 0; l < p.num_layers; ++l)
-        for (int ph = 0; ph < MG_PH; ++ph) {
-          const int nblk = s_units[ph].nblk;
-          const uint32_t bytes = (uint32_t)s_units[ph].nrows * 128u;
+        for (int i = 0; i < nu; ++i) {
+          const int nblk = s_cta.u[i].nblk;
+          const uint32_t bytes = (uint32_t)s_cta.u[i].nrows * 128u;
           for (int j = 0; j < nblk; ++j, ++it) {
             const int s = it % NST;
             if (it >= NST) mbar_wait(smem_u32(&bar_empty[s]), ((uint32_t)(it / NST) & 1u) ^ 1u);
@@ -122,8 +130,8 @@
   } else {
     const int wt = threadIdx.x - 32;
     const int ww = warp - 1;
-    unsigned bar_target = __ldcg(p.bar + 1);
-    const unsigned gen0 = bar_target;
+    const unsigned base = __ldcg(p.prog + cta);
+    auto done = [&](int l, int ph) { return base + (unsigned)(MG_NPHASE * l + ph + 1); };
     int mma_it = 0, tl_i = 0;
     const bool stamp = p.tl != nullptr && cta == 0 && wt == 0;
     if (stamp) p.tl[tl_i++] = gtime();
@@ -133,26 +141,25 @@
     const bool fs_cta = p.tl != nullptr && (cta == 0 || cta == 100) && wt == 0;
 #define FS() do { if (fs_cta && fs_on && fs_i < 250) fs[fs_i++] = gtime(); } while (0)
 
-    auto grid_sync = [&]() {
-      bar_target += (unsigned)G;
+    auto wait_for = [&](bool need, unsigned target) {
       FS();
+      if (need) {
+        const long long t0 = clock64();
+        while ((int)(ld_acquire(p.prog + wt) - target) < 0) {
+          if (clock64() - t0 > 4000000000ll) __trap();
+        }
+      }
       worker_bar();
-      if (wt == 0) {
-        red_release_add(p.bar, 1u);
-        FS();
-        const long long t0 = clock64();
-        while ((int)(ld_acquire(p.bar) - bar_target) < 0) {
-          if (clock64() - t0 > 4000000000ll) __trap();
-        }
-        if (stamp) p.tl[tl_i++] = gtime();
-        FS();
-      }
+      FS();
+    };
+    auto in_set = [&](int w) { return wt < G && ((s_cta.wait[w][wt >> 5] >> (wt & 31)) & 1u); };
+    auto finish = [&](int l, int ph) {
       worker_bar();
+      if (wt == 0) st_release(p.prog + cta, done(l, ph));
+      if (stamp) p.tl[tl_i++] = gtime();
     };
 
-    auto gemm_phase = [&](int ph, const bf16* actg, int K, float* out_f32, int N, int mode) {
-      const MegaUnit u = s_units[ph];
-      if (u.nblk <= 0) return;
+    auto gemm_unit = [&](const MegaUnit& u, const bf16* actg, int K, float* out_f32, int N, int mode) {
       {
         const int items = u.nblk * B * 8;
         constexpr int UN = 4;
@@ -230,47 +237,48 @@
         }
       }
       mma_it += u.nblk;
+      worker_bar();
     };
-
-    auto reduce_norm = [&](const float* part, auto splits_tag, const float* gamma) {
-      constexpr int S = decltype(splits_tag)::value;
-      for (int b = cta; b < B; b += G) {
-        float ld[2][S + 1];
-#pragma unroll
-        for (int h = 0; h < 2; ++h) {
-          const int n = wt + h * MG_WORKERS;
-          const bool ok = n < D;
-          ld[h][0] = ok ? __ldcg(p.x + (size_t)b * D + n) : 0.f;
-#pragma unroll
-          for (int s = 0; s < S; ++s) ld[h][s + 1] = ok ? __ldcg(part + ((size_t)s * B + b) * D + n) : 0.f;
-        }
-        float v[2], ss = 0.f;
-#pragma unroll
-        for (int h = 0; h < 2; ++h) {
-          float a = 0.f;
-#pragma unroll
-          for (int s = 0; s < S; ++s) a += ld[h][s + 1];
-          v[h] = ld[h][0] + a;
-          const int n = wt + h * MG_WORKERS;
-          if (n < D) {
-            p.x[(size_t)b * D + n] = v[h];
-            ss += v[h] * v[h];
-          }
-        }
-        ss = warp_sum(ss);
-        if (lane == 0) red[ww] = ss;
-        FS();
-        worker_bar();
-        float tot = 0.f;
-#pragma unroll
-        for (int i = 0; i < MG_NW; ++i) tot += red[i];
-        const float r = rsqrtf(tot / D + RMS_EPS);
-#pragma unroll
-        for (int h = 0; h < 2; ++h) {
-          const int n = wt + h * MG_WORKERS;
-          if (n < D) p.xn[(size_t)b * D + n] = __float2bfloat16_rn(gamma[n] * (v[h] * r));
-        }
-        worker_bar();
+    auto gemm_phase = [&](int ph, const bf16* actg, int K, float* out_f32, int N, int mode) {
+      int i0 = 0;
+      for (int q = 0; q < ph; ++q) i0 += s_cta.n[q];
+      for (int i = i0; i < i0 + s_cta.n[ph]; ++i) gemm_unit(s_cta.u[i], actg, K, out_f32, N, mode);
+    };
+
+    auto reduce_norm = [&](const float* part, int splits, const float* gamma) {
+      const int b = cta;
+      constexpr int NG = D / 32;
+      float v[2];
+#pragma unroll
+      for (int h = 0; h < 2; ++h) {
+        const int grp = ww + h * MG_NW;
+        if (grp < NG) {
+          const int n = grp * 32 + lane;
+          const float xv = __ldcg(p.x + (size_t)b * D + n);
+          float a[4] = {0.f, 0.f, 0.f, 0.f};
+          for (int s0 = 0; s0 < splits; s0 += 4) {
+            float ld[4];
+#pragma unroll
+            for (int q = 0; q < 4; ++q) ld[q] = s0 + q < splits ? __ldcg(part + ((size_t)(s0 + q) * B + b) * D + n) : 0.f;
+            split_add(a, ld, s0, splits);
+          }
+          v[h] = xv + split_total(a);
+          p.x[(size_t)b * D + n] = v[h];
+          const float ss = warp_sum(v[h] * v[h]);
+          if (lane == 0) red[grp] = ss;
+        }
+      }
+      worker_bar();
+      float tot = 0.f;
+#pragma unroll
+      for (int i = 0; i < NG; ++i) tot += red[i];
+#pragma unroll
+      for (int h = 0; h < 2; ++h) {
+        const int grp = ww + h * MG_NW;
+        if (grp < NG) {
+          const int n = grp * 32 + lane;
+          p.xn[(size_t)b * D + n] = __float2bfloat16_rn(gamma[n] * (v[h] * rsqrtf(tot / D + RMS_EPS)));
+        }
       }
     };
 
@@ -279,7 +287,8 @@
       fs_on = l == 1;
       bf16* kc_l = p.kcache + (size_t)l * p.kv_layer_stride;
       bf16* vc_l = p.vcache + (size_t)l * p.kv_layer_stride;
-      if (cta < B * NKV && warp >= 8) {
+      const bool attn = cta < B * NKV;
+      if (attn && warp >= 8) {
         const int b = cta / NKV, kvh = cta % NKV;
         const int L = min(p.ctx_len[b], p.max_ctx);
         const bf16* kb = kc_l + ((size_t)b * NKV + kvh) * p.max_ctx * HD;
@@ -289,32 +298,52 @@
           prefetch_l2(vb + (size_t)j * HD);
         }
       }
-      gemm_phase(0, p.xn, D, p.part_qkv, QKV_N, 0);
-      grid_sync();
-      for (int u = cta; u < B * NKV; u += G) {
-        const int b = u / NKV, kvh = u % NKV;
+      if (s_cta.n[0]) {
+        if (l > 0) wait_for(wt < B, done(l - 1, P_NORM2));
+        gemm_phase(0, p.xn, D, p.part_qkv, QKV_N, 0);
+      }
+      finish(l, P_QKV);
+      if (attn) {
+        wait_for(in_set(W_ATTN), done(l, P_QKV));
+        const int b = cta / NKV, kvh = cta % NKV;
         bf16* kb = kc_l + ((size_t)b * NKV + kvh) * p.max_ctx * HD;
         bf16* vb = vc_l + ((size_t)b * NKV + kvh) * p.max_ctx * HD;
         KvFrag fr;
-        decode_attn_unit<MG_NW, 1, MG_SPL_QKV>(attn_sm, wt, p.part_qkv, MG_SPL_QKV, B, b, kvh, Lw.qkv_bias, kb, vb, p.ctx_len[b], p.max_ctx,
+        decode_attn_unit<MG_ATTN_NW, 1, MG_NW>(attn_sm, wt, p.part_qkv, p.spl_qkv, B, b, kvh, Lw.qkv_bias, kb, vb, p.ctx_len[b], p.max_ctx,
                                                p.inv_freq, p.att + (size_t)b * D, fr, false);
-        worker_bar();
-      }
-      grid_sync();
-      gemm_phase(1, p.att, D, p.part_o, D, 0);
-      grid_sync();
-      reduce_norm(p.part_o, std::integral_constant<int, MG_SPL_O>(), Lw.ln2);
-      grid_sync();
-      gemm_phase(2, p.xn, D, nullptr, 2 * DFF, 1);
-      grid_sync();
-      gemm_phase(3, p.ffa, DFF, p.part_down, D, 0);
-      grid_sync();
-      reduce_norm(p.part_down, std::integral_constant<int, MG_SPL_DOWN>(), Lw.next_gamma);
-      if (l + 1 < p.num_layers) grid_sync();
-    }
-    if (cta == 0 && wt == 0) {
-      p.bar[1] = gen0 + (unsigned)G * (unsigned)(7 * p.num_layers - 1);
-      if (stamp) p.tl[tl_i++] = gtime();
+      }
+      finish(l, P_ATTN);
+      if (s_cta.n[1]) {
+        bool need = false;
+        if (wt < B * NKV)
+          for (int i = s_cta.n[0]; i < s_cta.n[0] + s_cta.n[1]; ++i) {
+            const int h = wt % NKV, g = NH / NKV;
+            need |= s_cta.u[i].kc0 / g <= h && h <= (s_cta.u[i].kc0 + s_cta.u[i].nblk - 1) / g;
+          }
+        wait_for(need, done(l, P_ATTN));
+        gemm_phase(1, p.att, D, p.part_o, D, 0);
+      }
+      finish(l, P_O);
+      if (cta < B) {
+        wait_for(in_set(W_NORM1), done(l, P_O));
+        reduce_norm(p.part_o, p.spl_o, Lw.ln2);
+      }
+      finish(l, P_NORM1);
+      if (s_cta.n[2]) {
+        wait_for(wt < B, done(l, P_NORM1));
+        gemm_phase(2, p.xn, D, nullptr, 2 * DFF, 1);
+      }
+      finish(l, P_GATE_UP);
+      if (s_cta.n[3]) {
+        wait_for(in_set(W_DOWN), done(l, P_GATE_UP));
+        gemm_phase(3, p.ffa, DFF, p.part_down, D, 0);
+      }
+      finish(l, P_DOWN);
+      if (cta < B) {
+        wait_for(in_set(W_NORM2), done(l, P_DOWN));
+        reduce_norm(p.part_down, p.spl_down, Lw.next_gamma);
+      }
+      finish(l, P_NORM2);
     }
   }
 }
@@ -340,62 +369,88 @@
   int splits[MG_PH] = {0, 0, 0, 0};
   uint8_t* wstream = nullptr;
   unsigned long long* cta_off = nullptr;
-  MegaUnit* units = nullptr;
+  MegaCta* ctas = nullptr;
   MegaLayerDev* layers = nullptr;
   size_t stream_bytes = 0;
 };
 
 struct MegaSession {
   float *part_qkv = nullptr, *part_o = nullptr, *part_down = nullptr;
-  unsigned* bar = nullptr;
+  unsigned* prog = nullptr;
 };
 
 void lm_mega_build(cvk_ctx* ctx, LlmModel* m) {
   const int G = ctx->num_sms, L = m->num_layers;
-  if (L > MG_MAX_LAYERS) return;
-  std::vector<MegaUnit> units((size_t)MG_PH * G, MegaUnit{0, 0, 0, 0, 0});
-  auto put = [&](int ph, int c, MegaUnit u) {
-    c = ((c % G) + G) % G;
-    CVK_REQUIRE(units[(size_t)ph * G + c].nblk == 0, "lm mega: two units on one CTA in a phase");
-    units[(size_t)ph * G + c] = u;
-  };
-  const int qkv_tiles = QKV_N / MG_TILE, o_tiles = D / MG_TILE, down_chunks = DFF / MG_BK;
-  if (qkv_tiles * MG_SPL_QKV > G || o_tiles * MG_SPL_O > G || o_tiles * MG_SPL_DOWN > G) return;
-  for (int t = 0; t < qkv_tiles; ++t)
-    for (int s = 0; s < MG_SPL_QKV; ++s) put(0, t * MG_SPL_QKV + s, MegaUnit{t * MG_TILE, MG_TILE, s * MG_CPU_QKV, MG_CPU_QKV, s});
-  for (int t = 0; t < o_tiles; ++t)
-    for (int s = 0; s < MG_SPL_O; ++s) put(1, G - o_tiles * MG_SPL_O + t * MG_SPL_O + s, MegaUnit{t * MG_TILE, MG_TILE, s * MG_CPU_O, MG_CPU_O, s});
+  if (L > MG_MAX_LAYERS || G < 64 * NKV || G > 32 * MG_MASKW) return;
+  const SkinnySplit sq = skinny_split(G, QKV_N, D), so = skinny_split(G, D, D), sd = skinny_split(G, D, DFF);
+  if (sq.splits > 4 || so.splits > 4) return;
+  std::vector<std::vector<MegaUnit>> cu((size_t)MG_PH * G);
+  std::vector<size_t> load(G, 0);
   {
     const int groups = 2 * DFF / 8, base = groups / G, extra = groups % G;
     if ((base + (extra ? 1 : 0)) * 8 > MG_MAXROWS || base < 1) return;
     int row = 0;
     for (int c = 0; c < G; ++c) {
       const int nr = (base + (c < extra ? 1 : 0)) * 8;
-      put(2, c, MegaUnit{row, nr, 0, MG_KCH, 0});
+      cu[(size_t)2 * G + c].push_back(MegaUnit{row, nr, 0, MG_KCH, 0});
+      load[c] += (size_t)nr * 128 * MG_KCH;
       row += nr;
     }
   }
-  {
-    const int base = down_chunks / MG_SPL_DOWN, extra = down_chunks % MG_SPL_DOWN;
-    for (int t = 0; t < o_tiles; ++t) {
-      int kc = 0;
-      for (int s = 0; s < MG_SPL_DOWN; ++s) {
-        const int nb = base + (s < extra ? 1 : 0);
-        put(3, t * MG_SPL_DOWN + s, MegaUnit{t * MG_TILE, MG_TILE, kc, nb, s});
-        kc += nb;
-      }
+  auto deal = [&](int ph, int N, int K, SkinnySplit sp) {
+    std::vector<MegaUnit> us;
+    const int kch = K / MG_BK;
+    for (int t = 0; t < N / MG_TILE; ++t)
+      for (int s = 0; s < sp.splits; ++s) us.push_back(MegaUnit{t * MG_TILE, MG_TILE, s * sp.cps, std::min(sp.cps, kch - s * sp.cps), s});
+    std::stable_sort(us.begin(), us.end(), [](const MegaUnit& x, const MegaUnit& y) { return x.nblk > y.nblk; });
+    for (const MegaUnit& u : us) {
+      int best = 0;
+      for (int c = 1; c < G; ++c)
+        if (load[c] < load[best] || (load[c] == load[best] && cu[(size_t)ph * G + c].size() < cu[(size_t)ph * G + best].size())) best = c;
+      cu[(size_t)ph * G + best].push_back(u);
+      load[best] += (size_t)u.nblk * MG_TILE * 128;
+    }
+  };
+  deal(0, QKV_N, D, sq);
+  deal(1, D, D, so);
+  deal(3, D, DFF, sd);
+  std::vector<MegaCta> ctas(G);
+  for (int c = 0; c < G; ++c) {
+    MegaCta& t = ctas[c];
+    memset(&t, 0, sizeof(t));
+    int i = 0;
+    for (int ph = 0; ph < MG_PH; ++ph) {
+      t.n[ph] = (int)cu[(size_t)ph * G + c].size();
+      for (const MegaUnit& u : cu[(size_t)ph * G + c]) {
+        if (i == MG_MAX_UNITS) return;
+        t.u[i++] = u;
+      }
+    }
+  }
+  auto add = [&](MegaCta& t, int w, int c) { t.wait[w][c >> 5] |= 1u << (c & 31); };
+  for (int c = 0; c < G; ++c) {
+    MegaCta& t = ctas[c];
+    const int h = c % NKV;
+    for (int o = 0; o < G; ++o) {
+      for (const MegaUnit& u : cu[(size_t)0 * G + o]) {
+        const int tile = u.row0 / MG_TILE, hd = tile < NH ? tile / (NH / NKV) : (tile - NH) % NKV;
+        if (hd == h) add(t, W_ATTN, o);
+      }
+      if (!cu[(size_t)1 * G + o].empty()) add(t, W_NORM1, o);
+      if (!cu[(size_t)3 * G + o].empty()) add(t, W_NORM2, o);
+      const MegaUnit& g = cu[(size_t)2 * G + o][0];
+      for (const MegaUnit& u : cu[(size_t)3 * G + c])
+        if (g.row0 < 2 * MG_BK * (u.kc0 + u.nblk) && 2 * MG_BK * u.kc0 < g.row0 + g.nrows) add(t, W_DOWN, o);
     }
   }
   LmMega* mg = new LmMega();
   mg->G = G;
-  mg->splits[0] = MG_SPL_QKV; mg->splits[1] = MG_SPL_O; mg->splits[2] = 1; mg->splits[3] = MG_SPL_DOWN;
-  std::vector<unsigned> lbytes(G, 0);
+  mg->splits[0] = sq.splits; mg->splits[1] = so.splits; mg->splits[2] = 1; mg->splits[3] = sd.splits;
   std::vector<unsigned long long> off(G, 0);
   size_t total = 0;
   for (int c = 0; c < G; ++c) {
-    for (int ph = 0; ph < MG_PH; ++ph) lbytes[c] += (unsigned)(units[(size_t)ph * G + c].nblk * units[(size_t)ph * G + c].nrows * 128);
     off[c] = total;
-    total += (size_t)lbytes[c] * L;
+    total += load[c] * L;
   }
   mg->stream_bytes = total;
   mg->wstream = (uint8_t*)ctx->dmalloc(total);
@@ -404,15 +459,15 @@
     for (int l = 0; l < L; ++l) {
       const LayerW& w = m->layers[l];
       const ConvW* Ws[MG_PH] = {&w.qkv, &w.o, &w.gate_up_il, &w.down};
-      unsigned long long dst = off[c] + (unsigned long long)l * lbytes[c];
-      for (int ph = 0; ph < MG_PH; ++ph) {
-        const MegaUnit& u = units[(size_t)ph * G + c];
-        CVK_REQUIRE(u.nblk == 0 || (Ws[ph]->w16 && u.row0 + u.nrows <= Ws[ph]->N && (u.kc0 + u.nblk) * MG_BK <= Ws[ph]->K), "lm mega: unit outside its weight");
-        for (int j = 0; j < u.nblk; ++j) {
-          descs.push_back(PackDesc{Ws[ph]->w16, Ws[ph]->K, u.row0, u.nrows, u.kc0 + j, dst});
-          dst += (unsigned long long)u.nrows * 128;
-        }
-      }
+      unsigned long long dst = off[c] + (unsigned long long)l * load[c];
+      for (int ph = 0; ph < MG_PH; ++ph)
+        for (const MegaUnit& u : cu[(size_t)ph * G + c]) {
+          CVK_REQUIRE(Ws[ph]->w16 && u.row0 + u.nrows <= Ws[ph]->N && (u.kc0 + u.nblk) * MG_BK <= Ws[ph]->K, "lm mega: unit outside its weight");
+          for (int j = 0; j < u.nblk; ++j) {
+            descs.push_back(PackDesc{Ws[ph]->w16, Ws[ph]->K, u.row0, u.nrows, u.kc0 + j, dst});
+            dst += (unsigned long long)u.nrows * 128;
+          }
+        }
     }
   {
     PackDesc* dd = nullptr;
@@ -435,7 +490,7 @@
     return d;
   };
   mg->cta_off = (unsigned long long*)up(off.data(), off.size() * sizeof(unsigned long long));
-  mg->units = (MegaUnit*)up(units.data(), units.size() * sizeof(MegaUnit));
+  mg->ctas = (MegaCta*)up(ctas.data(), ctas.size() * sizeof(MegaCta));
   mg->layers = (MegaLayerDev*)up(lay.data(), lay.size() * sizeof(MegaLayerDev));
   CVK_CHECK_CUDA(cudaFuncSetAttribute(lm_mega_kernel<32>, cudaFuncAttributeMaxDynamicSharedMemorySize, (int)mega_smem<32>()));
   CVK_CHECK_CUDA(cudaFuncSetAttribute(lm_mega_kernel<64>, cudaFuncAttributeMaxDynamicSharedMemorySize, (int)mega_smem<64>()));
@@ -460,7 +515,7 @@
   ms->part_qkv = (float*)alloc((size_t)mg->splits[0] * s->max_batch * QKV_N * sizeof(float));
   ms->part_o = (float*)alloc((size_t)mg->splits[1] * s->max_batch * D * sizeof(float));
   ms->part_down = (float*)alloc((size_t)mg->splits[3] * s->max_batch * D * sizeof(float));
-  ms->bar = (unsigned*)alloc(64);
+  ms->prog = (unsigned*)alloc((size_t)mg->G * sizeof(unsigned));
   s->mega_state = ms;
 }
 
@@ -476,14 +531,15 @@
   CVK_REQUIRE(mg && ms && B >= 1 && B <= 64 && m->num_layers <= MG_MAX_LAYERS, "lm mega: not initialised");
   const int bpad = B <= 32 ? 32 : 64;
   MegaParams p;
-  p.wstream = mg->wstream; p.cta_off = mg->cta_off; p.units = mg->units; p.layers = mg->layers;
+  p.wstream = mg->wstream; p.cta_off = mg->cta_off; p.ctas = mg->ctas; p.layers = mg->layers;
   p.num_layers = m->num_layers; p.B = B; p.max_ctx = s->max_ctx;
+  p.spl_qkv = mg->splits[0]; p.spl_o = mg->splits[1]; p.spl_down = mg->splits[3];
   p.x = s->x; p.xn = (bf16*)s->xn; p.att = (bf16*)s->att; p.ffa = (bf16*)s->ffa;
   p.part_qkv = ms->part_qkv; p.part_o = ms->part_o; p.part_down = ms->part_down;
   p.kcache = (bf16*)s->kcache; p.vcache = (bf16*)s->vcache;
   p.kv_layer_stride = (unsigned long long)s->max_batch * NKV * s->max_ctx * HD;
   p.ctx_len = s->ctx_len; p.inv_freq = m->d_inv_freq;
-  p.bar = ms->bar;
+  p.prog = ms->prog;
   p.tl = ctx->tl ? (long long*)ctx->tl + 2048 : nullptr;
   cudaLaunchConfig_t cfg = {};
   cfg.gridDim = dim3(mg->G);
```

New measurement: 437.9 (median of 6 runs). +1.7%, better.
